# pingooio/pingoo

Hardware: AMD Instinct MI355X
Metric: requests/sec matched (whole node), 1k-rule WAF (higher is better)
Workload: dtype u8

## Files before the change

### pingoo_amd/csrc/engine.cpp

```cpp
#include <hip/hip_runtime_api.h>

#include <cstdio>
#include <algorithm>
#include <cstring>
#include <map>
#include <memory>
#include <mutex>
#include <string>
#include <type_traits>
#include <unordered_map>
#include <vector>

#include "dirtable.h"
#include "georec.h"
#include "frontend.h"
#include "kernels.h"
#include "lscan_split.h"
#include "program.h"
#include "records.h"

using namespace pwaf;

struct pwaf_program {
    std::unique_ptr<Program> p;
// ... 81 lines not shown
struct PinBuf {
    void *p = nullptr;
    size_t cap = 0;
    int reserve(size_t bytes) {
        if (bytes <= cap) return PWAF_OK;
        if (p) (void)hipHostFree(p);
        p = nullptr;
        cap = 0;
        size_t want = bytes + bytes / 4 + 4096;
        hipError_t e = hipHostMalloc(&p, want, hipHostMallocPortable);
        if (e != hipSuccess) return fail(PWAF_E_NOMEM, std::string("hipHostMalloc failed: ") + hipGetErrorString(e));
        cap = want;
        return PWAF_OK;
    }
    void release() {
        if (p) (void)hipHostFree(p);
        p = nullptr;
        cap = 0;
    }
};

template <class T>
int upload(DevBuf &b, const std::vector<T> &v, size_t pad_bytes = 0) {
    size_t bytes = v.size() * sizeof(T);
    int rc = b.reserve(bytes + pad_bytes + 16);
    if (rc) return rc;
    if (bytes) HIP_TRY(hipMemcpy(b.p, v.data(), bytes, hipMemcpyHostToDevice));
    if (pad_bytes + 16) HIP_TRY(hipMemset((char *)b.p + bytes, 0, pad_bytes + 16));
    return PWAF_OK;
}

struct FlatDev {
    DevBuf flat, flat_classmap, emit_off, emit_list, end_off, end_list, delta;
    uint32_t n_states = 0, n_classes = 0;
    bool scalar_mode = false;
    uint32_t ill_class = 0;
    uint32_t n_full = 0, n_delta = 0;
    void release() {
        for (DevBuf *b : {&flat, &flat_classmap, &emit_off, &emit_list, &end_off, &end_list, &delta}) b->release();
        n_states = 0;
    }
};

struct DevGroup {
    DevBuf tab, classmap, special, list_off, list;
    uint32_t n_states, stride, n_classes, n_hot, start_emit, emit_base, special_base, atom_base, n_local;
    bool scalar_mode = false;
    uint32_t ill_class = 0;
    uint8_t field;
    uint32_t chunks = 1;
    int gate = -1;
    bool filtered = false;
    int share_owner = -1;
    uint32_t shared_bits = 0;
    int need_slot = -1;
    int visit_slot = -1;
    bool identity = false;
    GroupFilter filter;
    DevBuf ftable;
    FlatDev fl, rt;
    bool short_lit = false;
    DevBuf c_head, c_entries, c_bytes, c_classes;
    bool confirm = false;
    bool confirm_walk = false;
};

}

struct Scratch {
    std::mutex mu;
    hipStream_t stream = nullptr, side = nullptr;
    hipEvent_t ev_fork = nullptr, ev_join = nullptr, done = nullptr;
    bool used = false;
    hipStream_t last = nullptr;
    bool last_own = false;
    DevBuf status;
    uint64_t pool_entries = 0;
    struct View { void *p = nullptr; };
    View res_cols;
    bool retry = false;
    DevBuf err_sink;
    DevBuf ipres;
    DevBuf rec, pool, gate_lists, attr;
    DevBuf verdict_spill;
    DevBuf res_words;
    DevBuf zero_block;
    View ctrl, cand_bits, visit_bits, walk_bits;
    DevBuf chunk_bits, cand_cnt;
    DevBuf need;
    DevBuf pairs;
    DevBuf zero_off;
    static constexpr uint32_t kArgSlots = 8;
    DevBuf args;
    PinBuf arg_slot[kArgSlots];
    hipEvent_t arg_ev[kArgSlots] = {};
    bool arg_pending[kArgSlots] = {};
    uint32_t arg_next = 0;
    std::vector<DevBuf> stage_field_data, stage_field_off;
    DevBuf stage_ip, stage_v6, stage_port, stage_flags, stage_asn, stage_country, stage_out, stage_counts;
    DevBuf stage_hits, stage_hit_counts;
    DevBuf stage_geo;
    PinBuf pin_in, pin_out, pin_status;
    DevBuf packed;
    DevBuf rec_meta, rec_cols;
    PinBuf rec_pin, rec_back;
    int ensure(bool own_stream) {
        if (!side) {
            int least = 0, greatest = 0;
            (void)hipDeviceGetStreamPriorityRange(&least, &greatest);
            if (switches().side_priority_high) least = greatest;
            if (hipStreamCreateWithPriority(&side, hipStreamNonBlocking, least) != hipSuccess || hipEventCreateWithFlags(&ev_fork, hipEventDisableTiming) != hipSuccess ||
                hipEventCreateWithFlags(&ev_join, hipEventDisableTiming) != hipSuccess || hipEventCreateWithFlags(&done, hipEventDisableTiming) != hipSuccess)
                return fail(PWAF_E_DEVICE, "hipStreamCreate / hipEventCreate failed");
            for (hipEvent_t &ev : arg_ev)
                if (hipEventCreateWithFlags(&ev, hipEventDisableTiming) != hipSuccess) return fail(PWAF_E_DEVICE, "hipEventCreate failed");
        }
        if (own_stream && !stream && hipStreamCreateWithFlags(&stream, hipStreamNonBlocking) != hipSuccess) return fail(PWAF_E_DEVICE, "hipStreamCreate failed");
        return PWAF_OK;
    }
    void release() {
        for (DevBuf *b : {&status, &ipres, &rec, &res_words, &err_sink, &pool, &verdict_spill, &zero_block, &gate_lists, &attr, &chunk_bits, &cand_cnt, &need, &pairs, &zero_off, &args, &stage_ip, &stage_v6, &stage_port, &stage_flags,
                          &stage_asn, &stage_country, &stage_out, &stage_counts, &stage_geo, &stage_hits, &stage_hit_counts})
            b->release();
        for (PinBuf &b : arg_slot) b.release();
        for (hipEvent_t ev : arg_ev)
            if (ev) (void)hipEventDestroy(ev);
        for (auto &b : stage_field_data) b.release();
        for (auto &b : stage_field_off) b.release();
        packed.release();
        for (PinBuf *b : {&pin_in, &pin_out, &pin_status}) b->release();
        rec_meta.release();
        rec_cols.release();
        rec_pin.release();
        rec_back.release();
        if (stream) (void)hipStreamDestroy(stream);
        if (side) (void)hipStreamDestroy(side);
        for (hipEvent_t ev : {ev_fork, ev_join, done})
            if (ev) (void)hipEventDestroy(ev);
    }
};
static constexpr size_t kContexts = 3;

struct pwaf_engine {
    pwaf_program prog;
    int device = 0;
    std::vector<std::unique_ptr<Scratch>> ctx;
    size_t next_ctx = 0;
    std::vector<DevGroup> groups;
    DevBuf num_atoms, bit_atoms , trig_off, trig_rules, always_rules, country_luts , rules, lits, set_masks;
    uint32_t cmp_vars = 0;
    uint32_t cc_words = 1, n_cmp_atoms = 0, n_bit_atoms = 0, n_trig = 0, n_lazy = 0;
    DevBuf lazy_atoms;
    std::vector<uint32_t> lazy_vars;
    uint32_t n_short = 0;
    int short_field = -1;
    DevBuf short_atoms;
    uint32_t class_words = 1, acmp_words = 0, geo_default = 0, n_classes = 1;
    DevBuf class_rows, dir_esc, leaf_root, geo_leaf_root;
    std::vector<uint32_t> host_cc_masks, host_iu_masks1;
    std::vector<std::pair<uint32_t, uint32_t>> host_acmp;
    std::vector<int64_t> host_iu_vals1;
    DevBuf iu_vals[2], iu_masks[2];
    uint32_t iu_n[2] = {0, 0}, iu_words[2] = {1, 1};
    DevBuf ip_root4, ip_root6, ip_nodes, geo_root4, geo_root6, geo_nodes, geo_recs;
    std::mutex mu;
    std::mutex prof_mu;
    DevBuf residual_errors;
    std::string residual_note;
    JitKernel residual_jit;
    DevBuf residual_blob, geo_rec_root4, geo_rec_root6, geo_rec_nodes;
    DevBuf pass_base, colmask, dir24 , dir_chunks, dir_vals, dir_summary;
    uint32_t dir_sum_shift = 0, dir_common = 0;
    uint32_t dir_n_esc = 0, dir_n_vals = 0;
// ... 506 lines not shown
            HIP_TRY(hipEventCreate(&x));
            e->ev.push_back(x);
        }
        HIP_TRY(hipEventRecord(e->ev[ev_i], on));
        ev_i++;
        return PWAF_OK;
    }
    int begin(hipStream_t side = nullptr) {
        if (off()) return PWAF_OK;
        if (!side && last_main >= 0) { open_begin = last_main; return PWAF_OK; }
        const int rc = record(side ? side : stream);
        if (rc) return rc;
        open_begin = (long)ev_i - 1;
        if (!side) last_main = open_begin;
        return PWAF_OK;
    }
    int end(const char *name, uint64_t alg_bytes, hipStream_t side = nullptr) {
        if (sync_each) {
            hipError_t se = hipStreamSynchronize(side ? side : stream);
            fprintf(stderr, "[pwaf] %s done: %s\n", name, hipGetErrorString(se));
        }
        if (off()) return PWAF_OK;
        const int rc = record(side ? side : stream);
        if (rc) return rc;
        if (!side) last_main = (long)ev_i - 1;
        pwaf_kernel_time t{};
        snprintf(t.name, sizeof t.name, "%s", name);
        t.alg_bytes = alg_bytes;
        e->times.push_back(t);
        e->time_ev.push_back({(size_t)open_begin, ev_i - 1});
        return PWAF_OK;
    }
    void commit() { e->n_timed = ev_i; }
};

struct ArgSlotMark {
    Scratch &S;
    hipStream_t stream;
    int slot = -1;
    int record() {
        if (slot < 0) return PWAF_OK;
        const int k = slot;
        slot = -1;
        S.arg_pending[k] = true;
        HIP_TRY(hipEventRecord(S.arg_ev[k], stream));
        return PWAF_OK;
    }
    ~ArgSlotMark() { (void)record(); }
};

struct BatchRun {
    pwaf_engine *e;
    Scratch &S;
    const Program &P;
    const pwaf_batch &db;
    hipStream_t stream;
    const std::vector<uint32_t> *col_begin;
    const Switches &sw;
    KernelTimer prof;
    ArgSlotMark arg_slot;
    uint32_t n, n_groups, residual_pass, n_passes, bit_words, pair_stride;
    size_t n_slots, ctrl_words;
    uint32_t pool_cap = 0;
    uint32_t *status_word = nullptr;
    bool zero_deferred = false;
    size_t zero_bytes = 0;
    std::vector<pwaf_strcol> cols;
    std::vector<uint32_t> col_bytes;
    std::vector<uint8_t> col_known;
    VerdictArgs v{};
    bool ipres_launched = false, attr_launched = false;
    pwaf_geo *d_geo = nullptr;
    ListShape lshapes[2];
    std::vector<uint32_t> filter_index;
    std::vector<FilterArgs> fall;
    std::vector<FilterArgs> by_stride[2];
    std::vector<ConfirmArgs> call;
    std::vector<ListScanArgs> la[2];
    ColPtrChunk ptrs{};
    uint64_t alg_bytes[3] = {0, 0, 0};
    const FilterArgs *d_all = nullptr, *d_s1 = nullptr, *d_s2 = nullptr;
    const ConfirmArgs *d_c = nullptr;
    const ListScanArgs *d_la[2] = {nullptr, nullptr};
    uint32_t *c_plan = nullptr, *l_plan = nullptr;

    BatchRun(pwaf_engine *e_, Scratch &S_, const pwaf_batch &db_, hipStream_t stream_, const std::vector<uint32_t> *col_begin_)
        : e(e_), S(S_), P(*e_->prog.p), db(db_), stream(stream_), col_begin(col_begin_), sw(switches()), prof(e_, stream_), arg_slot{S_, stream_} {
        n = db.n;
        n_groups = (n + 63) / 64;
        residual_pass = (uint32_t)e->groups.size() + (P.fcmp.empty() ? 0u : 1u);
        n_passes = residual_pass + (P.n_residual ? 1u : 0u);
        bit_words = 2 * n_groups;
        pair_stride = std::max(1u, e->n_bit_atoms + e->n_cmp_atoms + e->n_short);
        n_slots = (size_t)std::max(kGapLists, e->n_gated);
        ctrl_words = 2 + n_slots + e->n_filtered;
    }


    int reserve_scratch(bool sync_status) {
        int rc;
        const uint64_t pool_cap64 = std::max<uint64_t>(std::max<uint64_t>(1u << 20, (uint64_t)n * 8), S.pool_entries);
        pool_cap = (uint32_t)std::min<uint64_t>(pool_cap64, 0x7FFFFFF0u);
        S.pool_entries = pool_cap;
        if (!S.status.p) {
            if ((rc = S.status.reserve(8))) return rc;
            HIP_TRY(hipMemsetAsync(S.status.p, 0, 8, stream));
        }
        status_word = (uint32_t *)S.status.p + (sync_status ? 1 : 0);
        if ((rc = S.rec.reserve((size_t)std::max(1u, n_passes) * n * 4))) return rc;
        if ((rc = S.attr.reserve(((size_t)n_groups * pair_stride + 64) * 16 + (size_t)n_groups * 4))) return rc;
        if ((rc = S.pool.reserve((size_t)pool_cap * sizeof(PoolEntry)))) return rc;
        uint32_t n_conf = 0;
        for (const DevGroup &d : e->groups) n_conf += (d.filtered && d.confirm) ? 1u : 0u;
        Layout z;
        const size_t z_ctrl = z.take(4 * ctrl_words), z_cand = z.take((size_t)e->n_filtered * bit_words * 4), z_visit = z.take((size_t)e->n_visit * bit_words * 4),
                     z_walk = z.take((size_t)n_conf * bit_words * 4);
        zero_bytes = z.size();
        if ((rc = S.zero_block.reserve(zero_bytes))) return rc;
        zero_deferred = e->n_filtered != 0;
        for (const DevGroup &d : e->groups) zero_deferred = zero_deferred && (d.gate >= 0 || d.identity || d.short_lit);
        if (!zero_deferred) HIP_TRY(hipMemsetAsync(S.zero_block.p, 0, zero_bytes, stream));
        char *const zbase = (char *)S.zero_block.p;
        S.ctrl.p = zbase + z_ctrl;
        S.cand_bits.p = zbase + z_cand;
        S.visit_bits.p = zbase + z_visit;
        S.walk_bits.p = zbase + z_walk;
        if (e->n_gated && (rc = S.gate_lists.reserve((size_t)e->n_gated * n * 4))) return rc;
        if (e->n_need && (rc = S.need.reserve((size_t)e->n_need * n * 4))) return rc;
        return PWAF_OK;
    }

    int resolve_columns(bool totals_known) {
        int rc;
        cols.resize(e->n_fields);
        col_bytes.assign(e->n_fields, 0);
        for (int f = 0; f < PWAF_N_FIELDS; f++) {
            cols[(size_t)f] = db.field[f];
            col_bytes[(size_t)f] = db.field_bytes[f];
        }
        bool missing_header = false;
        for (uint32_t f = PWAF_N_FIELDS; f < e->n_fields; f++) {
            const uint32_t k = f - PWAF_N_FIELDS;
            if (k < db.n_headers && db.headers != nullptr && db.headers[k].data != nullptr && db.headers[k].offsets != nullptr) {
                cols[f] = db.headers[k];
                col_bytes[f] = db.header_bytes ? db.header_bytes[k] : 0u;
            } else {
                missing_header = true;
            }
        }
        if (missing_header) {
            if (S.zero_off.cap < (size_t)(n + 1) * 4 + PWAF_ARENA_PAD) {
                if ((rc = S.zero_off.reserve((size_t)(n + 1) * 4 + PWAF_ARENA_PAD))) return rc;
                HIP_TRY(hipMemsetAsync(S.zero_off.p, 0, S.zero_off.cap, stream));
            }
            for (uint32_t f = PWAF_N_FIELDS; f < e->n_fields; f++)
                if (cols[f].data == nullptr) {
                    cols[f].data = (const uint8_t *)S.zero_off.p;
                    cols[f].offsets = (const uint32_t *)S.zero_off.p;
                    col_bytes[f] = 0;
                }
        }
        col_known.assign(e->n_fields, totals_known ? 1 : 0);
        for (uint32_t f = 0; f < e->n_fields; f++)
            if (col_bytes[f] != 0 || cols[f].data == (const uint8_t *)S.zero_off.p) col_known[f] = 1;
        return PWAF_OK;
    }

    int fill_verdict_args(pwaf_verdict *d_out, pwaf_counts *d_counts, uint32_t *d_match_idx, uint32_t *d_n_matches) {
        int rc;
        v.n = n;
        v.n_groups = n_groups;
        v.force_global_tables = (P.flags & PWAF_OPT_GLOBAL_VERDICT_TABLES) ? 1u : 0u;
        v.sparse_mode = verdict_mode(P.flags);
        if (v.sparse_mode) {
            const VerdictShape vs = verdict_shape(P.n_cols, (uint32_t)P.rules.size(), e->n_trig, (uint32_t)P.lits.size(), v.force_global_tables != 0, (int)v.sparse_mode, n_passes);
            v.v_cap = vs.v_cap;
            const bool entry_list = v.sparse_mode >= 3;
            const uint32_t spill_cols = entry_list ? P.n_cols : P.n_cols - std::min(vs.v_cap, P.n_cols);
            if (entry_list || spill_cols) {
                if ((rc = S.verdict_spill.reserve((size_t)verdict_blocks_sp(vs, e->n_cus) * vs.waves * spill_cols * 8))) return rc;
                v.spill = (unsigned long long *)S.verdict_spill.p;
            }
        }
        v.debug_skip = sw.debug_skip | (sw.attr_prio ? 0x80000000u : 0u);
        for (int f = 0; f < PWAF_N_FIELDS; f++) v.off[f] = db.field[f].offsets;
        v.ip = db.ip;
        v.ip_is_v6 = db.ip_is_v6;
        v.port = db.port;
        v.flags = db.flags;
        v.asn = db.asn;
        v.country = db.country;
        v.n_cols = P.n_cols;
        v.n_passes = n_passes;
        v.rec = (const uint32_t *)S.rec.p;
        v.passes = (const PassInfo *)e->pass_table.p;
        if (P.n_residual && e->residual_jit.function) {
            v.res_words = (P.n_residual + 31u) / 32u;
            v.res_base = P.residual_base;
            if ((rc = S.res_words.reserve((size_t)v.res_words * n * 4))) return rc;
            v.res_match = (const uint32_t *)S.res_words.p;
        }
        v.cand_bits = (const uint32_t *)S.cand_bits.p;
        v.visit_bits = (const uint32_t *)S.visit_bits.p;
        v.bit_words = bit_words;
        v.n_hlen = (uint32_t)e->hlen_fields.size();
        for (size_t k = 0; k < e->hlen_fields.size(); k++) v.hoff[k] = cols[e->hlen_fields[k]].offsets;
        v.gpairs = (uint4 *)S.attr.p;
        v.ghdr = (uint32_t *)((char *)S.attr.p + ((size_t)n_groups * pair_stride + 64) * 16);
        v.pair_stride = pair_stride;
        v.attr_blocks = e->n_cus;
        v.pool = (const PoolEntry *)S.pool.p;
        v.cmp = (const CmpAtomDev *)e->num_atoms.p;
        v.n_cmp = e->n_cmp_atoms;
        v.cmp_vars = e->cmp_vars;
        v.lazy = (const CmpAtomDev *)e->lazy_atoms.p;
        v.n_lazy = e->n_lazy;
        v.n_lazy_var = (uint32_t)e->lazy_vars.size();
        for (size_t k = 0; k < e->lazy_vars.size(); k++) v.lazy_var[k] = e->lazy_vars[k];
        v.n_short = e->n_short;
        v.short_atoms = (const ShortAtom *)e->short_atoms.p;
        if (e->n_short) {
            v.short_data = cols[(size_t)e->short_field].data;
            v.short_off = cols[(size_t)e->short_field].offsets;
        }
        v.n_trig = e->n_trig;
        v.n_lits = (uint32_t)P.lits.size();
        v.bit_col = (const uint32_t *)e->bit_atoms.p;
        v.trig_off = (const uint32_t *)e->trig_off.p;
        v.trig_rules = (const uint16_t *)e->trig_rules.p;
        v.always_rules = (const uint32_t *)e->always_rules.p;
        for (int var = 0; var < 2; var++) {
            v.iu_vals[var] = (const int64_t *)e->iu_vals[var].p;
            v.iu_masks[var] = (const uint32_t *)e->iu_masks[var].p;
            v.iu_n[var] = e->iu_n[var];
            v.iu_words[var] = e->iu_words[var];
        }
        v.country_masks = (const uint32_t *)e->country_luts.p;
        v.cc_words = e->cc_words;
        v.rules = (const DevRule *)e->rules.p;
        v.n_rules = (uint32_t)P.rules.size();
        v.lits = (const uint32_t *)e->lits.p;
        set_trie_args(e, v);
        if ((rc = S.ipres.reserve((size_t)n * (v.ipres_packed ? 4 : 8) + 64))) return rc;
        v.ipres = (uint32_t *)S.ipres.p;
        v.out = d_out;
        v.counts = (unsigned long long *)d_counts;
        v.match_idx = d_match_idx;
        v.n_matches = d_n_matches;
        return PWAF_OK;
    }

    int zero_head_records() {
        for (size_t k = 0; k < e->groups.size();) {
            size_t k1 = k;
            while (k1 < e->groups.size() && e->groups[k1].filtered && !e->groups[k1].filter.heads.empty()) k1++;
            if (k1 == k) { k++; continue; }
            HIP_TRY(hipMemsetAsync((uint32_t *)S.rec.p + k * (size_t)n, 0, (k1 - k) * (size_t)n * 4, stream));
            k = k1;
        }
        return PWAF_OK;
    }

    void pick_list_shapes() {
        uint32_t variant[2] = {2, 0};
        bool all_confirm = e->n_filtered != 0;
        for (const DevGroup &d : e->groups) all_confirm = all_confirm && (!d.filtered || d.confirm);
        if (all_confirm) variant[0] = 0;
        if (sw.list_shape >= 0) {
            variant[0] = (uint32_t)sw.list_shape & 15u;
            variant[1] = (uint32_t)sw.list_shape >> 4;
        }
        for (int phase = 0; phase < 2; phase++) lshapes[phase] = list_shape(variant[phase]);
    }


    template <class Launch>
    int timed(const char *name, uint64_t bytes, const char *what, Launch &&launch, hipStream_t side = nullptr) {
        const int rc = prof.begin(side);
        if (rc) return rc;
        const int he = launch();
        if (he) return fail(PWAF_E_DEVICE, std::string(what) + " launch failed: " + hipGetErrorString((hipError_t)he));
        return prof.end(name, bytes, side);
    }

    template <class Launch>
    int side_stage(hipStream_t q, const char *name, uint64_t code, const char *what, Launch &&launch) {
        const hipStream_t side = q != stream ? q : nullptr;
        const int rc = timed(name, code, what, launch, side);
        if (rc) return rc;
        if (side) HIP_TRY(hipEventRecord(S.ev_join, q));
        return PWAF_OK;
    }
    int ipres_stage(hipStream_t q) {
        if (ipres_launched) return PWAF_OK;
        ipres_launched = true;
        if (q != stream) {
            HIP_TRY(hipEventRecord(S.ev_fork, stream));
            HIP_TRY(hipStreamWaitEvent(q, S.ev_fork, 0));
        }
        const int rc = side_stage(q, "ipres", 0xFAu, "ipres kernel", [&] { return sw.skip_ipres ? (int)hipMemsetAsync(v.ipres, 0, (size_t)n * (v.ipres_packed ? 4 : 8), q) : launch_ipres(v, q); });
        if (rc || !d_geo) return rc;
        GeoRecArgs ga{};
        set_georec_args(e, ga);
        ga.ip = db.ip;
        ga.ip_is_v6 = db.ip_is_v6;
        ga.asn = db.asn;
        ga.country = db.country;
        ga.n = n;
        ga.out = (uint2 *)d_geo;
        return side_stage(q, "georec", 25ull * n, "georec kernel", [&] { return launch_georec(ga, q); });
    }
    int attr_stage(hipStream_t q) {
        if (attr_launched) return PWAF_OK;
        attr_launched = true;
        if (q == stream && sw.placement == 0) HIP_TRY(hipStreamWaitEvent(stream, S.ev_join, 0));
        return side_stage(q, "attr", 0xFEu, "attribute kernel", [&] { return sw.skip_attr ? (int)hipMemsetAsync(v.ghdr, 0, (size_t)n_groups * 4, q) : launch_attr(v, q); });
    }
    int attr_at_start() {
        int rc;
        if (sw.placement == 0) return ipres_stage(S.side);
        if (sw.placement == 3) return (rc = ipres_stage(S.side)) ? rc : attr_stage(S.side);
        return PWAF_OK;
    }
    int attr_after_filter() {
        int rc;
        switch (sw.placement) {
        case 0: return attr_stage(stream);
        case 1: return (rc = ipres_stage(stream)) ? rc : attr_stage(stream);
        case 2: return (rc = ipres_stage(S.side)) ? rc : attr_stage(S.side);
        default: return PWAF_OK;
        }
    }
    int join_side() {
        if (sw.placement >= 2) HIP_TRY(hipStreamWaitEvent(stream, S.ev_join, 0));
        return PWAF_OK;
    }

    int launch_plain_scans() {
        static const char *fn[5] = {"host", "url", "path", "method", "user_agent"};
        for (size_t gi = 0; gi < e->groups.size(); gi++) {
            const DevGroup &d = e->groups[gi];
            if (d.gate >= 0 || d.identity || d.short_lit) continue;
            const ScanArgs a = scan_args(gi);
            char nm[48];
            if (d.field < PWAF_N_FIELDS) snprintf(nm, sizeof nm, "scan_%s_g%zu", fn[d.field], gi);
            else snprintf(nm, sizeof nm, "scan_hdr%u_g%zu", d.field - PWAF_N_FIELDS, gi);
            prof.streaming = true;
            const int rc = timed(nm, (uint64_t)col_bytes[d.field] + 4ull * (n + 1), "scan kernel", [&] { return launch_scan(a, stream); });
            prof.streaming = false;
            if (rc) return rc;
        }
        return PWAF_OK;
    }

    int launch_filter_stage() {
        prof.streaming = true;
        const int rc = timed(by_stride[1].empty() ? "filter_s1" : by_stride[0].empty() ? "filter_s2" : "filter_mix", alg_bytes[1] + alg_bytes[2], "filter kernel", [&] {
            return launch_filter(by_stride[0].data(), (uint32_t)by_stride[0].size(), d_s1, by_stride[1].data(), (uint32_t)by_stride[1].size(), d_s2, stream);
        });
        prof.streaming = false;
        return rc;
    }
    int launch_resolve_stage() {
        bool any_list = false;
        for (const DevGroup &d : e->groups) any_list = any_list || (d.filtered && !d.confirm);
        return timed("resolve+compact", 0xFCu, "resolve / compact kernel", [&] {
            const int he = launch_resolve(fall.data(), (uint32_t)fall.size(), d_all, stream);
            return !he && any_list ? launch_compact(fall.data(), (uint32_t)fall.size(), d_all, stream) : he;
        });
    }
    int launch_confirm_stage() {
        if (call.empty()) return PWAF_OK;
        return timed("confirm", 0xF8u, "confirm kernel", [&] { return launch_confirm(call.data(), (uint32_t)call.size(), d_c, c_plan, e->n_cus, stream); });
    }
    int launch_list_scans() {
        uint32_t *plan_at = l_plan;
        for (int phase = 0; phase < 2; phase++) {
            uint32_t first = 0;
            for (const uint32_t cnt : e->lscan_launches[phase]) {
                char nm[48];
                snprintf(nm, sizeof nm, "lscan_x%u", cnt);
                const int rc = timed(nm, 0xFDu, "gated scan kernel", [&] { return launch_scan_gated(la[phase].data() + first, cnt, d_la[phase] + first, plan_at, lshapes[phase], stream); });
                if (rc) return rc;
                plan_at += 2 * cnt + 1;
                first += cnt;
            }
        }
        return PWAF_OK;
    }
    int launch_fcmp_stage() {
        if (P.fcmp.empty()) return PWAF_OK;
        FcmpArgs fa{};
        std::vector<uint32_t> slots;
        for (size_t k = 0; k < P.fcmp.size(); k++) {
            uint32_t sl[2];
            const uint32_t fld[2] = {P.fcmp[k].a, P.fcmp[k].b};
            for (int q = 0; q < 2; q++) {
                size_t at = std::find(slots.begin(), slots.end(), fld[q]) - slots.begin();
                if (at == slots.size()) slots.push_back(fld[q]);
                sl[q] = (uint32_t)at;
            }
            fa.atoms[k] = P.fcmp[k].op | (sl[0] << 8) | (sl[1] << 16);
        }
        for (size_t q = 0; q < slots.size() && q < kMaxFcmpFields; q++) {
            fa.data[q] = cols[slots[q]].data;
            fa.off[q] = cols[slots[q]].offsets;
        }
        fa.n = n;
        fa.n_atoms = (uint32_t)P.fcmp.size();
        fa.rec = (uint32_t *)S.rec.p + e->groups.size() * (size_t)n;
        set_pool(fa);
        return timed("fcmp", 0xFBu, "field comparison kernel", [&] { return launch_fcmp(fa, stream); });
    }
    template <class Args>
    int residual_inputs(Args &a) {
        a.data = (const uint8_t *const *)S.res_cols.p;
        a.off = (const uint32_t *const *)((const char *)S.res_cols.p + (size_t)e->n_fields * 8);
        a.blob = (const uint8_t *)e->residual_blob.p;
        a.n = n;
        a.n_rules = P.n_residual;
        a.ip = db.ip;
        a.ip_is_v6 = db.ip_is_v6;
        a.port = db.port;
        a.asn = db.asn;
        a.country = db.country;
        a.has_geo = (P.has_geo && P.residual_needs_geo) ? 1u : 0u;
        a.geo_root4 = (const uint32_t *)e->geo_rec_root4.p;
        a.geo_root6 = (const uint32_t *)e->geo_rec_root6.p;
        a.geo_nodes = (const uint32_t *)e->geo_rec_nodes.p;
        a.geo_recs = (const GeoRec *)e->geo_recs.p;
        a.rule_errors = (unsigned long long *)e->residual_errors.p;
        if (S.retry) {
            const int rc = S.err_sink.reserve((size_t)P.n_residual * 8);
            if (rc) return rc;
            a.rule_errors = (unsigned long long *)S.err_sink.p;
        }
        return PWAF_OK;
    }
    int launch_residual_stage() {
        if (!P.n_residual) return PWAF_OK;
        int rc;
        if (e->residual_jit.function) {
            ResidualJitArgs ja{};
            if ((rc = residual_inputs(ja))) return rc;
            ja.match_words = (uint32_t *)S.res_words.p;
            return timed("residual_jit", 0xF9u, "specialized residual kernel", [&] { return launch_residual_jit(e->residual_jit, ja, e->n_cus, stream); });
        }
        ResidualArgs ra{};
        if ((rc = residual_inputs(ra))) return rc;
        ra.rec = (uint32_t *)S.rec.p + (size_t)residual_pass * n;
        set_pool(ra);
        return timed("residual", 0xF9u, "residual kernel", [&] { return launch_residual(ra, stream); });
    }
    int launch_verdict_stage() { return timed("verdict", 0xFFu, "verdict kernel", [&] { return launch_verdict(v, stream); }); }
    int dump_counts() {
        std::vector<uint32_t> cw(ctrl_words);
        HIP_TRY(hipStreamSynchronize(stream));
        HIP_TRY(hipMemcpy(cw.data(), S.ctrl.p, 4 * ctrl_words, hipMemcpyDeviceToHost));
        fprintf(stderr, "[pwaf] n %u pool %u status %u |", n, cw[0], cw[1]);
        for (size_t k = 0; k < e->groups.size(); k++) {
            const DevGroup &d = e->groups[k];
            if (d.gate >= 0) fprintf(stderr, " pass %zu field %u %s list %u", k, d.field, d.filtered ? (d.confirm ? "confirm" : "filtered") : "gap", cw[2 + (size_t)d.gate]);
        }
        for (uint32_t k = 0; k < e->n_filtered; k++) fprintf(stderr, " pairs[%u] %u", k, cw[2 + n_slots + k]);
        fprintf(stderr, "\n");
        return PWAF_OK;
    }


    template <class Args>
    void set_pool(Args &a) const {
        a.pool = (PoolEntry *)S.pool.p;
        a.pool_count = (uint32_t *)S.ctrl.p;
        a.pool_cap = pool_cap;
        a.status = status_word;
    }
    bool feeds_gates(size_t gi) const { return e->n_gap && e->owns_factors[gi]; }
    template <class Args>
    void set_gate_feed(Args &a, const DevGroup &d) const {
        a.colmask_local = (const uint32_t *)e->colmask.p + d.atom_base;
        a.n_local = d.n_local;
        a.gate_lists = (uint32_t *)S.gate_lists.p;
        a.gate_count = (uint32_t *)S.ctrl.p + 2;
        if constexpr (!std::is_same<Args, ScanArgs>::value) {
            a.enq_bits = (uint32_t *)S.visit_bits.p;
            a.enq_words = bit_words;
        }
    }

    ScanArgs scan_args(size_t gi) const {
        const DevGroup &d = e->groups[gi];
        ScanArgs a{};
        if (feeds_gates(gi)) set_gate_feed(a, d);
        a.data = cols[d.field].data;
        a.off = cols[d.field].offsets;
        a.n = n;
        a.tab = (const uint16_t *)d.tab.p;
        a.classmap = (const uint8_t *)d.classmap.p;
        a.umap = d.scalar_mode ? (const uint8_t *)d.classmap.p + kUmapAt : nullptr;
        a.ill_class = d.ill_class;
        a.special = (const SpecialCell *)d.special.p;
        a.list_off = (const uint32_t *)d.list_off.p;
        a.list = (const uint16_t *)d.list.p;
        a.start_emit = d.start_emit;
        a.emit_base = d.emit_base;
        a.n_cus = e->n_cus;
        a.chunks = d.chunks;
        a.special_base = d.special_base;
        a.n_states = d.n_states;
        a.stride = d.stride;
        a.n_classes = d.n_classes;
        a.n_hot = d.n_hot;
        a.rec = (uint32_t *)S.rec.p + gi * (size_t)n;
        set_pool(a);
        return a;
    }

    int learn_arena_sizes() {
        bool ask = false;
        for (const DevGroup &d : e->groups)
            if (d.filtered && !col_known[d.field]) {
                HIP_TRY(hipMemcpyAsync(&col_bytes[d.field], cols[d.field].offsets + n, 4, hipMemcpyDeviceToHost, stream));
                ask = true;
            }
        if (ask) HIP_TRY(hipStreamSynchronize(stream));
        return PWAF_OK;
    }

    uint32_t slab0_of(uint32_t field) const { return col_begin ? (*col_begin)[field] / kStreamSlab : 0u; }

    int build_filter_args() {
        int rc;
        filter_index.assign(e->groups.size(), 0);
        if (!e->n_filtered) return PWAF_OK;
        const uint32_t words = (n + 31) / 32, n_cblocks = (words + kCompactWords - 1) / kCompactWords;
        uint64_t sub_entries = 0, n_slabs_all = 0, pair_bytes = 0;
        for (const DevGroup &d : e->groups)
            if (d.filtered) {
                const uint64_t slabs = slab_count(col_bytes[d.field], slab0_of(d.field));
                n_slabs_all += slabs;
                sub_entries += slabs * (kStreamSlab / 512);
                if (d.confirm) pair_bytes += (uint64_t)pair_cap_of((uint32_t)slabs, n) * sizeof(uint2);
            }
        if ((rc = S.chunk_bits.reserve((size_t)sub_entries * 4))) return rc;
        if ((rc = S.cand_cnt.reserve((size_t)(2 * n_slabs_all + (uint64_t)e->n_filtered * n_cblocks) * 4))) return rc;
        if (pair_bytes && (rc = S.pairs.reserve((size_t)pair_bytes))) return rc;
        const bool dense_switch = !(P.flags & PWAF_OPT_NO_DENSE_SWITCH);
        uint32_t fi = 0;
        uint64_t sub_at = 0, cnt_at = 0, pair_at = 0;
        for (size_t gi = 0; gi < e->groups.size(); gi++) {
            const DevGroup &d = e->groups[gi];
            if (!d.filtered) continue;
            fall.emplace_back();
            FilterArgs &f = fall.back();
            f.data = cols[d.field].data;
            f.off = cols[d.field].offsets;
            f.n = n;
            f.total = col_bytes[d.field];
            f.init = d.filter.init;
            f.mul = d.filter.mul;
            f.stride = d.filter.stride;
            f.debug = sw.filter_debug_skip;
            f.table = (const uint32_t *)d.ftable.p;
            f.n_heads = (uint32_t)std::min<size_t>(2, d.filter.heads.size());
            for (uint32_t h = 0; h < f.n_heads; h++) {
                const FilterHead &fh = d.filter.heads[h];
                uint8_t lit[16] = {0}, msk[16] = {0};
                memcpy(lit, fh.bytes, fh.len);
                memset(msk, 0xFF, fh.len);
                memcpy(f.head_w[h], lit, 16);
                memcpy(f.head_m[h], msk, 16);
                f.head_len[h] = fh.len | ((uint32_t)fh.exact << 8);
                f.head_code[h] = h == 0 ? (uint32_t)fh.local + 1u : ((uint32_t)fh.local + 1u) << 15;
            }
            f.slab0 = slab0_of(d.field);
            const uint32_t slabs = slabs_of(f);
            f.rec = (uint32_t *)S.rec.p + gi * (size_t)n;
            f.chunk_bits = (uint32_t *)S.chunk_bits.p + sub_at;
            f.sub_count = (uint32_t *)S.cand_cnt.p + cnt_at;
            f.pair_base = f.sub_count + slabs;
            f.block_count = f.pair_base + slabs;
            f.bitmap = (uint32_t *)S.cand_bits.p + (size_t)fi * bit_words;
            filter_index[gi] = fi;
            f.list = (uint32_t *)S.gate_lists.p + (size_t)d.gate * n;
            f.list_count = (uint32_t *)S.ctrl.p + 2 + d.gate;
            if (d.confirm) {
                f.pair_cap = pair_cap_of(slabs, n);
                f.pairs = (uint2 *)((char *)S.pairs.p + pair_at);
                f.pair_count = (uint32_t *)S.ctrl.p + 2 + n_slots + fi;
                pair_at += (uint64_t)f.pair_cap * sizeof(uint2);
                if (dense_switch) {
                    f.dense_flag = f.pair_count;
                    f.dense_thresh = (uint32_t)std::min<uint64_t>(0xFFFFFFFEu, (uint64_t)slabs * (kStreamSlab / 16) / 2);
                }
            }
            f.first_block = 0;
            sub_at += (uint64_t)slabs * (kStreamSlab / 512);
            cnt_at += 2 * slabs + n_cblocks;
            alg_bytes[f.stride == 2 ? 2 : 1] += (uint64_t)f.total + 4ull * (n + 1);
            fi++;
        }
        for (const FilterArgs &f : fall) {
            std::vector<FilterArgs> &sub = by_stride[f.stride == 2 ? 1 : 0];
            const uint32_t block = sub.empty() ? 0u : sub.back().first_block + (slabs_of(sub.back()) + kFilterWaves - 1) / kFilterWaves;
            sub.push_back(f);
            sub.back().first_block = block;
        }
        return PWAF_OK;
    }

    ConfirmArgs confirm_args(const FilterArgs &f, const DevGroup &d, size_t gi, uint32_t wi) const {
        ConfirmArgs c{};
        c.data = f.data;
        c.off = f.off;
        c.n = n;
        c.total = f.total;
        c.pairs = f.pairs;
        c.pair_count = f.pair_count;
        c.pair_cap = f.pair_cap;
        c.mul = f.mul;
        c.stride = f.stride;
        c.init = f.init;
        c.ftable = f.table;
        c.c_head = (const uint32_t *)d.c_head.p;
        c.c_entries = (const ConfirmEntry *)d.c_entries.p;
        c.c_bytes = (const uint8_t *)d.c_bytes.p;
        c.c_classes = (const uint32_t *)d.c_classes.p;
        c.n_entries = (uint32_t)d.filter.confirm.entries.size();
        c.n_bytes = (uint32_t)d.filter.confirm.bytes.size() & ~3u;
        c.n_class_words = (uint32_t)d.filter.confirm.classes.size();
        c.rec = f.rec;
        c.valid_bits = f.bitmap;
        c.dense_flag = f.dense_flag;
        c.dense_thresh = f.dense_thresh;
        c.walk_bits = (uint32_t *)S.walk_bits.p + (size_t)wi * bit_words;
        if (d.confirm_walk) {
            c.walk_list = f.list;
            c.walk_count = f.list_count;
        }
        set_pool(c);
        if (feeds_gates(gi)) {
            set_gate_feed(c, d);
            c.shared_bits = d.shared_bits;
        }
        return c;
    }
    void build_confirm_args() {
        for (size_t gi = 0; gi < e->groups.size(); gi++) {
            const DevGroup &d = e->groups[gi];
            if (d.filtered && d.confirm) call.push_back(confirm_args(fall[filter_index[gi]], d, gi, (uint32_t)call.size()));
        }
    }

    ListScanArgs list_args(size_t gi, const ListShape &lshape, bool full_table = false) const {
        const DevGroup &d = e->groups[gi];
        ListScanArgs a{};
        const DevGroup &src = d.share_owner >= 0 ? e->groups[(size_t)d.share_owner] : d;
        if (!d.identity) {
            a.req_list = (const uint32_t *)S.gate_lists.p + (size_t)src.gate * n;
            a.n_list = (const uint32_t *)S.ctrl.p + 2 + src.gate;
        }
        if (d.visit_slot >= 0) a.visited = (uint32_t *)S.visit_bits.p + (size_t)d.visit_slot * bit_words;
        if (d.share_owner >= 0) {
            a.need_in = (const uint32_t *)S.need.p + (size_t)src.need_slot * n;
            a.need_bit = (uint32_t)d.gate;
        }
        if (feeds_gates(gi)) {
            set_gate_feed(a, d);
            if (d.need_slot >= 0) {
                a.need_out = (uint32_t *)S.need.p + (size_t)d.need_slot * n;
                a.shared_bits = d.shared_bits;
            }
        }
        if (d.confirm) a.merge_rec = 1;
        a.behind_filter = d.filtered ? 1u : 0u;
        a.data = cols[d.field].data;
        a.off = cols[d.field].offsets;
        a.n = n;
        const FlatDev &F = (d.confirm && d.rt.n_states && !full_table) ? d.rt : d.fl;
        a.flat = (const uint16_t *)F.flat.p;
        a.classmap = (const uint8_t *)F.flat_classmap.p;
        a.umap = F.scalar_mode ? (const uint8_t *)F.flat_classmap.p + kUmapAt : nullptr;
        a.ill_class = F.ill_class;
        a.n_classes = F.n_classes;
        const uint32_t row_bytes = 2u * (F.n_classes + 3u), hb = list_hot_bytes(lshape);
        if (F.n_delta && (uint64_t)F.n_full * row_bytes + 48u + 8ull * F.n_delta <= hb) {
            a.n_hot = F.n_full;
            a.n_delta = F.n_delta;
            a.delta = (const uint64_t *)F.delta.p;
        } else {
            a.n_hot = std::min<uint32_t>(F.n_delta ? F.n_full : F.n_states, (hb - 48u) / row_bytes);
        }
        a.emit_off = (const uint32_t *)F.emit_off.p;
        a.emit_list = (const uint16_t *)F.emit_list.p;
        a.end_off = (const uint32_t *)F.end_off.p;
        a.end_list = (const uint16_t *)F.end_list.p;
        a.rec = (uint32_t *)S.rec.p + gi * (size_t)n;
        set_pool(a);
        a.n_cus = e->n_cus;
        return a;
    }
    const FilterArgs *dense_of(size_t gi) const {
        const FilterArgs *f = e->groups[gi].filtered ? &fall[filter_index[gi]] : nullptr;
        return f && f->dense_flag ? f : nullptr;
    }
    static void set_dense(ListScanArgs &a, const FilterArgs &f, uint32_t mode) {
        a.dense_flag = f.dense_flag;
        a.dense_thresh = f.dense_thresh;
        a.dense_mode = mode;
    }
    void build_list_args() {
        for (int phase = 0; phase < 2; phase++)
            for (size_t gi = 0; gi < e->groups.size(); gi++) {
                const DevGroup &d = e->groups[gi];
                if (d.identity ? phase != 0 : (d.gate < 0 || d.filtered != (phase == 0))) continue;
                const FilterArgs *const dense = phase == 0 && d.confirm ? dense_of(gi) : nullptr;
                const FilterArgs *const owner_dense = d.share_owner >= 0 ? dense_of((size_t)d.share_owner) : nullptr;
                if (dense) {
                    ListScanArgs a = list_args(gi, lshapes[phase], true);
                    a.req_list = nullptr;
                    a.n_list = nullptr;
                    a.merge_rec = 0;
                    a.visited = (uint32_t *)S.cand_bits.p + (size_t)filter_index[gi] * bit_words;
                    set_dense(a, *dense, 1);
                    la[phase].push_back(a);
                }
                if (d.confirm && !d.confirm_walk) continue;
                if (sw.skip_identity && d.identity) continue;
                ListScanArgs a = list_args(gi, lshapes[phase]);
                if (dense) set_dense(a, *dense, 2);
                else if (owner_dense) set_dense(a, *owner_dense, 3);
                la[phase].push_back(a);
            }
    }
    int check_list_plan() const {
        for (int phase = 0; phase < 2; phase++) {
            size_t planned = 0;
            for (const uint32_t c : e->lscan_launches[phase]) planned += c;
            if (planned != la[phase].size()) return fail(PWAF_E_DEVICE, "list-scan launch plan does not match the batch's descriptors");
        }
        return PWAF_OK;
    }
    void build_column_pointers() {
        if (!P.n_residual) return;
        const size_t nc = e->n_fields;
        ptrs.count = (uint32_t)(2 * nc);
        for (size_t f = 0; f < nc; f++) { ptrs.p[f] = cols[f].data; ptrs.p[nc + f] = cols[f].offsets; }
    }

    int upload_descriptors() {
        int rc;
        struct Part { size_t at; const void *src; size_t bytes; };
        const size_t b_all = fall.size() * sizeof(FilterArgs), b_s1 = by_stride[0].size() * sizeof(FilterArgs), b_s2 = by_stride[1].size() * sizeof(FilterArgs),
                     b_c = call.size() * sizeof(ConfirmArgs), b_l0 = la[0].size() * sizeof(ListScanArgs), b_l1 = la[1].size() * sizeof(ListScanArgs),
                     b_ptrs = (size_t)ptrs.count * sizeof(void *);
        Layout L;
        const Part up[7] = {{L.take(b_all), fall.data(), b_all}, {L.take(b_s1), by_stride[0].data(), b_s1}, {L.take(b_s2), by_stride[1].data(), b_s2}, {L.take(b_c), call.data(), b_c},
                            {L.take(b_l0 + sizeof(ListScanArgs)), la[0].data(), b_l0}, {L.take(b_l1 + sizeof(ListScanArgs)), la[1].data(), b_l1}, {L.take(b_ptrs), ptrs.p, b_ptrs}};
        const size_t up_bytes = L.size();
        const size_t a_cplan = L.take((call.size() + 2) * 4), a_lplan = L.take((lsplit::plan_words(e->lscan_launches[0]) + lsplit::plan_words(e->lscan_launches[1])) * 4);
        if ((rc = S.args.reserve(L.size()))) return rc;
        char *const abase = (char *)S.args.p;
        d_all = (const FilterArgs *)(abase + up[0].at);
        d_s1 = (const FilterArgs *)(abase + up[1].at);
        d_s2 = (const FilterArgs *)(abase + up[2].at);
        d_c = (const ConfirmArgs *)(abase + up[3].at);
        d_la[0] = (const ListScanArgs *)(abase + up[4].at);
        d_la[1] = (const ListScanArgs *)(abase + up[5].at);
        S.res_cols.p = abase + up[6].at;
        c_plan = (uint32_t *)(abase + a_cplan);
        l_plan = (uint32_t *)(abase + a_lplan);
        if (up_bytes) {
            const uint32_t slot = S.arg_next++ % Scratch::kArgSlots;
            if (S.arg_pending[slot]) HIP_TRY(hipEventSynchronize(S.arg_ev[slot]));
            if ((rc = S.arg_slot[slot].reserve(up_bytes))) return rc;
            char *const hb = (char *)S.arg_slot[slot].p;
            for (const Part &p : up)
                if (p.bytes) memcpy(hb + p.at, p.src, p.bytes);
            arg_slot.slot = (int)slot;
            const int he = upload_args_block(hb, S.args.p, up_bytes, zero_deferred ? S.zero_block.p : nullptr, zero_deferred ? zero_bytes : 0, stream);
            if (he) return fail(PWAF_E_DEVICE, std::string("descriptor upload failed: ") + hipGetErrorString((hipError_t)he));
        } else if (zero_deferred) {
            HIP_TRY(hipMemsetAsync(S.zero_block.p, 0, zero_bytes, stream));
        }
        zero_deferred = false;
        return PWAF_OK;
    }
};

int run_pipeline(pwaf_engine *e, Scratch &S, const pwaf_batch &db , pwaf_verdict *d_out, pwaf_counts *d_counts, uint32_t *d_match_idx,
                 uint32_t *d_n_matches, hipStream_t stream, bool totals_known = false, const std::vector<uint32_t> *col_begin = nullptr, bool sync_status = false,
                 pwaf_geo *d_geo = nullptr, const HitOut *d_hits = nullptr) {
    if (db.n == 0) return PWAF_OK;
    BatchRun b(e, S, db, stream, col_begin);
    b.d_geo = d_geo;
    int rc;
    if ((rc = b.reserve_scratch(sync_status)) || (rc = b.resolve_columns(totals_known))) return rc;
    if ((rc = b.fill_verdict_args(d_out, d_counts, d_match_idx, d_n_matches)) || (rc = b.zero_head_records())) return rc;
    if (d_hits && d_hits->any()) {
        b.v.hits = d_hits->hits;
        b.v.hits_cap = d_hits->cap;
        b.v.n_hits = d_hits->n_hits;
        b.v.rule_hits = (unsigned long long *)d_hits->rule_hits;
    }
    b.pick_list_shapes();
    if ((rc = b.attr_at_start()) || (rc = b.launch_plain_scans())) return rc;
    if ((rc = b.learn_arena_sizes()) || (rc = b.build_filter_args())) return rc;
    b.build_confirm_args();
    b.build_list_args();
    b.build_column_pointers();
    if ((rc = b.check_list_plan()) || (rc = b.upload_descriptors())) return rc;
    if (e->n_filtered) {
        if ((rc = b.launch_filter_stage())) return rc;
        if (!b.sw.attr_after_compact && (rc = b.attr_after_filter())) return rc;
        if ((rc = b.launch_resolve_stage()) || (rc = b.launch_confirm_stage())) return rc;
    }
    if ((rc = b.attr_after_filter())) return rc;
    if ((rc = b.launch_list_scans()) || (rc = b.launch_fcmp_stage()) || (rc = b.launch_residual_stage())) return rc;
    if ((rc = b.join_side()) || (rc = b.launch_verdict_stage())) return rc;
    if (b.sw.dump_counts && (rc = b.dump_counts())) return rc;
    if ((rc = b.arg_slot.record())) return rc;
    b.prof.commit();
    return PWAF_OK;
}

hipError_t mark_context_used(Scratch &S, hipStream_t s, bool own) {
    S.used = true;
    S.last = s;
    S.last_own = own;
    return hipEventRecord(S.done, s);
}

int device_error(const char *call, hipError_t he) { return fail(PWAF_E_DEVICE, std::string(call) + ": " + hipGetErrorString(he)); }

template <class After>
int run_with_retry(pwaf_engine *e, Scratch &S, const pwaf_batch &db, pwaf_verdict *d_out, pwaf_counts *d_counts, bool known, const std::vector<uint32_t> *begins, bool counts_zero,
                   After &&after, pwaf_geo *d_geo = nullptr, const HitOut *d_hits = nullptr) {
    const hipStream_t s = S.stream;
    int r = S.pin_status.reserve(16);
    volatile uint32_t *const st = (volatile uint32_t *)S.pin_status.p;
    for (int attempt = 0;; attempt++) {
        hipError_t he = hipSuccess;
        if (!r && d_counts && !(counts_zero && attempt == 0) && (he = hipMemsetAsync(d_counts, 0, sizeof *d_counts, s)) != hipSuccess) r = device_error("hipMemsetAsync", he);
        if (!r && d_hits && d_hits->n_hits && (he = hipMemsetAsync(d_hits->n_hits, 0, 4, s)) != hipSuccess) r = device_error("hipMemsetAsync", he);
        if (!r && d_hits && d_hits->rule_hits && e->prog.p->n_user_rules && (he = hipMemsetAsync(d_hits->rule_hits, 0, (size_t)e->prog.p->n_user_rules * 8, s)) != hipSuccess)
            r = device_error("hipMemsetAsync", he);
        if (!r) {
            S.retry = attempt > 0;
            r = run_pipeline(e, S, db, d_out, d_counts, nullptr, nullptr, s, known, begins, true, d_geo, d_hits);
            S.retry = false;
        }
        if (!r) {
            he = hipMemcpyAsync((void *)&st[0], (uint32_t *)S.status.p + 1, 4, hipMemcpyDeviceToHost, s);
            if (he == hipSuccess) he = hipMemcpyAsync((void *)&st[1], S.ctrl.p, 4, hipMemcpyDeviceToHost, s);
// ... 1198 lines not shown
            const pwaf_strcol *sc = sample_col(g.field);
            if (!sc || !gf.enabled) continue;
            if (alt[k].enabled) gf = alt[k];
            const uint8_t *data = sc->data;
            const uint32_t *off = sc->offsets;
            if (gf.est_candidate_rate > 0.4) {
                gf.enabled = false;
                gf.heads.clear();
                gf.note = "the filter flags more than 40 % of the sample";
                continue;
            }
            std::vector<uint64_t> &v = visits[k];
            std::fill(v.begin(), v.end(), 0);
            std::vector<uint64_t> &rv = T.rvisits[k];
            if (g.rtier) rv.assign(g.rtier->n_states, 0);
            std::vector<uint8_t> padded;
            if (gf.confirm.enabled) {
                padded.assign(data, data + off[n]);
                padded.resize(padded.size() + 2 * PWAF_ARENA_PAD, 0);
            }
            std::vector<uint16_t> lits;
            for (uint32_t i = 0; i < n; i++) {
                bool walk;
                if (gf.confirm.enabled) {
                    lits.clear();
                    walk = confirm_field_host(gf, padded.data(), off[i], off[i + 1], lits);
                } else {
                    walk = flagged(gf, sc, i);
                }
                if (!walk) continue;
                uint32_t st = 0;
                for (uint32_t p = off[i]; p < off[i + 1]; p++) {
                    st = g.trans[(size_t)st * g.n_classes + dfa_class_at(g, data + off[i], p - off[i], off[i + 1] - off[i])];
                    v[st]++;
                }
                if (g.rtier) {
                    const DfaGroup &r = *g.rtier;
                    uint32_t rs = 0;
                    for (uint32_t p = off[i]; p < off[i + 1]; p++) {
                        rs = r.trans[(size_t)rs * r.n_classes + dfa_class_at(r, data + off[i], p - off[i], off[i + 1] - off[i])];
                        rv[rs]++;
                    }
                }
            }
        }
    }
    for (size_t k = 0; k < P.groups.size(); k++) {
        const pwaf_strcol *sc = sample_col(P.groups[k].field);
        if (!sc) continue;
        const uint32_t *off = sc->offsets;
        const uint64_t total = (uint64_t)(off[n] - off[0]);
        const uint32_t t4 = 80u, t2 = 48u;
        T.chunks[k] = total >= (uint64_t)t4 * n ? 4u : total >= (uint64_t)t2 * n ? 2u : 1u;
    }
    return PWAF_OK;
}
}

int pwaf_program_tune(pwaf_program *p, const pwaf_batch *sample) {
    if (!p || !p->p) return fail(PWAF_E_INVALID_ARG, "program is NULL");
    int rc = validate_batch_header(sample);
    if (rc) return rc;
    if (sample->memory != PWAF_MEM_HOST) return fail(PWAF_E_INVALID_ARG, "pwaf_program_tune needs a HOST-memory sample");
    if (sample->n == 0) return PWAF_OK;
    TuneOut T;
    for (const DfaGroup &g : p->p->groups) T.filters.push_back(g.filter);
    if ((rc = tune_host(*p->p, sample, T))) return rc;
    for (size_t k = 0; k < p->p->groups.size(); k++) p->p->groups[k].filter = T.filters[k];
    p->dump.clear();
    return PWAF_OK;
}

int pwaf_engine_tune(pwaf_engine *e, const pwaf_batch *sample) {
    if (!e) return fail(PWAF_E_INVALID_ARG, "engine is NULL");
    int rc = validate_batch_header(sample);
    if (rc) return rc;
    if (sample->memory != PWAF_MEM_HOST) return fail(PWAF_E_INVALID_ARG, "pwaf_engine_tune needs a HOST-memory sample");
    std::vector<std::unique_lock<std::mutex>> ctx_locks;
    for (auto &c : e->ctx) ctx_locks.emplace_back(c->mu);
    std::lock_guard<std::mutex> lock(e->mu);
    HIP_TRY(hipSetDevice(e->device));
    const Program &P = *e->prog.p;
    if (sample->n == 0) return PWAF_OK;
    TuneOut T;
    for (const DevGroup &d : e->groups) T.filters.push_back(d.filter);
    if ((rc = tune_host(P, sample, T))) return rc;
    bool rows_only = false;
#ifdef PWAF_PROFILING
    rows_only = getenv("PWAF_TUNE_ROWS_ONLY") != nullptr;
#endif
    for (size_t k = 0; k < P.groups.size() && !rows_only; k++) {
        e->groups[k].filter = T.filters[k];
        if (T.chunks[k]) e->groups[k].chunks = T.chunks[k];
    }
    for (uint32_t f = 0; f < e->n_fields && f < T.mean_len.size(); f++)
        if (T.mean_len[f] > 0) e->mean_len[f] = T.mean_len[f];
    HIP_TRY(hipDeviceSynchronize());
    for (size_t k = 0; k < P.groups.size(); k++)
        if ((rc = build_device_group(P.groups[k], P.lds_hot_budget, e->groups[k], &T.visits[k], &T.class_freq[k])) ||
            (rc = build_flat_group(P.groups[k], e->groups[k].fl, e->groups[k].filter.enabled && P.groups[k].filter_cols.empty(), &T.visits[k])) ||
            (P.groups[k].rtier && (rc = build_flat_group(*P.groups[k].rtier, e->groups[k].rt, true, T.rvisits[k].empty() ? nullptr : &T.rvisits[k]))))
            return rc;
    if ((rc = assign_lists(e))) return rc;
    HIP_TRY(hipDeviceSynchronize());
    return PWAF_OK;
}

int pwaf_engine_device_status(pwaf_engine *e) {
    if (!e) return fail(PWAF_E_INVALID_ARG, "NULL argument");
    HIP_TRY(hipSetDevice(e->device));
    HIP_TRY(hipDeviceSynchronize());
    uint32_t any = 0;
    for (auto &c : e->ctx) {
        std::lock_guard<std::mutex> lock(c->mu);
        if (!c->status.p) continue;
        uint32_t status = 0;
        HIP_TRY(hipMemcpy(&status, c->status.p, 4, hipMemcpyDeviceToHost));
        if (status) {
            HIP_TRY(hipMemset(c->status.p, 0, 4));
            uint32_t asked = 0;
            if (c->ctrl.p) HIP_TRY(hipMemcpy(&asked, c->ctrl.p, 4, hipMemcpyDeviceToHost));
            c->pool_entries = std::max<uint64_t>(c->pool_entries * 2, (uint64_t)asked + asked / 4 + 1024);
        }
        any |= status;
    }
    if (any) return fail(PWAF_E_NOMEM, "scan overflow pool exhausted: verdicts of a device-resident batch since the last status call are incomplete "
                                       "(evaluate it again: the pool has been grown; the synchronous entry points retry by themselves)");
    return PWAF_OK;
}

}
namespace {
int evaluate_one_impl(pwaf_engine *e, const pwaf_request *r, pwaf_verdict *out, pwaf_geo *geo) {
    if (r->n_headers && !r->headers) return fail(PWAF_E_INVALID_ARG, "n_headers without a headers array");
    const uint32_t n_hdr = e->n_fields - PWAF_N_FIELDS;
    const uint32_t n_cols = PWAF_N_FIELDS + n_hdr;
    std::vector<const char *> ptr{r->host, r->url, r->path, r->method, r->user_agent};
    std::vector<uint32_t> len{r->host_len, r->url_len, r->path_len, r->method_len, r->user_agent_len};
    for (uint32_t k = 0; k < n_hdr; k++) {
        const bool have = k < r->n_headers;
        ptr.push_back(have ? r->headers[k].data : nullptr);
        len.push_back(have ? r->headers[k].len : 0u);
    }
    std::vector<std::vector<uint8_t>> arena(n_cols);
    std::vector<uint32_t> offs(2 * (size_t)n_cols);
    std::vector<pwaf_strcol> hcols(n_hdr);
    std::vector<uint32_t> hbytes(n_hdr);
    pwaf_batch b{};
    b.struct_size = sizeof b;
    b.n = 1;
    b.memory = PWAF_MEM_HOST;
    for (uint32_t f = 0; f < n_cols; f++) {
        arena[f].assign(len[f] + PWAF_ARENA_PAD, 0);
        if (len[f]) {
            if (!ptr[f]) return fail(PWAF_E_INVALID_ARG, "NULL field with non-zero length");
            memcpy(arena[f].data(), ptr[f], len[f]);
        }
        offs[2 * f] = 0;
        offs[2 * f + 1] = len[f];
        pwaf_strcol &c = f < PWAF_N_FIELDS ? b.field[f] : hcols[f - PWAF_N_FIELDS];
        c.data = arena[f].data();
        c.offsets = &offs[2 * f];
        if (f >= PWAF_N_FIELDS) hbytes[f - PWAF_N_FIELDS] = len[f];
    }
    if (n_hdr) {
        b.n_headers = n_hdr;
// ... 124 lines not shown
```

### pingoo_amd/csrc/kernels.h

```cpp
#pragma once
#include <cstdint>
#include <string>
#include <vector>

#include "program.h"

namespace pwaf {

static constexpr int kMaxPasses = 250;
static constexpr int kVerdictPre = 12;
static constexpr uint32_t kGapLists = 32;
static constexpr uint32_t kMaxHeaderLens = 8;
static constexpr uint32_t kDirChunkWords = 32;

static constexpr uint32_t REC_OVERFLOW = 0x80000000u;
struct PoolEntry {
    uint32_t atom;
    uint32_t next;
};

struct SpecialCell {
    uint32_t next_off;
    uint32_t emit;
};
// ... 33 lines not shown
    uint32_t n;
    const uint16_t *flat;
    const uint8_t *classmap;
    const uint8_t *umap;
    uint32_t ill_class;
    uint32_t n_classes;
    uint32_t n_hot;
    const uint64_t *delta;
    uint32_t n_delta;
    const uint32_t *emit_off;
    const uint16_t *emit_list;
    const uint32_t *end_off;
    const uint16_t *end_list;
    uint32_t *rec;
    PoolEntry *pool;
    uint32_t *pool_count;
    uint32_t pool_cap;
    uint32_t *status;
    const uint32_t *colmask_local;
    uint32_t n_local;
    uint32_t *gate_lists;
    uint32_t *gate_count;
    uint32_t *enq_bits;
    uint32_t enq_words;
    uint32_t behind_filter;
    const uint32_t *req_list;
    const uint32_t *n_list;
    uint32_t *visited;
    uint32_t *need_out;
    uint32_t shared_bits;
    const uint32_t *need_in;
    uint32_t need_bit;
    uint32_t merge_rec;
    uint32_t n_cus;
    const uint32_t *dense_flag;
    uint32_t dense_thresh;
    uint32_t dense_mode;
};
struct ListOf {
    const uint32_t *req_list;
    uint32_t n_l;
};

struct ConfirmArgs {
    const uint8_t *data;
    const uint32_t *off;
    uint32_t n;
    uint32_t total;
    const uint2 *pairs;
    const uint32_t *pair_count;
    uint32_t pair_cap;
    uint32_t mul, stride, init;
    const uint32_t *ftable;
    const uint32_t *c_head;
    const ConfirmEntry *c_entries;
    const uint8_t *c_bytes;
    const uint32_t *c_classes;
    uint32_t n_entries, n_bytes, n_class_words;
    uint32_t *rec;
    uint32_t *valid_bits;
    uint32_t *walk_bits;
    uint32_t *walk_list;
    uint32_t *walk_count;
    PoolEntry *pool;
    uint32_t *pool_count;
    uint32_t pool_cap;
    uint32_t *status;
    const uint32_t *colmask_local;
    uint32_t n_local;
    uint32_t *gate_lists;
    uint32_t *gate_count;
    uint32_t *enq_bits;
    uint32_t enq_words;
    uint32_t shared_bits;
    const uint32_t *dense_flag;
    uint32_t dense_thresh;
};
static constexpr uint32_t kConfirmThreads = 1024;
static constexpr uint32_t kConfirmPoolBytes = 40 * 1024;
struct ConfirmTableDev {
    const ConfirmArgs *c;
    uint32_t count;
};
int launch_confirm(const ConfirmArgs *host, uint32_t count, const ConfirmArgs *dev, uint32_t *plan, uint32_t n_cus, void *stream);

static constexpr uint32_t kStreamSlab = 128 * 1024;
static constexpr uint32_t kStreamIter = 4096;
static constexpr uint32_t kFilterWaves = 4;
static constexpr uint32_t kCompactWords = 2048;
struct FilterArgs {
    const uint8_t *data;
    const uint32_t *off;
    uint32_t n;
    uint32_t total;
    uint32_t slab0;
    uint32_t init;
    uint32_t mul;
    uint32_t stride;
    const uint32_t *table;
    uint32_t n_heads;
    uint32_t head_w[2][4];
    uint32_t head_m[2][4];
    uint32_t head_len[2];
    uint32_t head_code[2];
    uint32_t *rec;
    uint32_t *chunk_bits;
    uint32_t *sub_count;
    uint32_t *bitmap;
    uint32_t *block_count;
    uint32_t *list;
    uint32_t *list_count;
    uint2 *pairs;
    uint32_t *pair_count;
    uint32_t pair_cap;
    uint32_t *pair_base;
    const uint32_t *dense_flag;
    uint32_t dense_thresh;
    uint32_t first_block;
    uint32_t debug;
};
int upload_args_block(const void *host_pinned, void *dev, size_t bytes, void *zero , size_t zero_bytes, void *stream);
struct FilterTable {
    const FilterArgs *f;
    uint32_t count;
};
struct FilterMix {
    const FilterArgs *f1, *f2;
    uint32_t count1, count2, blocks1, blocks2;
};
int launch_filter(const FilterArgs *host1, uint32_t count1, const FilterArgs *dev1, const FilterArgs *host2, uint32_t count2, const FilterArgs *dev2, void *stream);
int launch_resolve(const FilterArgs *host, uint32_t count, const FilterArgs *dev, void *stream);
int launch_compact(const FilterArgs *host, uint32_t count, const FilterArgs *dev, void *stream);
int configure_kernels(int device);

static constexpr uint32_t kSrcSet = 0, kSetWordsMax = 16, kSrcCc = 16, kCcWordsMax = 8, kSrcPort = 24, kSrcAsn = 28, kIntWordsMax = 4, kSrcAcmp = 32, kAcmpWordsMax = 4,
                          kSrcWords = 36;
struct PassInfo {
    uint32_t base;
    uint32_t kind_slot;
};
struct FcmpArgs {
    const uint8_t *data[kMaxFcmpFields];
    const uint32_t *off[kMaxFcmpFields];
    uint32_t atoms[kMaxFcmpAtoms];
    uint32_t n, n_atoms;
    uint32_t *rec;
    PoolEntry *pool;
    uint32_t *pool_count;
    uint32_t pool_cap;
    uint32_t *status;
};
int launch_fcmp(const FcmpArgs &a, void *stream);
struct ResidualArgs {
    const uint8_t *const *data;
    const uint32_t *const *off;
    const uint8_t *blob;
    uint32_t n, n_rules;
    const uint8_t *ip;
    const uint8_t *ip_is_v6;
    const uint16_t *port;
    const uint32_t *asn;
    const uint16_t *country;
    uint32_t has_geo;
    const uint32_t *geo_root4, *geo_root6, *geo_nodes;
    const GeoRec *geo_recs;
    uint32_t *rec;
    PoolEntry *pool;
    uint32_t *pool_count;
    uint32_t pool_cap;
    uint32_t *status;
    unsigned long long *rule_errors;
};
int launch_residual(const ResidualArgs &a, void *stream);
struct ResidualJitArgs {
    const uint8_t *const *data;
    const uint32_t *const *off;
    const uint8_t *blob;
    uint32_t n, n_rules;
    const uint8_t *ip;
    const uint8_t *ip_is_v6;
    const uint16_t *port;
    const uint32_t *asn;
    const uint16_t *country;
    uint32_t has_geo, pad;
    const uint32_t *geo_root4, *geo_root6, *geo_nodes;
    const GeoRec *geo_recs;
    uint32_t *match_words;
    unsigned long long *rule_errors;
};
struct JitKernel {
    void *module = nullptr, *function = nullptr;
};
static constexpr uint32_t kMaxJitRules = 256;
bool rvm_specialize(const uint8_t *blob, size_t len, std::string &out, std::string &why);
bool rvm_jit_program(const uint8_t *blob, size_t len, std::string &out, std::string &why);
bool rtc_compile(const std::string &source, const std::string &arch, std::vector<char> &code, std::string &why);
bool jit_load(const std::vector<char> &code, JitKernel &out, std::string &why);
void jit_release(JitKernel &k);
int launch_residual_jit(const JitKernel &k, const ResidualJitArgs &a, uint32_t n_cus, void *stream);
struct ColPtrChunk {
    const void *p[2 * (PWAF_N_FIELDS + kMaxHeaders)];
    uint32_t count;
};
struct CmpAtomDev {
    uint32_t col, c;
};
struct ShortAtom {
    uint32_t col;
    uint32_t len_exact;
    uint32_t lit_lo, lit_hi;
};
struct VerdictArgs {
    uint32_t n, n_groups;
    uint32_t debug_skip;
    uint32_t force_global_tables;
    uint32_t sparse_mode;
    uint32_t v_cap;
    unsigned long long *spill;
    const uint32_t *off[PWAF_N_FIELDS];
    const uint8_t *ip;
    const uint8_t *ip_is_v6;
    const uint16_t *port;
    const uint8_t *flags;
    const uint32_t *asn;
    const uint16_t *country;
    uint32_t n_passes;
    const uint32_t *rec;
    const PassInfo *passes;
    const uint32_t *res_match;
    uint32_t res_words, res_base;
    const uint32_t *cand_bits, *visit_bits;
    uint32_t bit_words;
    const uint32_t *hoff[kMaxHeaderLens];
    const ShortAtom *short_atoms;
    uint32_t n_short;
    const uint8_t *short_data;
    const uint32_t *short_off;
    uint32_t n_hlen;
    const PoolEntry *pool;
    uint32_t n_cols;
    const CmpAtomDev *cmp;
    uint32_t n_cmp;
    uint32_t cmp_vars;
    const CmpAtomDev *lazy;
    uint32_t n_lazy;
    uint32_t lazy_var[4], n_lazy_var;
    const uint32_t *bit_col;
    const int64_t *iu_vals[2];
    const uint32_t *iu_masks[2];
    uint32_t iu_n[2], iu_words[2];
    const uint32_t *country_masks;
    uint32_t cc_words;
    const DevRule *rules;
    uint32_t n_rules;
    const uint32_t *lits;
    uint32_t n_lits, n_trig;
    const uint32_t *trig_off;
    const uint16_t *trig_rules;
    const uint32_t *always_rules;
    const uint32_t *ip_root4, *ip_root6, *ip_nodes;
    const uint32_t *set_masks;
    uint32_t set_words;
    uint32_t n_ip_lists;
    const uint32_t *geo_root4, *geo_root6, *geo_nodes;
    const uint32_t *dir24;
    const uint32_t *dir_chunks, *dir_vals;
    const uint32_t *dir_summary;
    uint32_t dir_sum_shift, dir_common;
    const uint2 *dir_esc;
    const uint32_t *class_rows;
    uint32_t class_words;
    uint32_t acmp_words;
    uint32_t geo_default;
    uint32_t *ipres;
    uint32_t ipres_packed;
    uint32_t has_geo;
    uint4 *gpairs;
    uint32_t *ghdr;
    uint32_t pair_stride;
    uint32_t attr_blocks;
    pwaf_verdict *out;
    unsigned long long *counts;
    uint32_t *match_idx;
    uint32_t *n_matches;
    pwaf_rule_hit *hits;
    uint32_t hits_cap;
    uint32_t *n_hits;
    unsigned long long *rule_hits;
};

int launch_scan(const ScanArgs &a, void *stream);
struct GatedTable {
    const ListScanArgs *g;
    uint32_t count;
    uint32_t debug;
};
struct ListShape {
    uint32_t threads, hot_bytes, wg_per_cu;
};
ListShape list_shape(uint32_t variant);
uint32_t list_hot_bytes(const ListShape &shape);
int launch_scan_gated(const ListScanArgs *host, uint32_t count, const ListScanArgs *dev, uint32_t *plan, const ListShape &shape, void *stream);
int launch_verdict(const VerdictArgs &a, void *stream);
int launch_ipres(const VerdictArgs &a, void *stream);
int launch_attr(const VerdictArgs &a, void *stream);
int launch_dir24(const VerdictArgs &a, void *out , void *esc, void *esc_count, void *stream);
struct GeoRecArgs {
    const uint8_t *ip, *ip_is_v6;
    const uint32_t *asn;
    const uint16_t *country;
    uint32_t n, has_geo;
    const uint32_t *root4, *root6, *nodes;
    const GeoRec *recs;
    const uint32_t *chunks, *vals, *summary;
    uint32_t sum_shift, common;
    uint32_t n_cus;
    uint2 *out;
};
int launch_georec(const GeoRecArgs &a, void *stream);
uint32_t scan_lds_bytes(uint32_t n_hot, uint32_t stride, uint32_t n_gate_atoms);
struct VerdictShape {
    uint32_t waves, lds_bytes, lds_tables;
    uint32_t sparse, v_cap, per_cu;
};
VerdictShape verdict_shape(uint32_t n_cols, uint32_t n_rules, uint32_t n_trig, uint32_t n_lits, bool force_global = false, int mode = 3, uint32_t n_passes = 0);
uint32_t verdict_blocks_sp(const VerdictShape &sh, uint32_t n_cus);

}
```

### pingoo_amd/csrc/kernels.hip

```cpp
#include <hip/hip_runtime.h>

#include <cstdlib>
#include <mutex>
#include <set>

#include "confirm.h"
#include "utf8.h"
#include "kernels.h"
#include "residual.h"

namespace pwaf {

static constexpr int kScanThreads = 1024;
static constexpr int kScanWaves = kScanThreads / 64;
static constexpr uint32_t kNone = 0xFFFFFFFFu;

#define PWAF_LDS __attribute__((address_space(3)))
#define PWAF_GLOBAL __attribute__((address_space(1)))
typedef const PWAF_LDS uint16_t *lds_u16_ptr;
typedef const PWAF_GLOBAL uint16_t *glb_u16_ptr;
typedef const PWAF_LDS uint32_t *lds_u32_ptr;
typedef const PWAF_LDS uint8_t *lds_u8_ptr;
typedef unsigned int u32x4 __attribute__((ext_vector_type(4)));
typedef u32x4 u32x4_u __attribute__((aligned(1)));
// ... 311 lines not shown
                        if (!slow && t >= emit_base) {
                            const uint32_t code = *reinterpret_cast<lds_u16_ptr>((uintptr_t)((t << 1) + emit_col2 + kClsBytes));
                            const uint32_t x = (code & 0x7FFFu) + 1;
                            if (!(code & 0x8000u) || h.ovf != kNone) slow = true;
                            else if (h.a0 == x || h.a1 == x) {}
                            else if (h.a0 == 0) h.a0 = x;
                            else if (h.a1 == 0) h.a1 = x;
                            else slow = true;
                        }
                        if (slow) {
                            const Walk wk = careful_step(gtab, a.special, a.list_off, a.list, a.pool, a.pool_count, a.pool_cap, hot_elems | (emit_base << 16),
                                                         special_base | (emit_col2 << 16), cur, crow, cls, t, h.a0, h.a1, h.ovf);
                            chain = chain && wk.row == t;
                            cur = wk.row;
                            crow = wk.crow;
                            h = wk.h;
                        } else {
                            cur = t;
                        }
                    } else {
                        chain = chain && t < special_base;
                    }
                };
                redo(t1, c2[k0], (uint32_t)k0 < cnt);
                redo(t2, c2[k0 + 1], (uint32_t)(k0 + 1) < cnt);
                redo(t3, c2[k0 + 2], (uint32_t)(k0 + 2) < cnt);
                redo(t4, c2[k0 + 3], (uint32_t)(k0 + 3) < cnt);
                row = cur;
            } else {
                row = t4;
            }
        }
        }
        p += cnt_all;

        if (r != kNone && p >= end) {
            const uint32_t e = row == hot_elems ? (uint32_t)*reinterpret_cast<glb_u16_ptr>(gtab + crow + (end_col << 1))
                                                : (uint32_t)*reinterpret_cast<lds_u16_ptr>((uintptr_t)(((row + end_col) << 1) + kClsBytes));
            if (e & 0x8000u) {
                const uint32_t x = (e & 0x7FFFu) + 1;
                if (h.ovf == kNone && (h.a0 == x || h.a1 == x)) {
                } else if (h.ovf == kNone && h.a0 == 0) {
                    h.a0 = x;
                } else if (h.ovf == kNone && h.a1 == 0) {
                    h.a1 = x;
                } else {
                    const SlowCtx sc{a.list_off, a.list, a.pool, a.pool_count, a.status, a.pool_cap};
                    h = record_atom(sc, x - 1, h);
                }
            } else if (e) {
                PWAF_EMIT(e - 1);
            }
            a.rec[r] = h.ovf != kNone ? (REC_OVERFLOW | h.ovf) : (h.a0 | (h.a1 << 15));
            if (a.colmask_local != nullptr && (h.a0 | (h.ovf + 1u)) != 0) {
                uint32_t need = 1;
                if (h.ovf == kNone) {
                    need = *reinterpret_cast<lds_u32_ptr>((uintptr_t)(gate_base + (h.a0 - 1) * 4));
                    if (h.a1) need |= *reinterpret_cast<lds_u32_ptr>((uintptr_t)(gate_base + (h.a1 - 1) * 4));
                }
                if (need) enqueue_gated(a.colmask_local, a.pool, a.gate_lists, a.gate_count, a.n, r, h);
            }
            r = kNone;
        }
        if (r == kNone && r2 != kNone) {
            r = r2;
            p = p2;
            end = end2;
            r2 = kNone;
            row = 0;
            h = Hits{0, 0, kNone};
            if (start_emit) PWAF_EMIT(start_emit - 1);
        }
#pragma unroll
        for (int q = 0; q < CH; q++) w[q] = wn[q];
        n_lo = f_lo;
        n_hi = f_hi;
        n_base = f_base;
    }
}

template <int CH, bool WIDE>
__global__ __launch_bounds__(kScanThreads) void scan_kernel(ScanArgs a) { scan_body<CH, WIDE>(a); }

__device__ __forceinline__ ListOf list_of(const ListScanArgs &a) {
    ListOf l{a.req_list, a.req_list != nullptr ? min(*a.n_list, a.n) : a.n};
    if (a.dense_mode != 0u) {
        const bool dense = *a.dense_flag > a.dense_thresh;
        if (a.dense_mode == 1u && !dense) l.n_l = 0u;
        if (a.dense_mode == 2u && dense) l.n_l = 0u;
        if (a.dense_mode == 3u && dense) l = ListOf{nullptr, a.n};
    }
    return l;
}

__global__ __launch_bounds__(256) void lscan_plan_kernel(GatedTable b, uint32_t *plan , uint32_t n_waves) {
    __shared__ uint32_t part[256];
    __shared__ unsigned long long all_entries;
    const uint32_t t = threadIdx.x;
    uint32_t items = 0;
    const uint32_t n_l = t < b.count ? list_of(b.g[t]).n_l : 0u;
    if (t == 0) all_entries = 0ull;
    __syncthreads();
    if (n_l != 0u) atomicAdd(&all_entries, (unsigned long long)n_l);
    __syncthreads();
    if (t < b.count) {
        const uint32_t room = n_waves > b.count ? n_waves - b.count : 1u;
        const unsigned long long per_wave = (all_entries + room - 1u) / room;
        uint32_t epi = 1;
        while (epi < 16u && epi < per_wave) epi <<= 1;
        while (epi < 64u * kListWalks && (n_l + epi - 1) / epi > n_waves) epi <<= 1;
        items = (n_l + epi - 1) / epi;
        plan[b.count + 1 + t] = epi;
    }
    part[t] = items;
    __syncthreads();
    for (uint32_t d = 1; d < 256; d <<= 1) {
        const uint32_t v = t >= d ? part[t - d] : 0u;
        __syncthreads();
        part[t] += v;
        __syncthreads();
    }
    if (t < b.count) plan[t] = part[t] - items;
    if (t == 0) plan[b.count] = part[255];
}

__device__ __forceinline__ uint32_t list_step_slow(const uint16_t *hot, const PWAF_GLOBAL uint16_t *flat, const uint64_t *delta, const uint32_t state, const uint32_t c,
                                                   const uint32_t stride, const uint32_t n_hot, const uint32_t n_delta) {
    if (state < n_hot) return hot[state * stride + c];
    const uint32_t k = state - n_hot;
    if (k < n_delta) {
        if (c + 2u == stride) return state;
        const uint64_t rec = delta[k];
        const uint32_t lo = (uint32_t)rec, hi = (uint32_t)(rec >> 32);
        if (c == ((lo >> 16) & 0xFFu)) return hi & 0xFFFFu;
        if (c == (lo >> 24)) return hi >> 16;
        return hot[(lo & 0xFFFFu) * stride + c];
    }
    return flat[state * stride + c];
}

template <uint32_t THREADS>
__device__ __forceinline__ void lscan_async(const ListScanArgs &a, const uint16_t *hot, const unsigned char *cls, const uint64_t *delta, uint32_t it, const uint32_t it_end,
                                            const uint32_t first, const uint32_t n_l, const uint32_t hot_elems, const uint32_t epi) {
    const uint32_t ncls = a.n_classes, stride = ncls + 3u;
    const PWAF_GLOBAL unsigned char *gdata = (const PWAF_GLOBAL unsigned char *)a.data;
    const PWAF_GLOBAL uint16_t *flat = (const PWAF_GLOBAL uint16_t *)a.flat;
    auto record_emit = [&](const uint32_t st, Hits &hh) {
        const uint32_t ei = st * stride + ncls;
        const uint32_t code = ei < hot_elems ? (uint32_t)hot[ei] : (uint32_t)flat[ei];
        const uint32_t x = (code & 0x7FFFu) + 1u;
        bool slow = !(code & 0x8000u) || hh.ovf != kNone;
        if (!slow) {
            if (hh.a0 == x || hh.a1 == x) {}
            else if (hh.a0 == 0) hh.a0 = x;
            else if (hh.a1 == 0) hh.a1 = x;
            else slow = true;
        }
        if (slow) hh = emit_list(a.emit_off, a.emit_list, a.pool, a.pool_count, a.status, a.pool_cap, st, hh);
    };
    for (it += wave_index(); it < it_end; it += THREADS / 64u) {
        const uint32_t li = (it - first) * epi + (threadIdx.x & 63u);
        bool live = (threadIdx.x & 63u) < epi && li < n_l;
        if (live && a.need_in != nullptr) live = ((a.need_in[li] >> a.need_bit) & 1u) != 0;
        const uint32_t r = live ? (a.req_list != nullptr ? a.req_list[li] : li) : 0u;
        if (live && a.visited != nullptr) atomicOr(&a.visited[r >> 5], 1u << (r & 31u));
        uint32_t p = live ? a.off[r] : 0u;
        const uint32_t end = live ? a.off[r + 1] : 0u;
        uint32_t state = 0, wp = p;
        Hits h{0, 0, kNone};
        uint32_t need_init = 0;
        if (live && a.merge_rec) {
            h = hits_of_record(a.rec[r]);
            if (a.colmask_local != nullptr && (h.a0 | (h.ovf + 1u)) != 0) need_init = gate_mask(a.colmask_local, a.pool, h);
        }
        if (live && a.emit_off[1] != a.emit_off[0]) h = emit_list(a.emit_off, a.emit_list, a.pool, a.pool_count, a.status, a.pool_cap, 0u, h);
        u32x4 w = *reinterpret_cast<const PWAF_GLOBAL u32x4_u *>(gdata + wp);
        u32x4 wn = *reinterpret_cast<const PWAF_GLOBAL u32x4_u *>(gdata + (wp + 16u < end ? wp + 16u : 0u));
        for (;;) {
            const bool active = p < end;
            const unsigned long long am = __ballot(active);
            if (am == 0) break;
            if (active && p - wp >= 16u) {
                w = wn;
                wp += 16u;
                wn = *reinterpret_cast<const PWAF_GLOBAL u32x4_u *>(gdata + (wp + 16u < end ? wp + 16u : 0u));
            }
            const uint32_t j = (p - wp) >> 2;
            const uint32_t wd = j == 0 ? w.x : j == 1 ? w.y : j == 2 ? w.z : w.w;
            const uint32_t cnt = active ? min(4u, end - p) : 0u;
            uint32_t c[4], t[4], sv[4];
#pragma unroll
            for (uint32_t k = 0; k < 4; k++) c[k] = cls[(wd >> (k * 8)) & 0xFFu];
            asm volatile("" : "+v"(c[0]), "+v"(c[1]), "+v"(c[2]), "+v"(c[3]));
            if (a.umap != nullptr && __ballot(active && (wd & 0x80808080u) != 0u) != 0ull) {
                const uint32_t f_start = active ? a.off[r] : 0u;
#pragma unroll
                for (uint32_t k = 0; k < 4; k++) {
                    const uint32_t byte = (wd >> (k * 8)) & 0xFFu;
                    if (byte >= 0xC0u && k < cnt) c[k] = lead_class(a.umap, a.ill_class, gdata, byte, p + k, end);
                    else if (byte >= 0x80u && k < cnt) c[k] = cont_class(c[k], a.ill_class, gdata, p + k, f_start, end);
                }
            }
#pragma unroll
            for (uint32_t k = 0; k < 4; k++) c[k] = k < cnt ? c[k] : ncls + 1u;
#pragma unroll
            for (uint32_t k = 0; k < 4; k++) {
                t[k] = *reinterpret_cast<lds_u16_ptr>((uintptr_t)min(__umul24(k == 0 ? state : sv[k - 1], 2u * stride) + 2u * c[k], 2u * hot_elems));
                sv[k] = t[k] & 0x7FFFu;
            }
            const uint32_t any = t[0] | t[1] | t[2] | t[3], top = max(max(t[0], t[1]), max(t[2], t[3]));
            const bool blocked = active && top == 0xFFFFu;
            const unsigned long long bm = __ballot(blocked);
            const uint32_t n_blocked = (uint32_t)__builtin_popcountll(bm);
            if (n_blocked < 32u && bm != am) {
                if (active && !blocked) {
                    if (any & 0x8000u) {
#pragma unroll
                        for (uint32_t k = 0; k < 4; k++)
                            if (t[k] & 0x8000u) record_emit(sv[k], h);
                    }
                    state = sv[3];
                    p += 4u;
                }
            } else if (blocked) {
#pragma unroll
                for (uint32_t k = 0; k < 4; k++) {
                    const uint32_t tt = list_step_slow(hot, flat, delta, state, c[k], stride, a.n_hot, a.n_delta);
                    state = tt & 0x7FFFu;
                    if (tt & 0x8000u) record_emit(state, h);
                }
                p += 4u;
            }
        }
        if (live) {
            if (a.end_off[state + 1] != a.end_off[state]) h = emit_list(a.end_off, a.end_list, a.pool, a.pool_count, a.status, a.pool_cap, state, h);
            a.rec[r] = h.ovf != kNone ? (REC_OVERFLOW | h.ovf) : (h.a0 | (h.a1 << 15));
            if (a.colmask_local != nullptr) {
                uint32_t need = 0;
                if ((h.a0 | (h.ovf + 1u)) != 0) need = gate_mask(a.colmask_local, a.pool, h);
                if (a.need_out != nullptr) a.need_out[li] = need;
                need &= ~(a.shared_bits | need_init);
                if (need) enqueue_mask_once(a.gate_lists, a.gate_count, a.n, r, need, a.enq_bits, a.enq_words);
            }
        }
    }
}

template <uint32_t THREADS>
__global__ __launch_bounds__(THREADS, THREADS == 512 ? 6 : 4) void lscan_kernel(GatedTable b, const uint32_t *plan, uint32_t hot_bytes) {
    extern __shared__ uint32_t lscan_lds[];
    __builtin_amdgcn_s_setprio(3);
    if ((uint32_t)(uintptr_t)(PWAF_LDS unsigned char *)lscan_lds != 0u) __builtin_trap();
    const uint32_t total = plan[b.count];
    const uint32_t it0 = (uint32_t)((uint64_t)total * blockIdx.x / gridDim.x), it1 = (uint32_t)((uint64_t)total * (blockIdx.x + 1) / gridDim.x);
    const unsigned char *cls = reinterpret_cast<const unsigned char *>(lscan_lds + (hot_bytes + 16u) / 4);
    const uint16_t *hot = reinterpret_cast<const uint16_t *>(lscan_lds);
    for (uint32_t it = it0; it < it1;) {
        uint32_t ps = 0;
        for (uint32_t lo = 0, hi = b.count; lo + 1 < hi;) {
            const uint32_t mid = (lo + hi) >> 1;
            if (plan[mid] <= it) lo = mid;
            else hi = mid;
            ps = lo;
        }
        const uint32_t first = plan[ps], it_end = min(it1, plan[ps + 1]), epi = plan[b.count + 1 + ps];
        ListScanArgs a = load_descriptor(&b.g[ps]);
        const ListOf lst = list_of(a);
        a.req_list = lst.req_list;
        const uint32_t ncls = a.n_classes, stride = ncls + 3u;
        const uint32_t hot_elems = a.n_hot * stride;
        uint64_t *delta_lds = reinterpret_cast<uint64_t *>(lscan_lds) + (hot_elems * 2u + 2u + 15u) / 16u * 2u;
        __syncthreads();
        {
            const uint4 *src = reinterpret_cast<const uint4 *>(a.flat);
            uint4 *dst = reinterpret_cast<uint4 *>(lscan_lds);
            const uint32_t units = (hot_elems * 2u + 15u) / 16u;
            for (uint32_t k = threadIdx.x; k < units; k += THREADS * 4u) {
                uint4 v[4];
#pragma unroll
                for (uint32_t q = 0; q < 4; q++) v[q] = k + q * THREADS < units ? src[k + q * THREADS] : make_uint4(0u, 0u, 0u, 0u);
#pragma unroll
                for (uint32_t q = 0; q < 4; q++)
                    if (k + q * THREADS < units) dst[k + q * THREADS] = v[q];
            }
            if (threadIdx.x < 64) lscan_lds[(hot_bytes + 16u) / 4 + threadIdx.x] = reinterpret_cast<const uint32_t *>(a.classmap)[threadIdx.x];
            for (uint32_t k = threadIdx.x; k < a.n_delta; k += THREADS) delta_lds[k] = a.delta[k];
        }
        __syncthreads();
        if (threadIdx.x == 0) reinterpret_cast<uint16_t *>(lscan_lds)[hot_elems] = 0xFFFFu;
        __syncthreads();
        const uint32_t n_l = lst.n_l;
#ifdef PWAF_PROFILING
        const bool long_list = (b.debug & 1u) ? false : (b.debug & 2u) ? true : (a.behind_filter != 0u && (uint64_t)n_l * 8u >= a.n);
#else
        const bool long_list = a.behind_filter != 0u && (uint64_t)n_l * 8u >= a.n;
#endif
        if (long_list) {
            lscan_async<THREADS>(a, hot, cls, delta_lds, it, it_end, first, n_l, hot_elems, epi);
            it = it_end;
            continue;
        }
        const PWAF_GLOBAL unsigned char *gdata = (const PWAF_GLOBAL unsigned char *)a.data;
        const PWAF_GLOBAL uint16_t *flat = (const PWAF_GLOBAL uint16_t *)a.flat;
        for (uint32_t iw = it + wave_index(); iw < it_end; iw += THREADS / 64u) {
            uint32_t li[kListWalks], r[kListWalks], p[kListWalks], end[kListWalks], state[kListWalks], need_init[kListWalks];
            bool live[kListWalks];
            Hits h[kListWalks];
            u32x4 w[kListWalks];
#pragma unroll
            for (uint32_t u = 0; u < kListWalks; u++) {
                li[u] = (iw - first) * epi + u * 64u + (threadIdx.x & 63u);
                live[u] = (threadIdx.x & 63u) + u * 64u < epi && li[u] < n_l;
                if (live[u] && a.need_in != nullptr) live[u] = ((a.need_in[li[u]] >> a.need_bit) & 1u) != 0;
                r[u] = live[u] ? (a.req_list != nullptr ? a.req_list[li[u]] : li[u]) : 0u;
            }
#pragma unroll
            for (uint32_t u = 0; u < kListWalks; u++) {
                if (live[u] && a.visited != nullptr) atomicOr(&a.visited[r[u] >> 5], 1u << (r[u] & 31));
                p[u] = live[u] ? a.off[r[u]] : 0u;
                end[u] = live[u] ? a.off[r[u] + 1] : 0u;
                state[u] = 0;
                h[u] = Hits{0, 0, kNone};
                need_init[u] = 0;
                if (live[u] && a.merge_rec) {
                    h[u] = hits_of_record(a.rec[r[u]]);
                    if (a.colmask_local != nullptr && (h[u].a0 | (h[u].ovf + 1u)) != 0) need_init[u] = gate_mask(a.colmask_local, a.pool, h[u]);
                }
            }
#pragma unroll
            for (uint32_t u = 0; u < kListWalks; u++) {
                if (live[u] && a.emit_off[1] != a.emit_off[0]) h[u] = emit_list(a.emit_off, a.emit_list, a.pool, a.pool_count, a.status, a.pool_cap, 0u, h[u]);
                w[u] = *reinterpret_cast<const PWAF_GLOBAL u32x4_u *>(gdata + p[u]);
// ... 27 lines not shown
                    if (a.umap != nullptr) lead_here = lead_here || (cnt[u] != 0u && window_has_high(w[u]));
                }
                const bool fix_classes = a.umap != nullptr && __ballot(lead_here) != 0ull;
#pragma unroll
                for (uint32_t k0 = 0; k0 < 16; k0 += 4) {
                    uint32_t c[kListWalks][4], t[kListWalks][4], sv[kListWalks][4];
#pragma unroll
                    for (uint32_t u = 0; u < kListWalks; u++) {
                        const uint32_t wd = k0 == 0 ? w[u].x : k0 == 4 ? w[u].y : k0 == 8 ? w[u].z : w[u].w;
#pragma unroll
                        for (uint32_t k = 0; k < 4; k++) {
                            const uint32_t cl = cls[(wd >> (k * 8)) & 0xFFu];
                            c[u][k] = k0 + k < cnt[u] ? cl : ncls + 1u;
                        }
                        if (fix_classes) {
#pragma unroll
                            for (uint32_t k = 0; k < 4; k++) {
                                const uint32_t byte = (wd >> (k * 8)) & 0xFFu;
                                if (byte >= 0xC0u && k0 + k < cnt[u]) c[u][k] = lead_class(a.umap, a.ill_class, gdata, byte, p[u] + k0 + k, end[u]);
                                else if (byte >= 0x80u && k0 + k < cnt[u]) c[u][k] = cont_class(c[u][k], a.ill_class, gdata, p[u] + k0 + k, live[u] ? a.off[r[u]] : 0u, end[u]);
                            }
                        }
                    }
#pragma unroll
                    for (uint32_t k = 0; k < 4; k++) {
#pragma unroll
                        for (uint32_t u = 0; u < kListWalks; u++) {
                    t[u][k] = *reinterpret_cast<lds_u16_ptr>((uintptr_t)min(__umul24(k == 0 ? state[u] : sv[u][k - 1], 2u * stride) + 2u * c[u][k], 2u * hot_elems));
                            sv[u][k] = t[u][k] & 0x7FFFu;
                        }
                    }
                    uint32_t any = 0, top = 0;
#pragma unroll
                    for (uint32_t u = 0; u < kListWalks; u++)
#pragma unroll
                        for (uint32_t k = 0; k < 4; k++) { any |= t[u][k]; top = max(top, t[u][k]); }
                    if (any & 0x8000u) {
                        if (top == 0xFFFFu) {
#pragma unroll
                            for (uint32_t k = 0; k < 4; k++) {
#pragma unroll
                                for (uint32_t u = 0; u < kListWalks; u++) {
                                    const uint32_t tt = list_step_slow(hot, flat, delta_lds, state[u], c[u][k], stride, a.n_hot, a.n_delta);
                                    state[u] = tt & 0x7FFFu;
                                    if (tt & 0x8000u) record_emit(state[u], h[u]);
                                }
                            }
                        } else {
#pragma unroll
                            for (uint32_t u = 0; u < kListWalks; u++) {
#pragma unroll
                                for (uint32_t k = 0; k < 4; k++)
                                    if (t[u][k] & 0x8000u) record_emit(sv[u][k], h[u]);
                                state[u] = sv[u][3];
                            }
                        }
                    } else {
#pragma unroll
                        for (uint32_t u = 0; u < kListWalks; u++) state[u] = sv[u][3];
                    }
                }
#pragma unroll
                for (uint32_t u = 0; u < kListWalks; u++) {
                    if (p[u] < end[u]) p[u] += 16u;
                    w[u] = wn[u];
                }
            }
#pragma unroll
            for (uint32_t u = 0; u < kListWalks; u++) {
                if (!live[u]) continue;
                if (a.end_off[state[u] + 1] != a.end_off[state[u]]) h[u] = emit_list(a.end_off, a.end_list, a.pool, a.pool_count, a.status, a.pool_cap, state[u], h[u]);
                a.rec[r[u]] = h[u].ovf != kNone ? (REC_OVERFLOW | h[u].ovf) : (h[u].a0 | (h[u].a1 << 15));
                if (a.colmask_local != nullptr) {
                    uint32_t need = 0;
                    if ((h[u].a0 | (h[u].ovf + 1u)) != 0) need = gate_mask(a.colmask_local, a.pool, h[u]);
                    if (a.need_out != nullptr) a.need_out[li[u]] = need;
                    need &= ~(a.shared_bits | need_init[u]);
                    if (need) enqueue_mask_once(a.gate_lists, a.gate_count, a.n, r[u], need, a.enq_bits, a.enq_words);
                }
            }
        }
        it = it_end;
    }
}

__global__ __launch_bounds__(256) void confirm_plan_kernel(ConfirmTableDev b, uint32_t *plan ) {
    __shared__ uint32_t part[256];
    const uint32_t t = threadIdx.x;
    uint32_t items = 0;
    if (t < b.count) {
        const ConfirmArgs *pa = &b.c[t];
        const bool dense = pa->dense_flag != nullptr && *pa->dense_flag > pa->dense_thresh;
        items = dense ? 0u : (min(*pa->pair_count, pa->pair_cap) + kConfirmThreads - 1) / kConfirmThreads;
    }
    part[t] = items;
    __syncthreads();
    for (uint32_t d = 1; d < 256; d <<= 1) {
        const uint32_t v = t >= d ? part[t - d] : 0u;
        __syncthreads();
        part[t] += v;
        __syncthreads();
    }
    if (t < b.count) plan[t] = part[t] - items;
    if (t == 0) plan[b.count] = part[255];
}

__device__ __noinline__ void merge_atom(PoolEntry *pool, uint32_t *pool_count, uint32_t *status, uint32_t pool_cap, uint32_t *rec, uint32_t atom) {
    auto rmw_read = [](uint32_t *p) { return atomicOr(p, 0u); };
    auto publish = [&](uint32_t idx, uint32_t at, uint32_t next) {
        const uint32_t t0 = atomicExch(&pool[idx].atom, at), t1 = atomicExch(&pool[idx].next, next);
        asm volatile("" ::"v"(t0), "v"(t1));
    };
    uint32_t old = rmw_read(rec);
    for (;;) {
        uint32_t upd;
        const uint32_t x = atom + 1u;
        if (!(old & REC_OVERFLOW)) {
            const uint32_t a0 = old & 0x7FFFu, a1 = (old >> 15) & 0x7FFFu;
            if (a0 == x || a1 == x) return;
            if (a0 == 0u) upd = old | x;
            else if (a1 == 0u) upd = old | (x << 15);
            else {
                const uint32_t idx = atomicAdd(pool_count, 3u);
                if (idx + 3u > pool_cap) { atomicOr(status, 1u); return; }
                publish(idx, a0 - 1u, kNone);
                publish(idx + 1u, a1 - 1u, idx);
                publish(idx + 2u, atom, idx + 1u);
                upd = REC_OVERFLOW | (idx + 2u);
            }
        } else {
            const uint32_t head = old & ~REC_OVERFLOW;
            for (uint32_t i = head; i != kNone; i = rmw_read(&pool[i].next))
                if (rmw_read(&pool[i].atom) == atom) return;
            const uint32_t idx = atomicAdd(pool_count, 1u);
            if (idx >= pool_cap) { atomicOr(status, 1u); return; }
            publish(idx, atom, head);
            upd = REC_OVERFLOW | idx;
        }
        const uint32_t seen = atomicCAS(rec, old, upd);
        if (seen == old) return;
        old = seen;
    }
}

__global__ __launch_bounds__(kConfirmThreads, 8) void confirm_kernel(ConfirmTableDev b, const uint32_t *plan) {
    __shared__ uint32_t head[kFilterEntries], ftab[kFilterEntries];
    __shared__ uint32_t pool[kConfirmPoolBytes / 4];
    constexpr uint32_t kConfirmQueue = 1024;
    __shared__ uint32_t app_cnt, app_base, app_queue[kConfirmQueue];
    __builtin_amdgcn_s_setprio(3);
    if (threadIdx.x == 0) app_cnt = 0;
    const uint32_t total = plan[b.count];
    const uint32_t it0 = (uint32_t)((uint64_t)total * blockIdx.x / gridDim.x), it1 = (uint32_t)((uint64_t)total * (blockIdx.x + 1) / gridDim.x);
    for (uint32_t it = it0; it < it1;) {
        uint32_t ps = 0;
        for (uint32_t lo = 0, hi = b.count; lo + 1 < hi;) {
            const uint32_t mid = (lo + hi) >> 1;
            if (plan[mid] <= it) lo = mid;
            else hi = mid;
            ps = lo;
        }
        const uint32_t first_item = plan[ps], it_end = min(it1, plan[ps + 1]);
        const ConfirmArgs a = load_descriptor(&b.c[ps]);
        __syncthreads();
        {
            const uint4 *sh = reinterpret_cast<const uint4 *>(a.c_head), *sf = reinterpret_cast<const uint4 *>(a.ftable);
            constexpr uint32_t kPer = kFilterEntries / 4 / kConfirmThreads;
            uint4 vh[kPer], vf[kPer];
#pragma unroll
            for (uint32_t q = 0; q < kPer; q++) { vh[q] = sh[q * kConfirmThreads + threadIdx.x]; vf[q] = sf[q * kConfirmThreads + threadIdx.x]; }
#pragma unroll
            for (uint32_t q = 0; q < kPer; q++) {
                reinterpret_cast<uint4 *>(head)[q * kConfirmThreads + threadIdx.x] = vh[q];
                reinterpret_cast<uint4 *>(ftab)[q * kConfirmThreads + threadIdx.x] = vf[q];
            }
        }
        const uint32_t e_words = a.n_entries * 3u, b_words = a.n_bytes / 4u, c_words = a.n_class_words;
        const bool in_lds = (uint64_t)e_words + b_words + c_words <= kConfirmPoolBytes / 4;
        const ConfirmEntry *t_entries = a.c_entries;
        const uint8_t *t_bytes = a.c_bytes;
        const uint32_t *t_classes = a.c_classes;
        if (in_lds) {
            const uint32_t *se = reinterpret_cast<const uint32_t *>(a.c_entries), *sb = reinterpret_cast<const uint32_t *>(a.c_bytes);
            for (uint32_t k = threadIdx.x; k < e_words; k += kConfirmThreads) pool[k] = se[k];
            for (uint32_t k = threadIdx.x; k < b_words; k += kConfirmThreads) pool[e_words + k] = sb[k];
            for (uint32_t k = threadIdx.x; k < c_words; k += kConfirmThreads) pool[e_words + b_words + k] = a.c_classes[k];
            t_entries = reinterpret_cast<const ConfirmEntry *>(pool);
            t_bytes = reinterpret_cast<const uint8_t *>(pool + e_words);
            t_classes = pool + e_words + b_words;
        }
        __syncthreads();
        const ConfirmView cv{nullptr, t_entries, t_bytes, t_classes, a.mul, a.stride, a.init};
        const uint32_t n_p = min(*a.pair_count, a.pair_cap);
        auto pair_of = [&](const uint32_t item) -> uint2 {
            const uint32_t k = (item - first_item) * kConfirmThreads + threadIdx.x;
            return (item < it_end && k < n_p) ? a.pairs[k] : make_uint2(kNone, 0u);
        };
        uint2 pr_next = pair_of(it), pr_after = pair_of(it + 1u);
        uint32_t fs_next = 0u, fe_next = 0u;
        ConfirmBytes tb_next{};
        if (pr_next.x != kNone) {
            confirm_load64(reinterpret_cast<const uint8_t *>(a.off + pr_next.x), fs_next, fe_next);
            tb_next = confirm_chunk_bytes(a.data, pr_next.y, a.total + PWAF_ARENA_PAD);
        }
        for (; it < it_end; it++) {
            const uint2 pr = pr_next;
            const bool live = pr.x != kNone;
            uint32_t r = live ? pr.x : 0u;
            uint32_t fs = fs_next, fe = fe_next;
            const ConfirmBytes tb = tb_next;
            pr_next = pr_after;
            if (pr_next.x != kNone) {
                confirm_load64(reinterpret_cast<const uint8_t *>(a.off + pr_next.x), fs_next, fe_next);
                tb_next = confirm_chunk_bytes(a.data, pr_next.y, a.total + PWAF_ARENA_PAD);
            }
            pr_after = pair_of(it + 2u);
            ConfirmChunk ch{0u, 0ull};
            if (live) ch = confirm_windows_of(cv, tb, 0u, 0xFFFFFFFFu, pr.y, [&](const uint32_t bin) { return ftab[bin]; });
            uint32_t mask = ch.mask, cnt = 0, j = 0, e0 = 0, pos = 0, widx = 0;
            bool walk = false;
            auto settle = [&](const uint32_t rq, const uint32_t need_lits, const bool wk, const bool aggregated) -> bool {
                bool w2 = wk;
                if (need_lits & a.shared_bits) w2 = true;
                const uint32_t direct = need_lits & ~a.shared_bits;
                if (direct) enqueue_mask_once(a.gate_lists, a.gate_count, a.n, rq, direct, a.enq_bits, a.enq_words);
                if (!w2 || a.walk_list == nullptr) return false;
                const uint32_t bit = 1u << (rq & 31u);
                if (atomicOr(&a.walk_bits[rq >> 5], bit) & bit) return false;
                atomicOr(&a.valid_bits[rq >> 5], bit);
                if (aggregated) return true;
                a.walk_list[atomicAdd(a.walk_count, 1u)] = rq;
                return false;
            };
            uint32_t need = 0;
            for (;;) {
                if (__ballot(j < cnt || mask != 0u) == 0) break;
                while (j >= cnt && mask != 0u) {
                    const uint32_t k = (uint32_t)__builtin_ctz(mask);
                    mask &= mask - 1u;
                    pos = pr.y * 16u + k;
                    const uint32_t bin = confirm_bin_of(ch, widx++, a.data, pos, a.mul);
                    while (pos >= fe && r + 1u < a.n) {
                        settle(r, need, walk, false);
                        need = 0;
                        walk = false;
                        r++;
                        fs = fe;
                        fe = a.off[r + 1];
                    }
                    if (pos >= fe) continue;
                    const uint32_t hd = head[bin];
                    e0 = hd & 0xFFFFFu;
                    cnt = hd >> 20;
                    j = 0;
                }
                if (j < cnt) {
                    const uint32_t res = in_lds ? confirm_entry<3>(t_entries, t_bytes, t_classes, e0 + j, a.data, fs, fe, pos)
                                                : confirm_entry<1>(t_entries, t_bytes, t_classes, e0 + j, a.data, fs, fe, pos);
                    j++;
                    if (res == 2u) {
                        walk = true;
                    } else if (res & 1u) {
                        const uint32_t atom = res >> 8;
                        merge_atom(a.pool, a.pool_count, a.status, a.pool_cap, a.rec + r, atom);
                        atomicOr(&a.valid_bits[r >> 5], 1u << (r & 31u));
                        if (a.colmask_local != nullptr) need |= a.colmask_local[atom];
                    }
                }
            }
            const bool append = live && settle(r, need, walk, true);
            if (append) {
                const uint32_t slot = atomicAdd(&app_cnt, 1u);
                if (slot < kConfirmQueue) app_queue[slot] = r;
                else a.walk_list[atomicAdd(a.walk_count, 1u)] = r;
            }
        }
        __syncthreads();
        {
            const uint32_t queued = min(app_cnt, kConfirmQueue);
            if (threadIdx.x == 0 && queued != 0) app_base = atomicAdd(a.walk_count, queued);
            __syncthreads();
            for (uint32_t k = threadIdx.x; k < queued; k += kConfirmThreads) a.walk_list[app_base + k] = app_queue[k];
            __syncthreads();
            if (threadIdx.x == 0) app_cnt = 0;
        }
    }
}

int launch_scan(const ScanArgs &a, void *stream) {
    const uint32_t lds = scan_lds_bytes(a.n_hot, a.stride, a.colmask_local ? a.n_local : 0u);
    const bool wide = a.n_classes > 127;
    const int v = (a.chunks == 4 ? 2 : a.chunks == 2 ? 1 : 0) + (wide ? 3 : 0);
    const void *fns[6] = {reinterpret_cast<const void *>(scan_kernel<1, false>), reinterpret_cast<const void *>(scan_kernel<2, false>),
                          reinterpret_cast<const void *>(scan_kernel<4, false>), reinterpret_cast<const void *>(scan_kernel<1, true>),
                          reinterpret_cast<const void *>(scan_kernel<2, true>), reinterpret_cast<const void *>(scan_kernel<4, true>)};
    const void *fn = fns[v];
    if (a.n == 0) return 0;
    uint32_t waves = (a.n + 255) / 256;
    uint32_t blocks = (waves + kScanWaves - 1) / kScanWaves;
#ifdef PWAF_PROFILING
    static const uint32_t forced_cap = getenv("PWAF_SCAN_BLOCKS") ? (uint32_t)atoi(getenv("PWAF_SCAN_BLOCKS")) : 0u;
#else
    const uint32_t forced_cap = 0;
#endif
    const uint32_t cap = forced_cap ? forced_cap : std::max(1u, a.n_cus);
    if (blocks > cap) blocks = cap;
    if (blocks == 0) blocks = 1;
    void *args[] = {const_cast<ScanArgs *>(&a)};
    hipError_t e = hipLaunchKernel(fn, dim3(blocks), dim3(kScanThreads), args, lds, (hipStream_t)stream);
    return (int)(e != hipSuccess ? e : hipGetLastError());
}

__global__ __launch_bounds__(256) void copy_args_kernel(const uint4 *__restrict__ src, uint4 *__restrict__ dst, uint32_t n16, uint4 *__restrict__ zero, uint32_t z16) {
    for (uint32_t i = blockIdx.x * 256u + threadIdx.x; i < n16; i += gridDim.x * 256u) dst[i] = src[i];
    for (uint32_t i = blockIdx.x * 256u + threadIdx.x; i < z16; i += gridDim.x * 256u) zero[i] = make_uint4(0u, 0u, 0u, 0u);
}
int upload_args_block(const void *host_pinned, void *dev, size_t bytes, void *zero, size_t zero_bytes, void *stream) {
    const uint32_t n16 = (uint32_t)((bytes + 15) / 16), z16 = (uint32_t)(zero_bytes / 16);
    if (n16 == 0 && z16 == 0) return 0;
    const uint32_t blocks = std::max(std::min<uint32_t>((n16 + 255) / 256, 64u), std::min<uint32_t>((z16 + 2047) / 2048, 1024u));
    hipLaunchKernelGGL(copy_args_kernel, dim3(std::max(1u, blocks)), dim3(256), 0, (hipStream_t)stream, (const uint4 *)host_pinned, (uint4 *)dev, n16, (uint4 *)zero, z16);
    return (int)hipGetLastError();
}

int launch_confirm(const ConfirmArgs *host, uint32_t count, const ConfirmArgs *dev, uint32_t *plan, uint32_t n_cus, void *stream) {
    if (count == 0 || host[0].n == 0) return 0;
    if (count > 256) return (int)hipErrorInvalidValue;
    ConfirmTableDev b{dev, count};
    hipLaunchKernelGGL(confirm_plan_kernel, dim3(1), dim3(256), 0, (hipStream_t)stream, b, plan);
    hipError_t e = hipGetLastError();
    if (e != hipSuccess) return (int)e;
    uint64_t max_items = 0;
    for (uint32_t k = 0; k < count; k++) max_items += ((uint64_t)host[k].pair_cap + kConfirmThreads - 1) / kConfirmThreads;
    const uint32_t blocks = (uint32_t)std::min<uint64_t>(max_items, (uint64_t)std::max(1u, n_cus) * 2u);
    const uint32_t *cplan = plan;
    hipLaunchKernelGGL(confirm_kernel, dim3(blocks), dim3(kConfirmThreads), 0, (hipStream_t)stream, b, cplan);
    return (int)hipGetLastError();
}

static const void *lscan_fn(bool wide) { return wide ? reinterpret_cast<const void *>(lscan_kernel<1024>) : reinterpret_cast<const void *>(lscan_kernel<512>); }

int launch_scan_gated(const ListScanArgs *host, uint32_t count, const ListScanArgs *dev, uint32_t *plan, const ListShape &shape, void *stream) {
    if (count == 0 || host[0].n == 0) return 0;
    if (count > 256) return (int)hipErrorInvalidValue;
    GatedTable b{dev, count, 0u};
#ifdef PWAF_PROFILING
    static const uint32_t async_mode = getenv("PWAF_LSCAN_ASYNC") ? (uint32_t)atoi(getenv("PWAF_LSCAN_ASYNC")) : 0u;
    b.debug = async_mode;
#endif
    const uint32_t blocks = std::max(1u, host[0].n_cus) * shape.wg_per_cu;
    hipLaunchKernelGGL(lscan_plan_kernel, dim3(1), dim3(256), 0, (hipStream_t)stream, b, plan, blocks * (shape.threads / 64u));
    hipError_t e = hipGetLastError();
    if (e != hipSuccess) return (int)e;
    const uint32_t *cplan = plan;
    uint32_t hot_bytes = list_hot_bytes(shape);
    void *args[] = {&b, &cplan, &hot_bytes};
    const void *fn = lscan_fn(shape.threads == 1024);
    e = hipLaunchKernel(fn, dim3(blocks), dim3(shape.threads), args, shape.hot_bytes + 16 + 256, (hipStream_t)stream);
    return (int)(e != hipSuccess ? e : hipGetLastError());
}

uint32_t list_hot_bytes(const ListShape &shape) { return shape.hot_bytes; }

ListShape list_shape(uint32_t variant) {
    switch (variant) {
        case 1: return ListShape{512, 72u * 1024u, 2};
        case 2: return ListShape{1024, 144u * 1024u, 1};
        case 3: return ListShape{512, 32u * 1024u, 4};
        default: return ListShape{kListThreads, kListHotBytes, 3};
    }
}

typedef unsigned short u16x2 __attribute__((ext_vector_type(2)));

template <bool HEADS, int STRIDE>
__device__ __forceinline__ void filter_rows(const FilterArgs &a, const uint32_t blk, const uint32_t wave, const uint32_t lane) {
    const PWAF_GLOBAL unsigned char *gdata = (const PWAF_GLOBAL unsigned char *)a.data;
    const uint32_t rel = blk * kFilterWaves + wave, slab = a.slab0 + rel;
    const uint64_t base64 = (uint64_t)slab * kStreamSlab;
    if (base64 >= a.total) return;
    const uint32_t total = a.total, base0 = (uint32_t)base64, slab_end = (uint32_t)min<uint64_t>(total, base64 + kStreamSlab);
    unsigned long long *my_bits = reinterpret_cast<unsigned long long *>(a.chunk_bits) + (size_t)rel * (kStreamSlab / 1024);
    uint32_t n_hit = 0;
    const uint32_t mul2 = a.mul | (a.mul << 16);
    constexpr uint32_t kRow = 1024;

    auto load_row = [&](const uint32_t b, const uint32_t q) {
        const uint32_t p = b + kRow * q + 16u * lane;
        return *reinterpret_cast<const PWAF_GLOBAL u32x4_u *>(gdata + (p < total ? p : 0u));
    };
    auto dword_at = [&](const uint32_t p) {
        return filter_fold4(*reinterpret_cast<const PWAF_GLOBAL uint32_t __attribute__((aligned(1))) *>(gdata + p));
    };
    auto slot_lo = [](const uint32_t masked) {
        uint32_t r;
        asm("v_lshrrev_b32_sdwa %0, 2, %1 dst_sel:DWORD dst_unused:UNUSED_PAD src0_sel:DWORD src1_sel:WORD_0" : "=v"(r) : "v"(masked));
        return r;
    };
    auto slot_hi = [](const uint32_t masked) {
        uint32_t r;
        asm("v_lshrrev_b32_sdwa %0, 2, %1 dst_sel:DWORD dst_unused:UNUSED_PAD src0_sel:DWORD src1_sel:WORD_1" : "=v"(r) : "v"(masked));
        return r;
    };
    auto bins4 = [&](const uint32_t x, const uint32_t next, uint32_t (&mm)[4]) {
        const uint32_t z = __builtin_amdgcn_alignbit(next, x, 8);
        const uint32_t hx = __builtin_bit_cast(uint32_t, __builtin_bit_cast(u16x2, x) * __builtin_bit_cast(u16x2, mul2));
        const uint32_t hz = __builtin_bit_cast(uint32_t, __builtin_bit_cast(u16x2, z) * __builtin_bit_cast(u16x2, mul2));
#ifdef PWAF_PROFILING
        if (a.debug & 1u) { mm[0] = hx | 0xFF000000u; mm[1] = hz | 0xFF000000u; mm[2] = (hx >> 3) | 0xFF000000u; mm[3] = (hz >> 5) | 0xFF000000u; return; }
#endif
        const uint32_t kx = hx & 0xFFF0FFF0u, kz = hz & 0xFFF0FFF0u;
        mm[0] = *reinterpret_cast<lds_u32_ptr>((uintptr_t)slot_lo(kx));
        mm[1] = *reinterpret_cast<lds_u32_ptr>((uintptr_t)slot_lo(kz));
        mm[2] = *reinterpret_cast<lds_u32_ptr>((uintptr_t)slot_hi(kx));
        mm[3] = *reinterpret_cast<lds_u32_ptr>((uintptr_t)slot_hi(kz));
    };
    auto bins2 = [&](const uint32_t x, uint32_t (&mm)[2]) {
        const uint32_t hx = __builtin_bit_cast(uint32_t, __builtin_bit_cast(u16x2, x) * __builtin_bit_cast(u16x2, mul2));
#ifdef PWAF_PROFILING
        if (a.debug & 1u) { mm[0] = hx | 0xFF000000u; mm[1] = (hx >> 3) | 0xFF000000u; return; }
#endif
        const uint32_t kx = hx & 0xFFF0FFF0u;
        mm[0] = *reinterpret_cast<lds_u32_ptr>((uintptr_t)slot_lo(kx));
        mm[1] = *reinterpret_cast<lds_u32_ptr>((uintptr_t)slot_hi(kx));
    };
    auto push = [](uint32_t &st, const uint32_t m) { asm("v_lshl_or_b32 %0, %1, 8, %2" : "=v"(st) : "v"(st), "v"(m)); };

    uint32_t rq = 0, ho[2] = {0xFFFFFFFFu, 0xFFFFFFFFu}, hn[2] = {0xFFFFFFFFu, 0xFFFFFFFFu};
    auto load_offs = [&](const uint32_t r0) {
        ho[0] = a.off[min(r0 + lane, a.n)];
        ho[1] = a.off[min(r0 + 64u + lane, a.n)];
        const uint32_t e1 = a.off[min(r0 + 128u, a.n)];
        hn[0] = (uint32_t)__builtin_amdgcn_update_dpp(__builtin_amdgcn_readfirstlane((int)ho[1]), (int)ho[0], 0x130 , 0xF, 0xF, false);
        hn[1] = (uint32_t)__builtin_amdgcn_update_dpp(__builtin_amdgcn_readfirstlane((int)e1), (int)ho[1], 0x130, 0xF, 0xF, false);
    };
    auto head_record = [&](const u32x4 w, const uint32_t flen) {
        uint32_t hrec = 0;
#pragma unroll
        for (int hq = 0; hq < 2; hq++) {
            if ((uint32_t)hq < a.n_heads) {
                const uint32_t diff = ((w.x ^ a.head_w[hq][0]) & a.head_m[hq][0]) | ((w.y ^ a.head_w[hq][1]) & a.head_m[hq][1]) |
// ... 411 lines not shown
    for (uint32_t q = 0; q < kWords / 64; q++) bits[q * 64 + lane] = slab_bits[q * 64 + lane];
    __builtin_amdgcn_fence(__ATOMIC_ACQ_REL, "wavefront");
    {
        uint32_t w[kWords / 64], mine = 0;
#pragma unroll
        for (uint32_t q = 0; q < kWords / 64; q++) {
            w[q] = bits[lane * (kWords / 64) + q];
            mine += (uint32_t)__builtin_popcount(w[q]);
        }
        uint32_t before = wave_scan_add(mine) - mine;
#pragma unroll
        for (uint32_t q = 0; q < kWords / 64; q++) {
            rank[lane * (kWords / 64) + q] = before;
            before += (uint32_t)__builtin_popcount(w[q]);
        }
    }
    __builtin_amdgcn_fence(__ATOMIC_ACQ_REL, "wavefront");
    auto rank_of = [&](const uint32_t c) {
        if (c >= kChunks) return rank[kWords - 1] + (uint32_t)__builtin_popcount(bits[kWords - 1]);
        return rank[c >> 5] + (uint32_t)__builtin_popcount(bits[c >> 5] & ((1u << (c & 31u)) - 1u));
    };
    const uint32_t back = 3u * a.stride;
    const uint64_t slab_b0 = (uint64_t)slab * kStreamSlab, b0 = slab_b0 + (uint64_t)lo_c * 16u;
    const uint32_t c_first = (uint32_t)(slab_b0 / 16);
    uint32_t lo = 0, hi = a.n;
    while (lo < hi) {
        const uint32_t span = hi - lo, step = (span + 63) / 64;
        const uint32_t probe = lo + lane * step;
        const bool ok = probe >= hi || (uint64_t)a.off[probe + 1] + back > b0;
        const unsigned long long m = __ballot(ok);
        if (m == 0) {
            lo += 63u * step + 1u;
            continue;
        }
        const uint32_t f = (uint32_t)__builtin_ctzll(m);
        const uint32_t nh = min(hi, lo + f * step);
        lo = f == 0 ? lo : lo + (f - 1u) * step + 1u;
        hi = nh;
    }
    const uint64_t b1 = slab_b0 + (uint64_t)hi_c * 16u;
    const uint32_t pair_base = a.pairs != nullptr ? a.pair_base[rel] : 0u;
    const uint32_t begin = __builtin_amdgcn_readfirstlane(a.off[0]);
    if (part == 0 && a.pairs != nullptr && (uint64_t)begin > slab_b0) {
        const uint32_t n_before = min((uint32_t)(((uint64_t)begin - slab_b0) >> 4), kChunks);
        for (uint32_t w = lane; w * 32u < n_before; w += 64) {
            uint32_t bw = bits[w];
            if (n_before - w * 32u < 32u) bw &= (1u << (n_before - w * 32u)) - 1u;
            const uint32_t word = bits[w];
            while (bw) {
                const uint32_t bit = (uint32_t)__builtin_ctz(bw);
                bw &= bw - 1u;
                const uint32_t at = pair_base + rank[w] + (uint32_t)__builtin_popcount(word & ((1u << bit) - 1u));
                if (at < a.pair_cap) a.pairs[at] = make_uint2(kNone, 0u);
            }
        }
    }
    if (sparse) {
        bool redo = false;
        for (uint32_t k = lane; k < cnt; k += 64) {
            uint32_t wlo = 0, whi = kWords;
            while (wlo + 1u < whi) {
                const uint32_t mid = (wlo + whi) >> 1;
                if (rank[mid] <= k) wlo = mid;
                else whi = mid;
            }
            uint32_t word = bits[wlo];
            for (uint32_t skip = k - rank[wlo]; skip != 0u; skip--) word &= word - 1u;
            const uint32_t chunk = c_first + wlo * 32u + (uint32_t)__builtin_ctz(word), byte0 = chunk * 16u;
            if (byte0 + 16u <= begin) continue;
            const uint32_t key = max(byte0, begin);
            uint32_t l = lo, h = min(a.n, lo + 4096u);
            const uint32_t h0 = h;
            while (l < h) {
                const uint32_t mid = (l + h) >> 1;
                if (a.off[mid + 1] > key) h = mid;
                else l = mid + 1u;
            }
            if (l == h0) {
                if (h0 < a.n) { redo = true; continue; }
                if (pair_base + k < a.pair_cap) a.pairs[pair_base + k] = make_uint2(kNone, 0u);
                continue;
            }
            if (pair_base + k < a.pair_cap) a.pairs[pair_base + k] = make_uint2(l, chunk);
            if (a.n_heads == 0) {
                uint32_t r = l, steps = 0;
                for (; r < a.n && steps < 48u; r++, steps++) {
                    const uint32_t s = a.off[r];
                    if (s >= byte0 + 16u) break;
                    if (a.off[r + 1] > s) a.rec[r] = 0u;
                }
                if (steps == 48u) redo = true;
            }
        }
        if (__ballot(redo) == 0ull) return;
    }
    {
    uint32_t s_n = 0xFFFFFFFFu, e_n = 0xFFFFFFFFu;
    {
        const uint32_t r = lo + lane;
        if (r < a.n) { s_n = a.off[r]; e_n = a.off[r + 1]; }
    }
    for (uint32_t rb = lo; rb < a.n; rb += 64) {
        const uint32_t r = rb + lane;
        const bool live = r < a.n;
        const uint32_t s = s_n, e = e_n;
        {
            const uint32_t r2 = r + 64;
            s_n = e_n = 0xFFFFFFFFu;
            if (r2 < a.n) { s_n = a.off[r2]; e_n = a.off[r2 + 1]; }
        }
        if (a.pairs != nullptr) {
            if (a.n_heads == 0 && live && e > s) {
                const uint32_t g_lo = s >> 4, g_hi = (e - 1u) >> 4;
                if (g_hi >= c_first + lo_c && g_lo < c_first + hi_c) {
                    const uint32_t y0 = g_lo > c_first + lo_c ? g_lo - c_first : lo_c, y1 = min(g_hi - c_first, hi_c - 1u);
                    if (rank_of(y1 + 1u) != rank_of(y0)) a.rec[r] = 0u;
                }
            }
            if (live && e > s) {
                const uint32_t f_lo = s == begin ? s >> 4 : (s + 15u) >> 4, f_hi = (e - 1u) >> 4;
                if (f_lo <= f_hi && f_hi >= c_first + lo_c && f_lo < c_first + hi_c) {
                    const uint32_t x0 = f_lo > c_first + lo_c ? f_lo - c_first : lo_c, x1 = min(f_hi - c_first, hi_c - 1u);
                    for (uint32_t w = x0 >> 5; w <= (x1 >> 5); w++) {
                        const uint32_t word = bits[w];
                        uint32_t bw = word;
                        if (w == (x0 >> 5)) bw &= ~0u << (x0 & 31u);
                        if (w == (x1 >> 5)) bw &= ~0u >> (31u - (x1 & 31u));
                        while (bw) {
                            const uint32_t bit = (uint32_t)__builtin_ctz(bw);
                            bw &= bw - 1u;
                            const uint32_t at = pair_base + rank[w] + (uint32_t)__builtin_popcount(word & ((1u << bit) - 1u));
                            if (at < a.pair_cap) a.pairs[at] = make_uint2(r, c_first + w * 32u + bit);
                        }
                    }
                }
            }
            if (__ballot(live && (uint64_t)s >= b1) != 0) break;
            continue;
        }
        bool mark = false;
        if (live && (uint64_t)s < b1 + 16) {
            const uint32_t j_lo = s == 0 ? 0u : (s - 1u) / 16u, j_hi = (uint32_t)(((uint64_t)e + back - 1u) / 16u);
            const uint32_t x0 = j_lo > c_first + lo_c ? j_lo - c_first : lo_c;
            if (j_hi >= c_first + lo_c && x0 < hi_c) {
                const uint32_t x1 = min(j_hi - c_first, hi_c - 1u);
                mark = x0 <= x1 && rank_of(x1 + 1u) != rank_of(x0);
            }
        }
        const unsigned long long m = __ballot(mark);
        if (m != 0) {
            const uint32_t sh = rb & 31u, w0 = rb >> 5;
            const uint32_t parts[3] = {(uint32_t)(m << sh), (uint32_t)(sh ? m >> (32u - sh) : m >> 32), sh ? (uint32_t)(m >> (64u - sh)) : 0u};
            if (lane < 3 && parts[lane] != 0) atomicOr(&a.bitmap[w0 + lane], parts[lane]);
        }
        if (__ballot(live && (uint64_t)s >= b1 + 16) != 0) break;
    }
    }
}

__global__ __launch_bounds__(256) void compact_kernel(FilterTable B) {
    __builtin_amdgcn_s_setprio(3);
    __shared__ uint32_t red[256];
    const FilterArgs a = load_descriptor(&B.f[blockIdx.y]);
    const uint32_t words = (a.n + 31) / 32, w0 = blockIdx.x * kCompactWords, tid = threadIdx.x, wave = wave_index(), lane = tid & 63;
    if (w0 >= words) return;
    const uint32_t n_blocks = (words + kCompactWords - 1) / kCompactWords;
    uint32_t acc = 0;
    for (uint32_t bq = tid; bq < blockIdx.x; bq += 256) acc += a.block_count[bq];
    red[tid] = acc;
    __syncthreads();
    for (uint32_t h = 128; h > 0; h >>= 1) {
        if (tid < h) red[tid] += red[tid + h];
        __syncthreads();
    }
    const uint32_t base = red[0];
    __syncthreads();
    constexpr uint32_t kSteps = kCompactWords / 256;
    const uint32_t wave_w0 = w0 + wave * (kSteps * 64);
    uint32_t wv[kSteps], mine = 0;
#pragma unroll
    for (uint32_t q = 0; q < kSteps; q++) {
        const uint32_t w = wave_w0 + q * 64 + lane;
        wv[q] = w < words ? a.bitmap[w] : 0u;
        mine += (uint32_t)__builtin_popcount(wv[q]);
    }
    const uint32_t wave_total = (uint32_t)__builtin_amdgcn_readlane((int)wave_scan_add(mine), 63);
    if (lane == 0) red[wave] = wave_total;
    __syncthreads();
    uint32_t pos0 = base;
    for (uint32_t k = 0; k < wave; k++) pos0 += red[k];
#pragma unroll
    for (uint32_t q = 0; q < kSteps; q++) {
        uint32_t w = wv[q];
        const uint32_t pc = (uint32_t)__builtin_popcount(w), incl = wave_scan_add(pc);
        uint32_t pos = pos0 + incl - pc;
        const uint32_t r0 = (wave_w0 + q * 64 + lane) * 32;
        while (w) {
            a.list[pos++] = r0 + (uint32_t)__builtin_ctz(w);
            w &= w - 1;
        }
        pos0 += (uint32_t)__builtin_amdgcn_readlane((int)incl, 63);
// ... 54 lines not shown
    unsigned char *tables = lds + (size_t)n_waves * wave_bytes;
    const VerdictTables vt = verdict_tables(a.n_cols, a.n_rules, a.n_trig, a.n_lits, LT);
    uint16_t *l_trig_off = reinterpret_cast<uint16_t *>(tables + vt.trig_off);
    uint16_t *l_trig_rules = reinterpret_cast<uint16_t *>(tables + vt.trig_rules);
    uint2 *l_rules = reinterpret_cast<uint2 *>(tables + vt.rules);
    uint32_t *l_lits = reinterpret_cast<uint32_t *>(tables + vt.lits);
    uint16_t *l_pub = reinterpret_cast<uint16_t *>(tables + vt.pub);
    if (LT) {
        for (uint32_t k = tid; k <= a.n_cols; k += blockDim.x) l_trig_off[k] = (uint16_t)a.trig_off[k];
        for (uint32_t k = tid; k < a.n_trig; k += blockDim.x) l_trig_rules[k] = a.trig_rules[k];
        for (uint32_t k = tid; k < a.n_rules; k += blockDim.x) {
            const DevRule dr = a.rules[k];
            l_rules[k] = make_uint2(dr.lit_off, dr.lit_cnt | ((uint32_t)dr.eff_unverified << 16) | ((uint32_t)dr.eff_verified << 24));
            l_pub[k] = (uint16_t)dr.public_idx;
        }
        for (uint32_t k = tid; k < a.n_lits; k += blockDim.x) l_lits[k] = a.lits[k];
    }
    __syncthreads();
    const unsigned long long mybit = 1ull << lane;
    const unsigned long long lt_mask = mybit - 1;
    unsigned long long cnt_block = 0, cnt_captcha = 0, cnt_bypass = 0, cnt_allow = 0;

    const uint32_t h_always = lane < rulew ? a.always_rules[lane] : 0u;

    constexpr int kPre = kVerdictPre;
    constexpr int kBitRegs = BR;
    struct Bits {
        unsigned long long w[kBitRegs];
    };
    struct Inputs {
        uint32_t rv[kPre];
        uint32_t base[kPre];
        Bits bits;
        unsigned long long rest[kBitRegs];
        uint32_t flags, n_pairs;
        uint4 pair0;
        uint32_t res0;
    };
    const uint32_t *my_bits[kBitRegs];
    uint32_t my_base[kBitRegs];
    bool my_live[kBitRegs];
#pragma unroll
    for (int r = 0; r < kBitRegs; r++) {
        const uint32_t ps = (uint32_t)r * 64 + lane;
        my_live[r] = ps < a.n_passes;
        my_bits[r] = nullptr;
        my_base[r] = 0;
        if (my_live[r]) {
            const PassInfo pi = a.passes[ps];
            const uint32_t kind = pi.kind_slot >> 24, slot = pi.kind_slot & 0xFFFFFFu;
            if (kind == 3) my_live[r] = false;
            my_bits[r] = kind == 1 ? a.cand_bits + (size_t)slot * a.bit_words : kind == 2 ? a.visit_bits + (size_t)slot * a.bit_words : nullptr;
            my_base[r] = pi.base;
        }
    }
    auto request_bits = [&](const uint32_t g, Bits &bt) {
        const uint32_t gg = min(g, a.n_groups - 1);
#pragma unroll
        for (int r = 0; r < kBitRegs; r++) {
            bt.w[r] = !my_live[r] ? 0ull : my_bits[r] != nullptr ? *reinterpret_cast<const unsigned long long *>(my_bits[r] + 2 * (size_t)gg) : ~0ull;
        }
    };
    auto request_inputs = [&](const uint32_t g, const Bits &bt, Inputs &in) {
        const uint32_t i = g * 64 + lane;
        const bool valid = g < a.n_groups && i < a.n;
        unsigned long long nz[kBitRegs];
#pragma unroll
        for (int r = 0; r < kBitRegs; r++) nz[r] = (uint32_t)r * 64 < a.n_passes ? __ballot(bt.w[r] != 0) : 0ull;
#pragma unroll
        for (int q = 0; q < kPre; q++) {
            uint32_t ps = kNone, base = kNone;
            unsigned long long word = 0;
#pragma unroll
            for (int r = 0; r < kBitRegs; r++) {
                if (ps == kNone && nz[r] != 0) {
                    const int l = __builtin_ctzll(nz[r]);
                    nz[r] &= nz[r] - 1;
                    ps = (uint32_t)r * 64 + (uint32_t)l;
                    word = ((unsigned long long)(uint32_t)__builtin_amdgcn_readlane((int)(bt.w[r] >> 32), l) << 32) | (uint32_t)__builtin_amdgcn_readlane((int)(uint32_t)bt.w[r], l);
                    base = (uint32_t)__builtin_amdgcn_readlane((int)my_base[r], l);
                }
            }
            in.base[q] = base;
            in.rv[q] = (ps != kNone && valid && ((word >> lane) & 1ull)) ? a.rec[(size_t)ps * a.n + i] : 0u;
        }
#pragma unroll
        for (int r = 0; r < kBitRegs; r++) in.rest[r] = nz[r];
        in.bits = bt;
        in.flags = valid ? (uint32_t)a.flags[i] : 0u;
        const uint32_t gg = min(g, a.n_groups - 1);
        in.n_pairs = a.ghdr[gg];
        in.pair0 = a.gpairs[(size_t)gg * a.pair_stride + lane];
        in.res0 = (a.res_words && valid) ? a.res_match[i] : 0u;
    };
    if (!SP) {
        for (uint32_t k = lane; k < a.n_cols; k += 64) col[k] = 0;
        for (uint32_t k = lane; k < colw; k += 64) colnz[k] = 0;
    }
    const uint32_t g_stride = gridDim.x * n_waves;
    Inputs cur;
    Bits b_nxt;
    {
        Bits b_cur;
        request_bits(blockIdx.x * n_waves + wave, b_cur);
        request_inputs(blockIdx.x * n_waves + wave, b_cur, cur);
        request_bits(blockIdx.x * n_waves + wave + g_stride, b_nxt);
    }

    for (uint32_t g = blockIdx.x * n_waves + wave; g < a.n_groups; g += g_stride) {
        const uint32_t i = g * 64 + lane;
        const bool valid = i < a.n;
        const unsigned long long valid_mask = __ballot(valid);
        Inputs nxt;
        request_inputs(g + g_stride, b_nxt, nxt);
        request_bits(g + 2 * g_stride, b_nxt);

        if (!SP) {
            for (uint32_t wv = lane; wv < colw; wv += 64) {
                uint32_t nzw = colnz[wv];
                colnz[wv] = wv == 0 ? 1u : 0u;
                while (nzw) {
                    col[wv * 32 + (uint32_t)__builtin_ctz(nzw)] = 0;
                    nzw &= nzw - 1;
                }
            }
        } else {
            for (uint32_t wv = lane; wv < colw; wv += 64) nz[2 * wv] = wv == 0 ? 1u : 0u;
        }
        for (uint32_t k = lane; k < rulew; k += 64) rulebm[k] = k < 64 ? h_always : a.always_rules[k];
        __builtin_amdgcn_fence(__ATOMIC_ACQ_REL, "wavefront");
        if (!SP && lane == 0) col[0] = ~0ull;

        const uint32_t flags = cur.flags;
        const uint4 *pairs = a.gpairs + (size_t)g * a.pair_stride;
        const uint32_t n_pairs = cur.n_pairs;
        const uint4 pair0 = cur.pair0;
        const unsigned long long verified_mask = __ballot(valid && (flags & PWAF_FLAG_CAPTCHA_VERIFIED));

        auto slot_of = [&](const uint32_t c) {
            const uint32_t w = c >> 5, bits = nz[2 * w], before = nz[2 * w + 1];
            return before + (uint32_t)__builtin_popcount(bits & ((1u << (c & 31u)) - 1u));
        };
        auto word_at = [&](const uint32_t slot) -> unsigned long long * { return slot < v_cap ? vals + slot : spill + (slot - v_cap); };
        auto mark_all = [&](auto phase_tag) {
            constexpr int PH = decltype(phase_tag)::value;
            auto put = [&](const uint32_t c, const unsigned long long m) {
                if (PH == 0) atomicOr(&nz[2 * (c >> 5)], 1u << (c & 31u));
                else if (PH == 1) atomicOr(word_at(slot_of(c)), m);
                else {
                    atomicOr(&col[c], m);
                    atomicOr(&colnz[c >> 5], 1u << (c & 31));
                }
            };
            auto mark_hits = [&](const uint32_t rv, const uint32_t base) {
                if (__ballot(rv != 0) == 0) return;
                if (rv & REC_OVERFLOW) {
                    for (uint32_t k = rv & ~REC_OVERFLOW; k != kNone;) {
                        const PoolEntry pe = a.pool[k];
                        put(base + pe.atom, mybit);
                        k = pe.next;
                    }
                }
#pragma unroll
                for (int half = 0; half < 2; half++) {
                    const uint32_t x = (rv & REC_OVERFLOW) ? 0u : (half == 0 ? rv & 0x7FFFu : (rv >> 15) & 0x7FFFu);
                    unsigned long long todo = __ballot(x != 0);
                    while (todo) {
                        const uint32_t leader = (uint32_t)__builtin_ctzll(todo);
                        const uint32_t xa = (uint32_t)__builtin_amdgcn_readlane((int)x, (int)__builtin_amdgcn_readfirstlane(leader));
                        const unsigned long long same = __ballot(x == xa);
                        todo &= ~same;
                        if (lane == leader) put(base + xa - 1, same);
                    }
                }
            };
            if (!(dbg_skip & 1u)) {
#pragma unroll
                for (int q = 0; q < kPre; q++) {
                    if (cur.base[q] == kNone) break;
                    mark_hits(cur.rv[q], cur.base[q]);
                }
#pragma unroll
                for (int r = 0; r < kBitRegs; r++) {
                    unsigned long long m = cur.rest[r];
                    while (m) {
                        const int l = __builtin_ctzll(m);
                        m &= m - 1;
                        const uint32_t ps = (uint32_t)r * 64 + (uint32_t)l;
                        const unsigned long long word = ((unsigned long long)(uint32_t)__builtin_amdgcn_readlane((int)(cur.bits.w[r] >> 32), l) << 32) |
                                                        (uint32_t)__builtin_amdgcn_readlane((int)(uint32_t)cur.bits.w[r], l);
                        const uint32_t base = (uint32_t)__builtin_amdgcn_readlane((int)my_base[r], l);
                        mark_hits((valid && ((word >> lane) & 1ull)) ? a.rec[(size_t)ps * a.n + i] : 0u, base);
                    }
                }
            }
            for (uint32_t w = 0; w < a.res_words; w++) {
                const uint32_t mw = w == 0 ? cur.res0 : (valid ? a.res_match[(size_t)w * a.n + i] : 0u);
                if (__ballot(mw != 0u) == 0ull) continue;
                uint32_t any = mw;
                for (uint32_t d = 1; d < 64u; d <<= 1) any |= (uint32_t)__shfl_xor((int)any, (int)d, 64);
                any = (uint32_t)__builtin_amdgcn_readfirstlane((int)any);
                for (; any; any &= any - 1u) {
                    const uint32_t k = (uint32_t)__builtin_ctz(any);
                    const unsigned long long who = __ballot(((mw >> k) & 1u) != 0u);
                    if (lane == 0) put(a.res_base + 32u * w + k, who);
                }
            }
            if (!(dbg_skip & 2u)) {
                for (uint32_t p = lane; p < n_pairs; p += 64) {
                    const uint4 pr = p < 64 ? pair0 : pairs[p];
                    const unsigned long long v = ((unsigned long long)pr.w << 32) | pr.z;
                    if (PH == 0) atomicOr(&nz[2 * (pr.x >> 5)], 1u << (pr.x & 31u));
                    else if (PH == 1) {
                        const uint32_t sl = slot_of(pr.x);
                        if (sl < v_cap) vals[sl] = v;
                        else atomicOr(spill + (sl - v_cap), v);
                    }
                    else {
                        col[pr.x] = v;
                        atomicOr(&colnz[pr.x >> 5], 1u << (pr.x & 31));
                    }
                }
            }
        };
        uint32_t n_dirty = 0;
        if (SP) {
            mark_all(std::integral_constant<int, 0>{});
            __builtin_amdgcn_fence(__ATOMIC_ACQ_REL, "wavefront");
            for (uint32_t wb = 0; wb < colw; wb += 64) {
                const uint32_t bits = wb + lane < colw ? nz[2 * (wb + lane)] : 0u;
                const uint32_t pc = (uint32_t)__builtin_popcount(bits), incl = wave_scan_add(pc);
                if (wb + lane < colw) nz[2 * (wb + lane) + 1] = n_dirty + incl - pc;
                n_dirty += (uint32_t)__builtin_amdgcn_readlane((int)incl, 63);
            }
            for (uint32_t k = lane; k < n_dirty; k += 64) {
                if (k < v_cap) vals[k] = k == 0 ? ~0ull : 0ull;
                else atomicExch(spill + (k - v_cap), 0ull);
            }
            __builtin_amdgcn_fence(__ATOMIC_ACQ_REL, "wavefront");
            mark_all(std::integral_constant<int, 1>{});
        } else {
            mark_all(std::integral_constant<int, 2>{});
        }
        __builtin_amdgcn_fence(__ATOMIC_ACQ_REL, "wavefront");
        auto nz_bits = [&](const uint32_t wv) { return SP ? nz[2 * wv] : colnz[wv]; };
        auto col_word = [&](const uint32_t c) -> unsigned long long {
            if (!SP) return col[c];
            const uint32_t w = c >> 5, bits = nz[2 * w], before = nz[2 * w + 1];
            if (!((bits >> (c & 31u)) & 1u)) return 0ull;
            const uint32_t sl = before + (uint32_t)__builtin_popcount(bits & ((1u << (c & 31u)) - 1u));
            return sl < v_cap ? vals[sl] : __hip_atomic_load(spill + (sl - v_cap), __ATOMIC_RELAXED, __HIP_MEMORY_SCOPE_AGENT);
        };

        if (!(dbg_skip & 8u)) {
            uint32_t n_nz = 0;
            for (uint32_t wb = 0; wb < colw; wb += 64) {
                uint32_t nzv = wb + lane < colw ? nz_bits(wb + lane) : 0u;
                const uint32_t pc = (uint32_t)__builtin_popcount(nzv), incl = wave_scan_add(pc);
                uint32_t pos = n_nz + incl - pc;
                while (nzv) {
                    if (pos < a.n_rules) cand[pos] = (uint16_t)((wb + lane) * 32 + (uint32_t)__builtin_ctz(nzv));
                    pos++;
                    nzv &= nzv - 1;
                }
                n_nz += (uint32_t)__builtin_amdgcn_readlane((int)incl, 63);
            }
            __builtin_amdgcn_fence(__ATOMIC_ACQ_REL, "wavefront");
            if (n_nz <= a.n_rules) {
                for (uint32_t j = lane; j < n_nz; j += 64) {
                    const uint32_t c = cand[j];
                    const uint32_t kb = LT ? (uint32_t)l_trig_off[c] : a.trig_off[c], ke = LT ? (uint32_t)l_trig_off[c + 1] : a.trig_off[c + 1];
                    for (uint32_t k = kb; k < ke; k++) {
                        const uint32_t r = LT ? (uint32_t)l_trig_rules[k] : (uint32_t)a.trig_rules[k];
                        atomicOr(&rulebm[r >> 5], 1u << (r & 31));
                    }
// ... 153 lines not shown
    asm volatile("s_mov_b32 m0, %4\n\ts_nop 0\n\tv_writelane_b32 %0, %3, m0\n\tv_writelane_b32 %1, %5, m0\n\tv_writelane_b32 %2, %6, m0"
                 : "+v"(c), "+v"(lo), "+v"(hi)
                 : "s"(s_col), "s"(s_l), "s"(s_lo), "s"(s_hi)
                 : "m0");
}
#pragma clang diagnostic pop

template <bool LT, int BR, bool HITS>
__global__ __launch_bounds__(768, BR == 1 ? (HITS ? 5 : 6) : 1) void verdict2_kernel(VerdictArgs a) {
    extern __shared__ __align__(16) unsigned char lds[];
    const uint32_t tid = threadIdx.x, wave = wave_index(), lane = tid & 63, n_waves = blockDim.x >> 6;
#ifdef PWAF_PROFILING
    const uint32_t dbg_skip = a.debug_skip;
#else
    constexpr uint32_t dbg_skip = 0;
#endif
    const uint32_t rulew = (a.n_rules + 31) / 32;
    const uint32_t e_cap = a.v_cap;
    const uint32_t wave_bytes = verdict_wave_lds_el(a.n_cols, a.n_rules, e_cap);
    unsigned char *mine = lds + (size_t)wave * wave_bytes;
    unsigned long long *vals = reinterpret_cast<unsigned long long *>(mine);
    uint32_t *rulebm = reinterpret_cast<uint32_t *>(vals + e_cap);
    uint16_t *ecol = reinterpret_cast<uint16_t *>(rulebm + rulew);
    uint16_t *cand = reinterpret_cast<uint16_t *>(reinterpret_cast<unsigned char *>(ecol) + ((e_cap * 2 + 3) & ~3u));
    uint8_t *slot = reinterpret_cast<unsigned char *>(cand) + ((a.n_rules * 2 + 3) & ~3u);
    const uint32_t slot_words = ((a.n_cols + 7) & ~7u) / 4;
    unsigned long long *spill = a.spill + (size_t)(blockIdx.x * n_waves + wave) * a.n_cols;
    unsigned char *tables = lds + (size_t)n_waves * wave_bytes;
    const VerdictTables vt = verdict_tables(a.n_cols, a.n_rules, a.n_trig, a.n_lits, LT);
    uint16_t *l_trig_off = reinterpret_cast<uint16_t *>(tables + vt.trig_off);
    uint16_t *l_trig_rules = reinterpret_cast<uint16_t *>(tables + vt.trig_rules);
    uint2 *l_rules = reinterpret_cast<uint2 *>(tables + vt.rules);
    uint32_t *l_lits = reinterpret_cast<uint32_t *>(tables + vt.lits);
    uint16_t *l_pub = reinterpret_cast<uint16_t *>(tables + vt.pub);
    if (LT) {
        for (uint32_t k = tid; k <= a.n_cols; k += blockDim.x) l_trig_off[k] = (uint16_t)a.trig_off[k];
        for (uint32_t k = tid; k < a.n_trig; k += blockDim.x) l_trig_rules[k] = a.trig_rules[k];
        for (uint32_t k = tid; k < a.n_rules; k += blockDim.x) {
            const DevRule dr = a.rules[k];
            l_rules[k] = make_uint2(dr.lit_off, dr.lit_cnt | ((uint32_t)dr.eff_unverified << 16) | ((uint32_t)dr.eff_verified << 24));
            l_pub[k] = (uint16_t)dr.public_idx;
        }
        for (uint32_t k = tid; k < a.n_lits; k += blockDim.x) l_lits[k] = a.lits[k];
    }
    for (uint32_t k = lane; k < slot_words; k += 64) reinterpret_cast<uint32_t *>(slot)[k] = 0u;
    __builtin_amdgcn_fence(__ATOMIC_ACQ_REL, "wavefront");
    if (lane == 0) {
        slot[0] = 1;
        vals[0] = ~0ull;
        ecol[0] = 0;
    }
    __syncthreads();
    const unsigned long long mybit = 1ull << lane;
    const unsigned long long lt_mask = mybit - 1;
    unsigned long long cnt_block = 0, cnt_captcha = 0, cnt_bypass = 0, cnt_allow = 0;
    uint32_t q_rk = 0, q_lo = 0, q_hi = 0, q_n = 0, q_g0 = 0, q_k = 0;
    const uint32_t q_stride = gridDim.x * n_waves;
    auto q_flush = [&]() {
        if (q_n == 0) return;
        uint32_t slot0 = 0;
        if (lane == 0) slot0 = atomicAdd(a.n_hits, q_n);
        slot0 = __builtin_amdgcn_readfirstlane(slot0);
        const uint32_t at = slot0 + lane;
        if (lane < q_n && at < a.hits_cap) {
            pwaf_rule_hit h;
            h.rule_idx = q_rk & 0xFFFFu;
            h.group = q_g0 + (q_rk >> 16) * q_stride;
            h.mask = ((unsigned long long)q_hi << 32) | q_lo;
            a.hits[at] = h;
        }
        q_n = 0;
    };
    const uint32_t h_always = lane < rulew ? a.always_rules[lane] : 0u;
    const bool true_triggers = a.trig_off[1] != a.trig_off[0];

    constexpr int kPre = BR == 1 ? 4 : kVerdictPre;
    constexpr int kBitRegs = BR;
    struct Bits {
        unsigned long long w[kBitRegs];
    };
    struct Inputs {
        uint32_t rv[kPre];
        uint32_t base[kPre];
        Bits bits;
        unsigned long long rest[kBitRegs];
        uint32_t flags, n_pairs;
        uint4 pair0;
        uint32_t res0;
        uint32_t lraw[2];
    };
    const uint32_t *my_bits[kBitRegs];
    uint32_t my_base[kBitRegs];
    bool my_live[kBitRegs];
#pragma unroll
    for (int r = 0; r < kBitRegs; r++) {
        const uint32_t ps = (uint32_t)r * 64 + lane;
        my_live[r] = ps < a.n_passes;
        my_bits[r] = nullptr;
        my_base[r] = 0;
        if (my_live[r]) {
            const PassInfo pi = a.passes[ps];
            const uint32_t kind = pi.kind_slot >> 24, sl = pi.kind_slot & 0xFFFFFFu;
            if (kind == 3) my_live[r] = false;
            my_bits[r] = kind == 1 ? a.cand_bits + (size_t)sl * a.bit_words : kind == 2 ? a.visit_bits + (size_t)sl * a.bit_words : nullptr;
            my_base[r] = pi.base;
        }
    }
    auto request_bits = [&](const uint32_t g, Bits &bt) {
        const uint32_t gg = min(g, a.n_groups - 1);
#pragma unroll
        for (int r = 0; r < kBitRegs; r++)
            bt.w[r] = !my_live[r] ? 0ull : my_bits[r] != nullptr ? *reinterpret_cast<const unsigned long long *>(my_bits[r] + 2 * (size_t)gg) : ~0ull;
    };
    auto request_inputs = [&](const uint32_t g, const Bits &bt, Inputs &in) {
        const uint32_t i = g * 64 + lane;
        const bool valid = g < a.n_groups && i < a.n;
        unsigned long long nzp[kBitRegs];
#pragma unroll
        for (int r = 0; r < kBitRegs; r++) nzp[r] = (uint32_t)r * 64 < a.n_passes ? __ballot(bt.w[r] != 0) : 0ull;
#pragma unroll
        for (int q = 0; q < kPre; q++) {
            uint32_t ps = kNone, base = kNone;
            unsigned long long word = 0;
#pragma unroll
            for (int r = 0; r < kBitRegs; r++) {
                if (ps == kNone && nzp[r] != 0) {
                    const int l = __builtin_ctzll(nzp[r]);
                    nzp[r] &= nzp[r] - 1;
                    ps = (uint32_t)r * 64 + (uint32_t)l;
                    word = ((unsigned long long)(uint32_t)__builtin_amdgcn_readlane((int)(bt.w[r] >> 32), l) << 32) | (uint32_t)__builtin_amdgcn_readlane((int)(uint32_t)bt.w[r], l);
                    base = (uint32_t)__builtin_amdgcn_readlane((int)my_base[r], l);
                }
            }
            in.base[q] = base;
            in.rv[q] = (ps != kNone && valid && ((word >> lane) & 1ull)) ? a.rec[(size_t)ps * a.n + i] : 0u;
        }
#pragma unroll
        for (int r = 0; r < kBitRegs; r++) in.rest[r] = nzp[r];
        in.bits = bt;
        in.flags = valid ? (uint32_t)a.flags[i] : 0u;
        const uint32_t gg = min(g, a.n_groups - 1);
        {
            const uint32_t *src = a.ghdr + gg;
#pragma unroll
            for (uint32_t sl = 0; sl < 2; sl++) {
                if (sl >= a.n_lazy_var) break;
                const uint32_t vi = a.lazy_var[sl];
                if (vi != 5u && lane == 1u + sl) src = (vi < 5u ? a.off[vi] : a.hoff[vi - 7u]) + gg * 64u;
            }
            in.n_pairs = *src;
        }
        in.pair0 = a.gpairs[(size_t)gg * a.pair_stride + lane];
        in.res0 = (a.res_words && valid) ? a.res_match[i] : 0u;
        in.lraw[0] = in.lraw[1] = 0u;
        const uint32_t ii = valid ? i : 0u;
#pragma unroll
        for (uint32_t sl = 0; sl < 2; sl++) {
            if (sl >= a.n_lazy_var || (dbg_skip & 2048u)) break;
            const uint32_t vi = a.lazy_var[sl];
            if (vi == 5u) {
                in.lraw[sl] = a.port[ii];
            } else {
                const uint32_t *o = vi < 5u ? a.off[vi] : a.hoff[vi - 7u];
                in.lraw[sl] = o[ii + 1];
            }
        }
    };
    const uint32_t g_stride = gridDim.x * n_waves;
    Inputs cur;
    Bits b_nxt;
    {
        Bits b_cur;
        request_bits(blockIdx.x * n_waves + wave, b_cur);
        request_inputs(blockIdx.x * n_waves + wave, b_cur, cur);
        request_bits(blockIdx.x * n_waves + wave + g_stride, b_nxt);
    }

    for (uint32_t g = blockIdx.x * n_waves + wave; g < a.n_groups; g += g_stride) {
        const uint32_t i = g * 64 + lane;
        const bool valid = i < a.n;
        const unsigned long long valid_mask = __ballot(valid);
        Inputs nxt;
        request_inputs(g + g_stride, b_nxt, nxt);
        request_bits(g + 2 * g_stride, b_nxt);

        for (uint32_t k = lane; k < rulew; k += 64) rulebm[k] = k < 64 ? h_always : a.always_rules[k];
        __builtin_amdgcn_fence(__ATOMIC_ACQ_REL, "wavefront");

        const uint32_t flags = cur.flags;
        const uint4 *pairs = a.gpairs + (size_t)g * a.pair_stride;
        const uint32_t n_pairs = (uint32_t)__builtin_amdgcn_readlane((int)cur.n_pairs, 0);
        const unsigned long long verified_mask = __ballot(valid && (flags & PWAF_FLAG_CAPTCHA_VERIFIED));

        uint32_t n_entries = 1;
        auto triggers = [&](const uint32_t c) {
            if (dbg_skip & 8u) return;
            const uint32_t kb = LT ? (uint32_t)l_trig_off[c] : a.trig_off[c], ke = LT ? (uint32_t)l_trig_off[c + 1] : a.trig_off[c + 1];
            for (uint32_t k = kb; k < ke; k++) {
                const uint32_t r = LT ? (uint32_t)l_trig_rules[k] : (uint32_t)a.trig_rules[k];
                atomicOr(&rulebm[r >> 5], 1u << (r & 31));
            }
        };
        if (true_triggers && lane == 0) triggers(0);
        auto append_batch = [&](const uint32_t c, const uint32_t lo, const uint32_t hi, const uint32_t cnt) {
            if (lane < cnt) {
                const uint32_t e = n_entries + lane;
                const unsigned long long m = ((unsigned long long)hi << 32) | lo;
                if (e < e_cap) {
                    slot[c] = (uint8_t)(e + 1u);
                    vals[e] = m;
                    ecol[e] = (uint16_t)c;
                } else {
                    slot[c] = 255;
                    atomicExch(spill + c, m);
                }
                triggers(c);
            }
            n_entries += cnt;
        };
        const uint32_t n_first = (dbg_skip & 2u) ? 0u : min(n_pairs, 64u);
        uint32_t b_col = cur.pair0.x, b_lo = cur.pair0.z, b_hi = cur.pair0.w, bn = n_first;
        if (bn == 64) {
            append_batch(b_col, b_lo, b_hi, 64);
            bn = 0;
        }
        auto flush = [&]() {
            if (bn == 0) return;
            append_batch(b_col, b_lo, b_hi, bn);
            bn = 0;
        };
        auto append = [&](const uint32_t c, const unsigned long long m) {
            park96(b_col, b_lo, b_hi, c, m, bn);
            if (++bn == 64) flush();
        };
        auto merge_or_append = [&](const uint32_t c, const unsigned long long m) {
            const uint32_t s = (uint32_t)__builtin_amdgcn_readfirstlane((int)(uint32_t)slot[c]);
            if (s == 0) {
                const uint32_t e = n_entries++;
                if (lane == 0) {
                    if (e < e_cap) {
                        slot[c] = (uint8_t)(e + 1u);
                        vals[e] = m;
                        ecol[e] = (uint16_t)c;
                    } else {
                        slot[c] = 255;
                        atomicExch(spill + c, m);
                    }
                    triggers(c);
                }
            } else if (lane == 0) {
                if (s < 255u) vals[s - 1u] |= m;
                else atomicOr(spill + c, m);
            }
            __builtin_amdgcn_fence(__ATOMIC_ACQ_REL, "wavefront");
        };
        auto mark_hits = [&](const uint32_t rv, const uint32_t base) {
            if (__ballot(rv != 0) == 0) return;
            const bool chained = (rv & REC_OVERFLOW) != 0;
            const bool any_chain = __ballot(chained) != 0;
            if (any_chain) {
                flush();
                __builtin_amdgcn_fence(__ATOMIC_ACQ_REL, "wavefront");
            }
            const uint32_t x0 = chained ? 0u : rv & 0x7FFFu, x1 = chained ? 0u : (rv >> 15) & 0x7FFFu;
            unsigned long long t0 = __ballot(x0 != 0), t1 = __ballot(x1 != 0);
            while ((t0 | t1) != 0) {
                uint32_t xa;
                if (t0 != 0) xa = (uint32_t)__builtin_amdgcn_readlane((int)x0, __builtin_ctzll(t0));
                else xa = (uint32_t)__builtin_amdgcn_readlane((int)x1, __builtin_ctzll(t1));
                const unsigned long long s0 = __ballot(x0 == xa), s1 = __ballot(x1 == xa);
                t0 &= ~s0;
                t1 &= ~s1;
                if (any_chain) merge_or_append(base + xa - 1u, s0 | s1);
                else append(base + xa - 1u, s0 | s1);
            }
            if (any_chain) {
                uint32_t k = chained ? rv & ~REC_OVERFLOW : kNone;
                while (__ballot(k != kNone) != 0) {
                    uint32_t x = 0;
                    if (k != kNone) {
                        const PoolEntry pe = a.pool[k];
                        x = pe.atom + 1u;
                        k = pe.next;
                    }
                    unsigned long long todo = __ballot(x != 0);
                    while (todo != 0) {
                        const uint32_t xa = (uint32_t)__builtin_amdgcn_readlane((int)x, __builtin_ctzll(todo));
                        const unsigned long long same = __ballot(x == xa);
                        todo &= ~same;
                        merge_or_append(base + xa - 1u, same);
                    }
                }
            }
        };
        if (!(dbg_skip & 1u)) {
#pragma unroll
            for (int q = 0; q < kPre; q++) {
                if (cur.base[q] == kNone) break;
                mark_hits(cur.rv[q], cur.base[q]);
            }
#pragma unroll
            for (int r = 0; r < kBitRegs; r++) {
                unsigned long long m = cur.rest[r];
                while (m) {
                    const int l = __builtin_ctzll(m);
                    m &= m - 1;
                    const uint32_t ps = (uint32_t)r * 64 + (uint32_t)l;
                    const unsigned long long word = ((unsigned long long)(uint32_t)__builtin_amdgcn_readlane((int)(cur.bits.w[r] >> 32), l) << 32) |
                                                    (uint32_t)__builtin_amdgcn_readlane((int)(uint32_t)cur.bits.w[r], l);
                    const uint32_t base = (uint32_t)__builtin_amdgcn_readlane((int)my_base[r], l);
                    mark_hits((valid && ((word >> lane) & 1ull)) ? a.rec[(size_t)ps * a.n + i] : 0u, base);
                }
            }
        }
        for (uint32_t w = 0; w < a.res_words; w++) {
            const uint32_t mw = w == 0 ? cur.res0 : (valid ? a.res_match[(size_t)w * a.n + i] : 0u);
            if (__ballot(mw != 0u) == 0ull) continue;
            for (uint32_t any = wave_or(mw); any; any &= any - 1u) {
                const uint32_t k = (uint32_t)__builtin_ctz(any);
                append(a.res_base + 32u * w + k, __ballot(((mw >> k) & 1u) != 0u));
            }
        }
        flush();
        if (!(dbg_skip & 2u)) {
            for (uint32_t p0 = 64; p0 < n_pairs; p0 += 64) {
                const uint32_t cnt = min(64u, n_pairs - p0);
                uint4 pr = make_uint4(0u, 0u, 0u, 0u);
                if (lane < cnt) pr = pairs[p0 + lane];
                append_batch(pr.x, pr.z, pr.w, cnt);
            }
        }
        __builtin_amdgcn_fence(__ATOMIC_ACQ_REL, "wavefront");
        const bool spilled = n_entries > e_cap;
        auto col_word = [&](const uint32_t c) -> unsigned long long {
            const uint32_t s = slot[c];
            if (!spilled) {
                const unsigned long long v = vals[s ? s - 1u : 0u];
                return s ? v : 0ull;
            }
            if (s == 0) return 0ull;
            return s < 255u ? vals[s - 1u] : __hip_atomic_load(spill + c, __ATOMIC_RELAXED, __HIP_MEMORY_SCOPE_AGENT);
        };

        uint32_t n_cand = 0;
        for (uint32_t wb = 0; wb < rulew && !(dbg_skip & 16u); wb += 64) {
            const uint32_t word = wb + lane < rulew ? rulebm[wb + lane] : 0u;
            const uint32_t pc = (uint32_t)__builtin_popcount(word), incl = wave_scan_add(pc);
            uint32_t pos = n_cand + incl - pc, wrd = word;
            while (wrd) {
                cand[pos++] = (uint16_t)((wb + lane) * 32 + (uint32_t)__builtin_ctz(wrd));
                wrd &= wrd - 1;
            }
            n_cand += (uint32_t)__builtin_amdgcn_readlane((int)incl, 63);
        }
        __builtin_amdgcn_fence(__ATOMIC_ACQ_REL, "wavefront");

        unsigned long long pending = valid_mask;
        uint32_t n_exact = 0;
        bool undecided = valid;
        uint32_t my_action = PWAF_ACTION_ALLOW, my_rule = PWAF_RULE_NONE;
        unsigned long long gated = 0;
        for (uint32_t base = 0; base < n_cand && (HITS || pending != 0) && !(dbg_skip & 32u); base += 64) {
            unsigned long long fire = 0, eff_mask = 0;
            unsigned long long match = 0;
            uint32_t lit_off = 0, lit_cnt = 0;
            bool lazy_seen = false;
            if (base + lane < n_cand) {
                const uint32_t my_cand = cand[base + lane];
                uint32_t eff_u, eff_v;
                if (LT) {
                    const uint2 hdr = l_rules[my_cand];
                    lit_off = hdr.x;
                    lit_cnt = hdr.y & 0xFFFFu;
                    eff_u = (hdr.y >> 16) & 0xFFu;
                    eff_v = hdr.y >> 24;
                } else {
                    const DevRule dr = a.rules[my_cand];
                    lit_off = dr.lit_off;
                    lit_cnt = dr.lit_cnt;
                    eff_u = dr.eff_unverified;
                    eff_v = dr.eff_verified;
                }
                unsigned long long acc_or = 0, acc_and = ~0ull;
                for (uint32_t k = lit_off; k < lit_off + lit_cnt; k += 4) {
                    uint32_t lit[4];
#pragma unroll
                    for (int q = 0; q < 4; q++) lit[q] = k + q < lit_off + lit_cnt ? (LT ? l_lits[k + q] : a.lits[k + q]) : 0u;
                    unsigned long long cw[4];
#pragma unroll
                    for (int q = 0; q < 4; q++) cw[q] = (lit[q] & LIT_LAZY) ? 0ull : col_word(lit[q] & LIT_ATOM_MASK);
#pragma unroll
                    for (int q = 0; q < 4; q++) {
                        const unsigned long long t = (lit[q] & LIT_NEG) ? ~cw[q] : cw[q];
                        acc_and &= (lit[q] & LIT_LAZY) ? ~0ull : t;
// ... 782 lines not shown
```

Baseline: 7.292 billion.

## Fold scan planning into preceding kernels and zero match records in verdict

Drops the separate confirm-plan and list-scan-plan kernels. The last block of the confirm kernel, or of each list-scan kernel, now computes the plan for the next list scan, using an atomic ticket counter and agent-scope fences. The filter kernel no longer clears per-request record words; the verdict kernel writes zeros back to the rec entries it consumed for filtered passes. The rec buffer now has a persistent stride and is memset in full only when it is reallocated or marked dirty. This removes small serial launches and redundant memsets, but adds cross-block ticket synchronisation and a correctness dependency on the verdict kernel leaving rec clean between calls.

```diff
diff --git a/pingoo_amd/csrc/engine.cpp b/pingoo_amd/csrc/engine.cpp
--- a/pingoo_amd/csrc/engine.cpp
+++ b/pingoo_amd/csrc/engine.cpp
@@ -187,13 +187,15 @@
     DevBuf err_sink;
     DevBuf ipres;
     DevBuf rec, pool, gate_lists, attr;
+    uint32_t rec_stride = 0;
+    bool rec_dirty = true;
     DevBuf verdict_spill;
     DevBuf res_words;
     DevBuf zero_block;
     View ctrl, cand_bits, visit_bits, walk_bits;
     DevBuf chunk_bits, cand_cnt;
+    DevBuf pairs;
     DevBuf need;
-    DevBuf pairs;
     DevBuf zero_off;
     static constexpr uint32_t kArgSlots = 8;
     DevBuf args;
@@ -866,7 +868,7 @@
     const FilterArgs *d_all = nullptr, *d_s1 = nullptr, *d_s2 = nullptr;
     const ConfirmArgs *d_c = nullptr;
     const ListScanArgs *d_la[2] = {nullptr, nullptr};
-    uint32_t *c_plan = nullptr, *l_plan = nullptr;
+    uint32_t *l_plan = nullptr;
 
     BatchRun(pwaf_engine *e_, Scratch &S_, const pwaf_batch &db_, hipStream_t stream_, const std::vector<uint32_t> *col_begin_)
         : e(e_), S(S_), P(*e_->prog.p), db(db_), stream(stream_), col_begin(col_begin_), sw(switches()), prof(e_, stream_), arg_slot{S_, stream_} {
@@ -877,7 +879,7 @@
         bit_words = 2 * n_groups;
         pair_stride = std::max(1u, e->n_bit_atoms + e->n_cmp_atoms + e->n_short);
         n_slots = (size_t)std::max(kGapLists, e->n_gated);
-        ctrl_words = 2 + n_slots + e->n_filtered;
+        ctrl_words = 2 + n_slots + e->n_filtered + e->lscan_launches[0].size() + e->lscan_launches[1].size();
     }
 
 
@@ -891,7 +893,14 @@
             HIP_TRY(hipMemsetAsync(S.status.p, 0, 8, stream));
         }
         status_word = (uint32_t *)S.status.p + (sync_status ? 1 : 0);
-        if ((rc = S.rec.reserve((size_t)std::max(1u, n_passes) * n * 4))) return rc;
+        {
+            const void *const had = S.rec.p;
+            const bool grew = n > S.rec_stride;
+            if (grew) S.rec_stride = n;
+            if ((rc = S.rec.reserve((size_t)std::max(1u, n_passes) * S.rec_stride * 4))) return rc;
+            if (S.rec.p != had || grew || S.rec_dirty) HIP_TRY(hipMemsetAsync(S.rec.p, 0, S.rec.cap, stream));
+            S.rec_dirty = true;
+        }
         if ((rc = S.attr.reserve(((size_t)n_groups * pair_stride + 64) * 16 + (size_t)n_groups * 4))) return rc;
         if ((rc = S.pool.reserve((size_t)pool_cap * sizeof(PoolEntry)))) return rc;
         uint32_t n_conf = 0;
@@ -976,7 +985,8 @@
         v.country = db.country;
         v.n_cols = P.n_cols;
         v.n_passes = n_passes;
-        v.rec = (const uint32_t *)S.rec.p;
+        v.rec = (uint32_t *)S.rec.p;
+        v.rec_stride = S.rec_stride;
         v.passes = (const PassInfo *)e->pass_table.p;
         if (P.n_residual && e->residual_jit.function) {
             v.res_words = (P.n_residual + 31u) / 32u;
@@ -1039,7 +1049,7 @@
             size_t k1 = k;
             while (k1 < e->groups.size() && e->groups[k1].filtered && !e->groups[k1].filter.heads.empty()) k1++;
             if (k1 == k) { k++; continue; }
-            HIP_TRY(hipMemsetAsync((uint32_t *)S.rec.p + k * (size_t)n, 0, (k1 - k) * (size_t)n * 4, stream));
+            HIP_TRY(hipMemsetAsync((uint32_t *)S.rec.p + k * (size_t)S.rec_stride, 0, ((k1 - k - 1) * (size_t)S.rec_stride + n) * 4, stream));
             k = k1;
         }
         return PWAF_OK;
@@ -1155,20 +1165,37 @@
     }
     int launch_confirm_stage() {
         if (call.empty()) return PWAF_OK;
-        return timed("confirm", 0xF8u, "confirm kernel", [&] { return launch_confirm(call.data(), (uint32_t)call.size(), d_c, c_plan, e->n_cus, stream); });
-    }
-    int launch_list_scans() {
+        const NextPlan next = lscan_chain.empty() ? NextPlan{} : next_plan(0);
+        return timed("confirm", 0xF8u, "confirm kernel", [&] { return launch_confirm(call.data(), (uint32_t)call.size(), d_c, e->n_cus, next, stream); });
+    }
+    struct ListLaunch { int phase; uint32_t first, cnt; uint32_t *plan; };
+    std::vector<ListLaunch> lscan_chain;
+    void chain_list_scans() {
         uint32_t *plan_at = l_plan;
         for (int phase = 0; phase < 2; phase++) {
             uint32_t first = 0;
             for (const uint32_t cnt : e->lscan_launches[phase]) {
-                char nm[48];
-                snprintf(nm, sizeof nm, "lscan_x%u", cnt);
-                const int rc = timed(nm, 0xFDu, "gated scan kernel", [&] { return launch_scan_gated(la[phase].data() + first, cnt, d_la[phase] + first, plan_at, lshapes[phase], stream); });
-                if (rc) return rc;
+                if (cnt != 0 && n != 0) lscan_chain.push_back(ListLaunch{phase, first, cnt, plan_at});
                 plan_at += 2 * cnt + 1;
                 first += cnt;
             }
+        }
+    }
+    NextPlan next_plan(size_t k) const {
+        const ListLaunch &l = lscan_chain[k];
+        uint32_t *const tickets = (uint32_t *)S.ctrl.p + 2 + n_slots + e->n_filtered;
+        return NextPlan{GatedTable{d_la[l.phase] + l.first, l.cnt, 0u}, l.plan, list_scan_waves(la[l.phase].data() + l.first, lshapes[l.phase]), tickets + k};
+    }
+    int launch_list_scans() {
+        for (size_t k = 0; k < lscan_chain.size(); k++) {
+            const ListLaunch &l = lscan_chain[k];
+            const bool planned = k != 0 || (e->n_filtered && confirm_launches(call.data(), (uint32_t)call.size()));
+            const NextPlan next = k + 1 < lscan_chain.size() ? next_plan(k + 1) : NextPlan{};
+            char nm[48];
+            snprintf(nm, sizeof nm, "lscan_x%u", l.cnt);
+            const int rc = timed(nm, 0xFDu, "gated scan kernel",
+                                 [&] { return launch_scan_gated(la[l.phase].data() + l.first, l.cnt, d_la[l.phase] + l.first, l.plan, lshapes[l.phase], planned, next, stream); });
+            if (rc) return rc;
         }
         return PWAF_OK;
     }
@@ -1192,7 +1219,7 @@
         }
         fa.n = n;
         fa.n_atoms = (uint32_t)P.fcmp.size();
-        fa.rec = (uint32_t *)S.rec.p + e->groups.size() * (size_t)n;
+        fa.rec = (uint32_t *)S.rec.p + e->groups.size() * (size_t)S.rec_stride;
         set_pool(fa);
         return timed("fcmp", 0xFBu, "field comparison kernel", [&] { return launch_fcmp(fa, stream); });
     }
@@ -1232,11 +1259,15 @@
         }
         ResidualArgs ra{};
         if ((rc = residual_inputs(ra))) return rc;
-        ra.rec = (uint32_t *)S.rec.p + (size_t)residual_pass * n;
+        ra.rec = (uint32_t *)S.rec.p + (size_t)residual_pass * S.rec_stride;
         set_pool(ra);
         return timed("residual", 0xF9u, "residual kernel", [&] { return launch_residual(ra, stream); });
     }
-    int launch_verdict_stage() { return timed("verdict", 0xFFu, "verdict kernel", [&] { return launch_verdict(v, stream); }); }
+    int launch_verdict_stage() {
+        const int rc = timed("verdict", 0xFFu, "verdict kernel", [&] { return launch_verdict(v, stream); });
+        if (!rc) S.rec_dirty = v.sparse_mode < 3 || (v.debug_skip & 1u) != 0;
+        return rc;
+    }
     int dump_counts() {
         std::vector<uint32_t> cw(ctrl_words);
         HIP_TRY(hipStreamSynchronize(stream));
@@ -1295,7 +1326,7 @@
         a.stride = d.stride;
         a.n_classes = d.n_classes;
         a.n_hot = d.n_hot;
-        a.rec = (uint32_t *)S.rec.p + gi * (size_t)n;
+        a.rec = (uint32_t *)S.rec.p + gi * (size_t)S.rec_stride;
         set_pool(a);
         return a;
     }
@@ -1359,7 +1390,7 @@
             }
             f.slab0 = slab0_of(d.field);
             const uint32_t slabs = slabs_of(f);
-            f.rec = (uint32_t *)S.rec.p + gi * (size_t)n;
+            f.rec = (uint32_t *)S.rec.p + gi * (size_t)S.rec_stride;
             f.chunk_bits = (uint32_t *)S.chunk_bits.p + sub_at;
             f.sub_count = (uint32_t *)S.cand_cnt.p + cnt_at;
             f.pair_base = f.sub_count + slabs;
@@ -1479,7 +1510,7 @@
         a.emit_list = (const uint16_t *)F.emit_list.p;
         a.end_off = (const uint32_t *)F.end_off.p;
         a.end_list = (const uint16_t *)F.end_list.p;
-        a.rec = (uint32_t *)S.rec.p + gi * (size_t)n;
+        a.rec = (uint32_t *)S.rec.p + gi * (size_t)S.rec_stride;
         set_pool(a);
         a.n_cus = e->n_cus;
         return a;
@@ -1542,7 +1573,7 @@
         const Part up[7] = {{L.take(b_all), fall.data(), b_all}, {L.take(b_s1), by_stride[0].data(), b_s1}, {L.take(b_s2), by_stride[1].data(), b_s2}, {L.take(b_c), call.data(), b_c},
                             {L.take(b_l0 + sizeof(ListScanArgs)), la[0].data(), b_l0}, {L.take(b_l1 + sizeof(ListScanArgs)), la[1].data(), b_l1}, {L.take(b_ptrs), ptrs.p, b_ptrs}};
         const size_t up_bytes = L.size();
-        const size_t a_cplan = L.take((call.size() + 2) * 4), a_lplan = L.take((lsplit::plan_words(e->lscan_launches[0]) + lsplit::plan_words(e->lscan_launches[1])) * 4);
+        const size_t a_lplan = L.take((lsplit::plan_words(e->lscan_launches[0]) + lsplit::plan_words(e->lscan_launches[1])) * 4);
         if ((rc = S.args.reserve(L.size()))) return rc;
         char *const abase = (char *)S.args.p;
         d_all = (const FilterArgs *)(abase + up[0].at);
@@ -1552,8 +1583,8 @@
         d_la[0] = (const ListScanArgs *)(abase + up[4].at);
         d_la[1] = (const ListScanArgs *)(abase + up[5].at);
         S.res_cols.p = abase + up[6].at;
-        c_plan = (uint32_t *)(abase + a_cplan);
         l_plan = (uint32_t *)(abase + a_lplan);
+        chain_list_scans();
         if (up_bytes) {
             const uint32_t slot = S.arg_next++ % Scratch::kArgSlots;
             if (S.arg_pending[slot]) HIP_TRY(hipEventSynchronize(S.arg_ev[slot]));
@@ -2918,6 +2949,7 @@
     HIP_TRY(hipSetDevice(e->device));
     const Program &P = *e->prog.p;
     if (sample->n == 0) return PWAF_OK;
+    for (auto &c : e->ctx) c->rec_dirty = true;
     TuneOut T;
     for (const DevGroup &d : e->groups) T.filters.push_back(d.filter);
     if ((rc = tune_host(P, sample, T))) return rc;
diff --git a/pingoo_amd/csrc/kernels.h b/pingoo_amd/csrc/kernels.h
--- a/pingoo_amd/csrc/kernels.h
+++ b/pingoo_amd/csrc/kernels.h
@@ -139,7 +139,9 @@
     const ConfirmArgs *c;
     uint32_t count;
 };
-int launch_confirm(const ConfirmArgs *host, uint32_t count, const ConfirmArgs *dev, uint32_t *plan, uint32_t n_cus, void *stream);
+struct NextPlan;
+inline bool confirm_launches(const ConfirmArgs *host, uint32_t count) { return count != 0 && host[0].n != 0; }
+int launch_confirm(const ConfirmArgs *host, uint32_t count, const ConfirmArgs *dev, uint32_t n_cus, const NextPlan &next, void *stream);
 
 static constexpr uint32_t kStreamSlab = 128 * 1024;
 static constexpr uint32_t kStreamIter = 4096;
@@ -282,7 +284,8 @@
     const uint32_t *asn;
     const uint16_t *country;
     uint32_t n_passes;
-    const uint32_t *rec;
+    uint32_t *rec;
+    uint32_t rec_stride;
     const PassInfo *passes;
     const uint32_t *res_match;
     uint32_t res_words, res_base;
@@ -357,7 +360,14 @@
 };
 ListShape list_shape(uint32_t variant);
 uint32_t list_hot_bytes(const ListShape &shape);
-int launch_scan_gated(const ListScanArgs *host, uint32_t count, const ListScanArgs *dev, uint32_t *plan, const ListShape &shape, void *stream);
+struct NextPlan {
+    GatedTable b;
+    uint32_t *plan;
+    uint32_t n_waves;
+    uint32_t *ticket;
+};
+uint32_t list_scan_waves(const ListScanArgs *host, const ListShape &shape);
+int launch_scan_gated(const ListScanArgs *host, uint32_t count, const ListScanArgs *dev, uint32_t *plan, const ListShape &shape, bool planned, const NextPlan &next, void *stream);
 int launch_verdict(const VerdictArgs &a, void *stream);
 int launch_ipres(const VerdictArgs &a, void *stream);
 int launch_attr(const VerdictArgs &a, void *stream);
diff --git a/pingoo_amd/csrc/kernels.hip b/pingoo_amd/csrc/kernels.hip
--- a/pingoo_amd/csrc/kernels.hip
+++ b/pingoo_amd/csrc/kernels.hip
@@ -417,10 +417,12 @@
 template <int CH, bool WIDE>
 __global__ __launch_bounds__(kScanThreads) void scan_kernel(ScanArgs a) { scan_body<CH, WIDE>(a); }
 
+template <bool FRESH = false>
 __device__ __forceinline__ ListOf list_of(const ListScanArgs &a) {
-    ListOf l{a.req_list, a.req_list != nullptr ? min(*a.n_list, a.n) : a.n};
+    auto word = [](const uint32_t *p) { return FRESH ? __hip_atomic_load(p, __ATOMIC_RELAXED, __HIP_MEMORY_SCOPE_AGENT) : *p; };
+    ListOf l{a.req_list, a.req_list != nullptr ? min(word(a.n_list), a.n) : a.n};
     if (a.dense_mode != 0u) {
-        const bool dense = *a.dense_flag > a.dense_thresh;
+        const bool dense = word(a.dense_flag) > a.dense_thresh;
         if (a.dense_mode == 1u && !dense) l.n_l = 0u;
         if (a.dense_mode == 2u && dense) l.n_l = 0u;
         if (a.dense_mode == 3u && dense) l = ListOf{nullptr, a.n};
@@ -428,35 +430,60 @@
     return l;
 }
 
-__global__ __launch_bounds__(256) void lscan_plan_kernel(GatedTable b, uint32_t *plan , uint32_t n_waves) {
-    __shared__ uint32_t part[256];
-    __shared__ unsigned long long all_entries;
+__device__ __forceinline__ void lscan_plan(const GatedTable &b, uint32_t *plan , const uint32_t n_waves, uint32_t *lds) {
+    unsigned long long *all_entries = reinterpret_cast<unsigned long long *>(lds + 2);
+    uint32_t *part = lds + 4;
     const uint32_t t = threadIdx.x;
     uint32_t items = 0;
-    const uint32_t n_l = t < b.count ? list_of(b.g[t]).n_l : 0u;
-    if (t == 0) all_entries = 0ull;
+    const uint32_t n_l = t < b.count ? list_of<true>(b.g[t]).n_l : 0u;
+    if (t == 0) *all_entries = 0ull;
     __syncthreads();
-    if (n_l != 0u) atomicAdd(&all_entries, (unsigned long long)n_l);
+    if (n_l != 0u) atomicAdd(all_entries, (unsigned long long)n_l);
     __syncthreads();
     if (t < b.count) {
         const uint32_t room = n_waves > b.count ? n_waves - b.count : 1u;
-        const unsigned long long per_wave = (all_entries + room - 1u) / room;
+        const unsigned long long per_wave = (*all_entries + room - 1u) / room;
         uint32_t epi = 1;
         while (epi < 16u && epi < per_wave) epi <<= 1;
         while (epi < 64u * kListWalks && (n_l + epi - 1) / epi > n_waves) epi <<= 1;
         items = (n_l + epi - 1) / epi;
         plan[b.count + 1 + t] = epi;
     }
-    part[t] = items;
+    if (t < 256u) part[t] = items;
     __syncthreads();
     for (uint32_t d = 1; d < 256; d <<= 1) {
-        const uint32_t v = t >= d ? part[t - d] : 0u;
+        const uint32_t v = (t < 256u && t >= d) ? part[t - d] : 0u;
         __syncthreads();
-        part[t] += v;
+        if (t < 256u) part[t] += v;
         __syncthreads();
     }
     if (t < b.count) plan[t] = part[t] - items;
     if (t == 0) plan[b.count] = part[255];
+}
+
+__device__ __forceinline__ void plan_next_launch(const NextPlan &np, uint32_t *lds) {
+    if (np.b.count == 0u) return;
+    asm volatile("s_waitcnt vmcnt(0)" ::: "memory");
+    __syncthreads();
+    if (threadIdx.x == 0) {
+        __builtin_amdgcn_fence(__ATOMIC_RELEASE, "agent");
+        asm volatile("s_waitcnt vmcnt(0)" ::: "memory");
+        const uint32_t drawn = __hip_atomic_fetch_add(np.ticket, 1u, __ATOMIC_RELAXED, __HIP_MEMORY_SCOPE_AGENT);
+        const bool last = drawn + 1u == gridDim.x;
+        if (last) {
+            __builtin_amdgcn_fence(__ATOMIC_ACQUIRE, "agent");
+            asm volatile("s_waitcnt vmcnt(0)" ::: "memory");
+        }
+        lds[0] = last ? 1u : 0u;
+    }
+    __syncthreads();
+    if (lds[0] == 0u) return;
+    lscan_plan(np.b, np.plan, np.n_waves, lds);
+}
+
+__global__ __launch_bounds__(256) void lscan_plan_first_kernel(GatedTable b, uint32_t *plan, uint32_t n_waves) {
+    __shared__ unsigned long long lds[130];
+    lscan_plan(b, plan, n_waves, reinterpret_cast<uint32_t *>(lds));
 }
 
 __device__ __forceinline__ uint32_t list_step_slow(const uint16_t *hot, const PWAF_GLOBAL uint16_t *flat, const uint64_t *delta, const uint32_t state, const uint32_t c,
@@ -582,7 +609,7 @@
 }
 
 template <uint32_t THREADS>
-__global__ __launch_bounds__(THREADS, THREADS == 512 ? 6 : 4) void lscan_kernel(GatedTable b, const uint32_t *plan, uint32_t hot_bytes) {
+__global__ __launch_bounds__(THREADS, THREADS == 512 ? 6 : 4) void lscan_kernel(GatedTable b, const uint32_t *plan, uint32_t hot_bytes, NextPlan next) {
     extern __shared__ uint32_t lscan_lds[];
     __builtin_amdgcn_s_setprio(3);
     if ((uint32_t)(uintptr_t)(PWAF_LDS unsigned char *)lscan_lds != 0u) __builtin_trap();
@@ -776,28 +803,10 @@
         }
         it = it_end;
     }
-}
-
-__global__ __launch_bounds__(256) void confirm_plan_kernel(ConfirmTableDev b, uint32_t *plan ) {
-    __shared__ uint32_t part[256];
-    const uint32_t t = threadIdx.x;
-    uint32_t items = 0;
-    if (t < b.count) {
-        const ConfirmArgs *pa = &b.c[t];
-        const bool dense = pa->dense_flag != nullptr && *pa->dense_flag > pa->dense_thresh;
-        items = dense ? 0u : (min(*pa->pair_count, pa->pair_cap) + kConfirmThreads - 1) / kConfirmThreads;
-    }
-    part[t] = items;
-    __syncthreads();
-    for (uint32_t d = 1; d < 256; d <<= 1) {
-        const uint32_t v = t >= d ? part[t - d] : 0u;
-        __syncthreads();
-        part[t] += v;
-        __syncthreads();
-    }
-    if (t < b.count) plan[t] = part[t] - items;
-    if (t == 0) plan[b.count] = part[255];
-}
+    plan_next_launch(next, lscan_lds);
+}
+
+__device__ __forceinline__ uint32_t wave_scan_add(uint32_t x);
 
 __device__ __noinline__ void merge_atom(PoolEntry *pool, uint32_t *pool_count, uint32_t *status, uint32_t pool_cap, uint32_t *rec, uint32_t atom) {
     auto rmw_read = [](uint32_t *p) { return atomicOr(p, 0u); };
@@ -837,14 +846,37 @@
     }
 }
 
-__global__ __launch_bounds__(kConfirmThreads, 8) void confirm_kernel(ConfirmTableDev b, const uint32_t *plan) {
+__global__ __launch_bounds__(kConfirmThreads, 8) void confirm_kernel(ConfirmTableDev b, NextPlan next) {
     __shared__ uint32_t head[kFilterEntries], ftab[kFilterEntries];
     __shared__ uint32_t pool[kConfirmPoolBytes / 4];
     constexpr uint32_t kConfirmQueue = 1024;
-    __shared__ uint32_t app_cnt, app_base, app_queue[kConfirmQueue];
+    __shared__ uint32_t app_cnt, app_base;
+    __shared__ __attribute__((aligned(8))) uint32_t app_queue[kConfirmQueue];
+    __shared__ uint32_t plan[257];
     __builtin_amdgcn_s_setprio(3);
     if (threadIdx.x == 0) app_cnt = 0;
-    const uint32_t total = plan[b.count];
+    {
+        const uint32_t t = threadIdx.x;
+        uint32_t items = 0, incl = 0;
+        if (t < b.count) {
+            const ConfirmArgs *pa = &b.c[t];
+            const bool dense = pa->dense_flag != nullptr && *pa->dense_flag > pa->dense_thresh;
+            items = dense ? 0u : (min(*pa->pair_count, pa->pair_cap) + kConfirmThreads - 1) / kConfirmThreads;
+        }
+        if (t < 256u) {
+            incl = wave_scan_add(items);
+            if ((t & 63u) == 63u) app_queue[t >> 6] = incl;
+        }
+        __syncthreads();
+        if (t < 256u) {
+            uint32_t before = 0;
+            for (uint32_t w = 0; w < (t >> 6); w++) before += app_queue[w];
+            plan[t] = before + incl - items;
+            if (t == 255u) plan[256] = before + incl;
+        }
+        __syncthreads();
+    }
+    const uint32_t total = plan[256];
     const uint32_t it0 = (uint32_t)((uint64_t)total * blockIdx.x / gridDim.x), it1 = (uint32_t)((uint64_t)total * (blockIdx.x + 1) / gridDim.x);
     for (uint32_t it = it0; it < it1;) {
         uint32_t ps = 0;
@@ -979,6 +1011,7 @@
             if (threadIdx.x == 0) app_cnt = 0;
         }
     }
+    plan_next_launch(next, app_queue);
 }
 
 int launch_scan(const ScanArgs &a, void *stream) {
@@ -1017,24 +1050,22 @@
     return (int)hipGetLastError();
 }
 
-int launch_confirm(const ConfirmArgs *host, uint32_t count, const ConfirmArgs *dev, uint32_t *plan, uint32_t n_cus, void *stream) {
-    if (count == 0 || host[0].n == 0) return 0;
+int launch_confirm(const ConfirmArgs *host, uint32_t count, const ConfirmArgs *dev, uint32_t n_cus, const NextPlan &next, void *stream) {
+    if (!confirm_launches(host, count)) return 0;
     if (count > 256) return (int)hipErrorInvalidValue;
     ConfirmTableDev b{dev, count};
-    hipLaunchKernelGGL(confirm_plan_kernel, dim3(1), dim3(256), 0, (hipStream_t)stream, b, plan);
-    hipError_t e = hipGetLastError();
-    if (e != hipSuccess) return (int)e;
     uint64_t max_items = 0;
     for (uint32_t k = 0; k < count; k++) max_items += ((uint64_t)host[k].pair_cap + kConfirmThreads - 1) / kConfirmThreads;
-    const uint32_t blocks = (uint32_t)std::min<uint64_t>(max_items, (uint64_t)std::max(1u, n_cus) * 2u);
-    const uint32_t *cplan = plan;
-    hipLaunchKernelGGL(confirm_kernel, dim3(blocks), dim3(kConfirmThreads), 0, (hipStream_t)stream, b, cplan);
+    const uint32_t blocks = (uint32_t)std::max<uint64_t>(1u, std::min<uint64_t>(max_items, (uint64_t)std::max(1u, n_cus) * 2u));
+    hipLaunchKernelGGL(confirm_kernel, dim3(blocks), dim3(kConfirmThreads), 0, (hipStream_t)stream, b, next);
     return (int)hipGetLastError();
 }
 
 static const void *lscan_fn(bool wide) { return wide ? reinterpret_cast<const void *>(lscan_kernel<1024>) : reinterpret_cast<const void *>(lscan_kernel<512>); }
 
-int launch_scan_gated(const ListScanArgs *host, uint32_t count, const ListScanArgs *dev, uint32_t *plan, const ListShape &shape, void *stream) {
+uint32_t list_scan_waves(const ListScanArgs *host, const ListShape &shape) { return std::max(1u, host[0].n_cus) * shape.wg_per_cu * (shape.threads / 64u); }
+
+int launch_scan_gated(const ListScanArgs *host, uint32_t count, const ListScanArgs *dev, uint32_t *plan, const ListShape &shape, bool planned, const NextPlan &next, void *stream) {
     if (count == 0 || host[0].n == 0) return 0;
     if (count > 256) return (int)hipErrorInvalidValue;
     GatedTable b{dev, count, 0u};
@@ -1043,14 +1074,17 @@
     b.debug = async_mode;
 #endif
     const uint32_t blocks = std::max(1u, host[0].n_cus) * shape.wg_per_cu;
-    hipLaunchKernelGGL(lscan_plan_kernel, dim3(1), dim3(256), 0, (hipStream_t)stream, b, plan, blocks * (shape.threads / 64u));
-    hipError_t e = hipGetLastError();
-    if (e != hipSuccess) return (int)e;
+    if (!planned) {
+        hipLaunchKernelGGL(lscan_plan_first_kernel, dim3(1), dim3(256), 0, (hipStream_t)stream, b, plan, list_scan_waves(host, shape));
+        const hipError_t pe = hipGetLastError();
+        if (pe != hipSuccess) return (int)pe;
+    }
     const uint32_t *cplan = plan;
     uint32_t hot_bytes = list_hot_bytes(shape);
-    void *args[] = {&b, &cplan, &hot_bytes};
+    NextPlan np = next;
+    void *args[] = {&b, &cplan, &hot_bytes, &np};
     const void *fn = lscan_fn(shape.threads == 1024);
-    e = hipLaunchKernel(fn, dim3(blocks), dim3(shape.threads), args, shape.hot_bytes + 16 + 256, (hipStream_t)stream);
+    const hipError_t e = hipLaunchKernel(fn, dim3(blocks), dim3(shape.threads), args, shape.hot_bytes + 16 + 256, (hipStream_t)stream);
     return (int)(e != hipSuccess ? e : hipGetLastError());
 }
 
@@ -1628,15 +1662,6 @@
                 continue;
             }
             if (pair_base + k < a.pair_cap) a.pairs[pair_base + k] = make_uint2(l, chunk);
-            if (a.n_heads == 0) {
-                uint32_t r = l, steps = 0;
-                for (; r < a.n && steps < 48u; r++, steps++) {
-                    const uint32_t s = a.off[r];
-                    if (s >= byte0 + 16u) break;
-                    if (a.off[r + 1] > s) a.rec[r] = 0u;
-                }
-                if (steps == 48u) redo = true;
-            }
         }
         if (__ballot(redo) == 0ull) return;
     }
@@ -1656,13 +1681,6 @@
             if (r2 < a.n) { s_n = a.off[r2]; e_n = a.off[r2 + 1]; }
         }
         if (a.pairs != nullptr) {
-            if (a.n_heads == 0 && live && e > s) {
-                const uint32_t g_lo = s >> 4, g_hi = (e - 1u) >> 4;
-                if (g_hi >= c_first + lo_c && g_lo < c_first + hi_c) {
-                    const uint32_t y0 = g_lo > c_first + lo_c ? g_lo - c_first : lo_c, y1 = min(g_hi - c_first, hi_c - 1u);
-                    if (rank_of(y1 + 1u) != rank_of(y0)) a.rec[r] = 0u;
-                }
-            }
             if (live && e > s) {
                 const uint32_t f_lo = s == begin ? s >> 4 : (s + 15u) >> 4, f_hi = (e - 1u) >> 4;
                 if (f_lo <= f_hi && f_hi >= c_first + lo_c && f_lo < c_first + hi_c) {
@@ -1883,7 +1901,7 @@
                 }
             }
             in.base[q] = base;
-            in.rv[q] = (ps != kNone && valid && ((word >> lane) & 1ull)) ? a.rec[(size_t)ps * a.n + i] : 0u;
+            in.rv[q] = (ps != kNone && valid && ((word >> lane) & 1ull)) ? a.rec[(size_t)ps * a.rec_stride + i] : 0u;
         }
 #pragma unroll
         for (int r = 0; r < kBitRegs; r++) in.rest[r] = nz[r];
@@ -1991,7 +2009,7 @@
                         const unsigned long long word = ((unsigned long long)(uint32_t)__builtin_amdgcn_readlane((int)(cur.bits.w[r] >> 32), l) << 32) |
                                                         (uint32_t)__builtin_amdgcn_readlane((int)(uint32_t)cur.bits.w[r], l);
                         const uint32_t base = (uint32_t)__builtin_amdgcn_readlane((int)my_base[r], l);
-                        mark_hits((valid && ((word >> lane) & 1ull)) ? a.rec[(size_t)ps * a.n + i] : 0u, base);
+                        mark_hits((valid && ((word >> lane) & 1ull)) ? a.rec[(size_t)ps * a.rec_stride + i] : 0u, base);
                     }
                 }
             }
@@ -2311,6 +2329,7 @@
     struct Inputs {
         uint32_t rv[kPre];
         uint32_t base[kPre];
+        uint32_t zb[kPre];
         Bits bits;
         unsigned long long rest[kBitRegs];
         uint32_t flags, n_pairs;
@@ -2321,19 +2340,23 @@
     const uint32_t *my_bits[kBitRegs];
     uint32_t my_base[kBitRegs];
     bool my_live[kBitRegs];
+    unsigned long long zero_back[kBitRegs];
 #pragma unroll
     for (int r = 0; r < kBitRegs; r++) {
         const uint32_t ps = (uint32_t)r * 64 + lane;
         my_live[r] = ps < a.n_passes;
         my_bits[r] = nullptr;
         my_base[r] = 0;
+        bool zb = false;
         if (my_live[r]) {
             const PassInfo pi = a.passes[ps];
             const uint32_t kind = pi.kind_slot >> 24, sl = pi.kind_slot & 0xFFFFFFu;
             if (kind == 3) my_live[r] = false;
+            zb = kind == 1;
             my_bits[r] = kind == 1 ? a.cand_bits + (size_t)sl * a.bit_words : kind == 2 ? a.visit_bits + (size_t)sl * a.bit_words : nullptr;
             my_base[r] = pi.base;
         }
+        zero_back[r] = __ballot(zb);
     }
     auto request_bits = [&](const uint32_t g, Bits &bt) {
         const uint32_t gg = min(g, a.n_groups - 1);
@@ -2349,7 +2372,7 @@
         for (int r = 0; r < kBitRegs; r++) nzp[r] = (uint32_t)r * 64 < a.n_passes ? __ballot(bt.w[r] != 0) : 0ull;
 #pragma unroll
         for (int q = 0; q < kPre; q++) {
-            uint32_t ps = kNone, base = kNone;
+            uint32_t ps = kNone, base = kNone, zb = kNone;
             unsigned long long word = 0;
 #pragma unroll
             for (int r = 0; r < kBitRegs; r++) {
@@ -2357,12 +2380,14 @@
                     const int l = __builtin_ctzll(nzp[r]);
                     nzp[r] &= nzp[r] - 1;
                     ps = (uint32_t)r * 64 + (uint32_t)l;
+                    if ((zero_back[r] >> l) & 1ull) zb = ps;
                     word = ((unsigned long long)(uint32_t)__builtin_amdgcn_readlane((int)(bt.w[r] >> 32), l) << 32) | (uint32_t)__builtin_amdgcn_readlane((int)(uint32_t)bt.w[r], l);
                     base = (uint32_t)__builtin_amdgcn_readlane((int)my_base[r], l);
                 }
             }
             in.base[q] = base;
-            in.rv[q] = (ps != kNone && valid && ((word >> lane) & 1ull)) ? a.rec[(size_t)ps * a.n + i] : 0u;
+            in.zb[q] = zb;
+            in.rv[q] = (ps != kNone && valid && ((word >> lane) & 1ull)) ? a.rec[(size_t)ps * a.rec_stride + i] : 0u;
         }
 #pragma unroll
         for (int r = 0; r < kBitRegs; r++) in.rest[r] = nzp[r];
@@ -2526,6 +2551,7 @@
 #pragma unroll
             for (int q = 0; q < kPre; q++) {
                 if (cur.base[q] == kNone) break;
+                if (cur.zb[q] != kNone && cur.rv[q] != 0u) a.rec[(size_t)cur.zb[q] * a.rec_stride + i] = 0u;
                 mark_hits(cur.rv[q], cur.base[q]);
             }
 #pragma unroll
@@ -2538,7 +2564,9 @@
                     const unsigned long long word = ((unsigned long long)(uint32_t)__builtin_amdgcn_readlane((int)(cur.bits.w[r] >> 32), l) << 32) |
                                                     (uint32_t)__builtin_amdgcn_readlane((int)(uint32_t)cur.bits.w[r], l);
                     const uint32_t base = (uint32_t)__builtin_amdgcn_readlane((int)my_base[r], l);
-                    mark_hits((valid && ((word >> lane) & 1ull)) ? a.rec[(size_t)ps * a.n + i] : 0u, base);
+                    const uint32_t rv_here = (valid && ((word >> lane) & 1ull)) ? a.rec[(size_t)ps * a.rec_stride + i] : 0u;
+                    if (((zero_back[r] >> l) & 1ull) && rv_here != 0u) a.rec[(size_t)ps * a.rec_stride + i] = 0u;
+                    mark_hits(rv_here, base);
                 }
             }
         }
```

Result: slower. 7.178 billion (-1.6%).
